# DrorT/demucs

Hardware: AMD Instinct MI355X
Metric: real-time factor (audio-sec/wall-sec) htdemucs 4-stem 44.1kHz stereo, 1/8 GPU (higher is better)
Workload: dtype f32

## Files before the change

demucs_amd/_lib.py:

```python
from __future__ import annotations

import ctypes as C
import os
import threading

_HERE = os.path.dirname(os.path.abspath(__file__))
LIB_PATH = os.environ.get("DEMUCS_AMD_LIB") or os.path.join(_HERE, "libdemucs_amd.so")

MI_OK = 0


class MiTensorDesc(C.Structure):
    _fields_ = [("name", C.c_char_p), ("data", C.c_void_p), ("numel", C.c_int64)]


class MiConfig(C.Structure):
    _fields_ = [("n_sources", C.c_int32), ("segment_length", C.c_int32), ("max_batch", C.c_int32),
                ("dtype", C.c_int32)]


class MiProfileRow(C.Structure):
    _fields_ = [("name", C.c_char * 48), ("launches", C.c_int64), ("ms", C.c_double), ("flops", C.c_double),
                ("bytes", C.c_double)]


class MiConvDesc(C.Structure):
    _fields_ = [
        ("wt", C.c_void_p), ("M", C.c_int32), ("Mpad", C.c_int32), ("K", C.c_int32), ("Kpad", C.c_int32),
        ("ktab", C.c_void_p),
        ("x", C.c_void_p), ("x_bstride", C.c_int64),
        ("B", C.c_int32), ("D1", C.c_int32), ("D2", C.c_int32), ("O1", C.c_int32), ("O2", C.c_int32),
        ("S1", C.c_int32), ("S2", C.c_int32),
        ("pro", C.c_int32), ("pro_stats", C.c_void_p), ("pro_w", C.c_void_p), ("pro_b", C.c_void_p),
        ("row_mode", C.c_int32),
        ("epi", C.c_int32), ("flags", C.c_int32),
        ("bias", C.c_void_p), ("scale", C.c_void_p), ("res", C.c_void_p), ("emb", C.c_void_p),
        ("y", C.c_void_p), ("y_bstride", C.c_int64), ("y_cstride", C.c_int64),
        ("stats", C.c_void_p), ("gn_stats", C.c_void_p), ("gn_w", C.c_void_p), ("gn_b", C.c_void_p),
        ("out_len", C.c_int32), ("tile_m", C.c_int32), ("plain", C.c_int32), ("half", C.c_int32),
        ("o2_valid", C.c_int32), ("ktab_len", C.c_int32), ("sink", C.c_void_p), ("wx", C.c_void_p), ("tr_stride", C.c_int32), ("tr_pad", C.c_int32), ("x_ld", C.c_int32), ("x_ld_pad", C.c_int32), ("wh", C.c_void_p),
        ("xh", C.c_void_p), ("xh_n", C.c_int64), ("yh", C.c_void_p), ("yh_n", C.c_int64),
        ("wtap", C.c_void_p), ("ntaps", C.c_int32), ("tap_k2", C.c_int32), ("tap_pad1", C.c_int32), ("tap_pad2", C.c_int32),
        ("tap_dil1", C.c_int32), ("tap_dil2", C.c_int32), ("yh_pq", C.c_int64),
        ("dma_rows", C.c_int32), ("dma_rows_pad", C.c_int32),
    ]


SIGNATURES = {
    "mi_model_create": (C.c_int, [C.POINTER(MiConfig), C.POINTER(MiTensorDesc), C.c_size_t, C.POINTER(C.c_void_p)]),
    "mi_model_destroy": (None, [C.c_void_p]),
    "mi_model_forward": (C.c_int, [C.c_void_p, C.c_void_p, C.c_void_p, C.c_int32, C.c_void_p]),
    "mi_model_forward_core": (C.c_int, [C.c_void_p, C.c_void_p, C.c_void_p, C.c_void_p, C.c_void_p, C.c_int32, C.c_void_p]),
    "mi_model_tap": (C.c_int, [C.c_void_p, C.c_char_p, C.c_void_p, C.c_int32, C.POINTER(C.c_int64), C.c_void_p]),
    "mi_hmodel_create": (C.c_int, [C.POINTER(MiConfig), C.POINTER(MiTensorDesc), C.c_size_t, C.POINTER(C.c_void_p)]),
    "mi_hmodel_destroy": (None, [C.c_void_p]),
    "mi_hmodel_forward": (C.c_int, [C.c_void_p, C.c_void_p, C.c_void_p, C.c_int32, C.c_int32, C.c_void_p]),
    "mi_hmodel_tap": (C.c_int, [C.c_void_p, C.c_char_p, C.c_void_p, C.c_int32, C.POINTER(C.c_int64), C.c_void_p]),
    "mi_hmodel_device_bytes": (C.c_int64, [C.c_void_p]),
    "mi_hmodel_status": (C.c_int, [C.c_void_p, C.c_void_p]),
    "mi_set_two_streams": (C.c_int, [C.c_int32]),
    "mi_set_split_bf16": (C.c_int, [C.c_int32]),
    "mi_set_istft_fused": (C.c_int, [C.c_int32]),
    "mi_set_transpose_tiles": (C.c_int, [C.c_int32]),
    "mi_profile_begin": (C.c_int, [C.c_void_p]),
    "mi_profile_end": (C.c_int, [C.c_void_p, C.POINTER(MiProfileRow), C.c_int32, C.POINTER(C.c_int32), C.c_void_p]),
    "mi_model_device_bytes": (C.c_int64, [C.c_void_p]),
    "mi_segments_gather": (C.c_int, [C.c_void_p, C.c_int64, C.c_int32, C.c_void_p, C.c_int32, C.c_int32, C.c_void_p,
                                     C.c_int64, C.c_void_p]),
    "mi_ola_accumulate": (C.c_int, [C.c_void_p, C.c_int64, C.c_int32, C.c_void_p, C.c_int32, C.c_int64, C.c_void_p, C.c_void_p,
                                    C.c_void_p, C.c_int32, C.c_int64, C.c_int64, C.c_void_p, C.c_int32, C.c_void_p]),
    "mi_ola_finish": (C.c_int, [C.c_void_p, C.c_int64, C.c_int32, C.c_int64, C.c_void_p, C.c_void_p, C.c_int32,
                                C.c_int32, C.c_void_p, C.c_void_p]),
    "mi_segments_gather_packed": (C.c_int, [C.c_void_p, C.c_int64, C.c_int32, C.c_void_p, C.c_int32, C.c_int32, C.c_void_p,
                                            C.c_int64, C.c_void_p]),
    "mi_ola_accumulate_packed": (C.c_int, [C.c_void_p, C.c_int64, C.c_int32, C.c_void_p, C.c_int32, C.c_int64, C.c_void_p, C.c_int32,
                                           C.c_void_p, C.c_int32, C.c_void_p, C.c_int64, C.c_void_p]),
    "mi_ola_finish_packed": (C.c_int, [C.c_void_p, C.c_int64, C.c_int32, C.c_void_p, C.c_int32, C.c_void_p, C.c_int32, C.c_void_p,
                                       C.c_int64, C.c_void_p]),
    "mi_stream_emit": (C.c_int, [C.c_void_p, C.c_int64, C.c_int32, C.c_int32, C.c_void_p, C.c_int32, C.c_void_p, C.c_int32,
                                 C.c_void_p, C.c_int64, C.c_void_p, C.c_int32, C.c_int32, C.c_int32, C.c_void_p, C.c_int64,
                                 C.c_void_p, C.c_int64, C.c_void_p]),
    "mi_streams_emit": (C.c_int, [C.c_void_p, C.c_int64, C.c_int32, C.c_int32, C.c_void_p, C.c_int32, C.c_int64, C.c_void_p,
                                  C.c_int32, C.c_void_p, C.c_int32, C.c_void_p, C.c_int64, C.c_void_p, C.c_int32, C.c_int32,
                                  C.c_int32, C.c_void_p, C.c_int32, C.c_void_p, C.c_int64, C.c_void_p]),
    "mi_streams_append": (C.c_int, [C.c_void_p, C.c_int64, C.c_int32, C.c_void_p, C.c_int32, C.c_int64, C.c_void_p, C.c_int32,
                                    C.c_void_p]),
    "mi_streams_convert_append": (C.c_int, [C.c_void_p, C.c_int64, C.c_int32, C.c_void_p, C.c_int32, C.c_int64, C.c_void_p, C.c_int64,
                                            C.c_void_p, C.c_int64, C.c_void_p, C.c_int32, C.c_int32, C.c_void_p]),
    "mi_streams_compact": (C.c_int, [C.c_void_p, C.c_int64, C.c_void_p, C.c_int64, C.c_void_p, C.c_int32, C.c_int64, C.c_void_p]),
    "mi_mono_stats_scratch_bytes": (C.c_int32, []),
    "mi_mono_stats": (C.c_int, [C.c_void_p, C.c_int32, C.c_int64, C.c_void_p, C.c_void_p, C.c_void_p]),
    "mi_track_affine": (C.c_int, [C.c_void_p, C.c_int64, C.c_void_p, C.c_int32, C.c_void_p]),
    "mi_prevent_clip": (C.c_int, [C.c_void_p, C.c_int64, C.c_int32, C.c_void_p, C.c_void_p, C.c_void_p]),
    "mi_two_stems": (C.c_int, [C.c_void_p, C.c_int32, C.c_int32, C.c_void_p, C.c_int32, C.c_int64, C.c_void_p, C.c_void_p]),
    "mi_deliver_peaks": (C.c_int, [C.c_void_p, C.c_int32, C.c_int64, C.c_int32, C.c_int32, C.c_void_p, C.c_int32, C.c_int64, C.c_void_p]),
    "mi_deliver_pcm": (C.c_int, [C.c_void_p, C.c_int32, C.c_int64, C.c_int32, C.c_int32, C.c_void_p, C.c_int32, C.c_void_p, C.c_int64,
                                 C.c_void_p]),
    "mi_deliver_resample_pcm": (C.c_int, [C.c_void_p, C.c_int32, C.c_int64, C.c_int32, C.c_int32, C.c_void_p, C.c_int64, C.c_void_p,
                                          C.c_int64, C.c_int32, C.c_void_p, C.c_int64, C.c_void_p]),
    "mi_stft_cac": (C.c_int, [C.c_void_p, C.c_int32, C.c_int32, C.c_void_p, C.c_void_p]),
    "mi_istft_cac": (C.c_int, [C.c_void_p, C.c_int32, C.c_int32, C.c_int32, C.c_void_p, C.c_void_p]),
    "mi_stft_norm": (C.c_int, [C.c_void_p, C.c_int32, C.c_int32, C.c_void_p, C.c_int32, C.c_void_p, C.c_void_p, C.c_void_p]),
    "mi_istft_full": (C.c_int, [C.c_void_p, C.c_int32, C.c_int32, C.c_int32, C.c_int32, C.c_void_p, C.c_void_p, C.c_int32, C.c_void_p,
                                C.c_void_p, C.c_void_p]),
    "mi_item_norm": (C.c_int, [C.c_void_p, C.c_int32, C.c_int64, C.c_void_p, C.c_void_p, C.c_void_p, C.c_void_p]),
    "mi_item_denorm": (C.c_int, [C.c_void_p, C.c_int32, C.c_int64, C.c_void_p, C.c_void_p, C.c_void_p]),
    "mi_conv_forward": (C.c_int, [C.POINTER(MiConvDesc), C.c_void_p]),
    "mi_resample_frac": (C.c_int, [C.c_void_p, C.c_int32, C.c_int64, C.c_void_p, C.c_int32, C.c_int32, C.c_int32, C.c_void_p, C.c_int64,
                                   C.c_void_p]),
    "mi_conv_pack_split": (C.c_int, [C.c_void_p, C.c_int32, C.c_int32, C.c_int32, C.c_void_p, C.c_void_p]),
    "mi_conv_pack_half": (C.c_int, [C.c_void_p, C.c_int32, C.c_int32, C.c_int32, C.c_void_p, C.c_void_p]),
    "mi_f32_to_image": (C.c_int, [C.c_void_p, C.c_int32, C.c_int32, C.c_int64, C.c_int32, C.c_void_p, C.c_void_p]),
    "mi_conv_pack_tap": (C.c_int, [C.c_void_p, C.c_int32, C.c_int32, C.c_int32, C.c_int32, C.c_void_p, C.c_void_p]),
    "mi_attention": (C.c_int, [C.c_void_p, C.c_void_p, C.c_void_p, C.c_void_p, C.c_int32, C.c_int32, C.c_int32,
                               C.c_int32, C.c_int64, C.c_int64, C.c_int64, C.c_int32, C.c_void_p]),
    "mi_attention_split": (C.c_int, [C.c_void_p, C.c_void_p, C.c_void_p, C.c_void_p, C.c_int32, C.c_int32, C.c_int32,
                                     C.c_int32, C.c_int64, C.c_int64, C.c_int64, C.c_void_p]),
    "mi_attention_heads": (C.c_int, [C.c_void_p, C.c_void_p, C.c_void_p, C.c_void_p, C.c_int32, C.c_int32, C.c_int32, C.c_int32,
                                     C.c_int32, C.c_int32, C.c_int32, C.c_void_p]),
    "mi_attention_heads_image": (C.c_int, [C.c_void_p, C.c_void_p, C.c_void_p, C.c_void_p, C.c_int64, C.c_int32, C.c_int32, C.c_int32,
                                           C.c_int32, C.c_int32, C.c_int32, C.c_int32, C.c_void_p]),
    "mi_attention_image": (C.c_int, [C.c_void_p, C.c_void_p, C.c_void_p, C.c_void_p, C.c_int64, C.c_int32, C.c_int32, C.c_int32,
                                     C.c_int32, C.c_int64, C.c_int64, C.c_int32, C.c_void_p]),
    "mi_lstm_seq": (C.c_int, [C.c_void_p, C.c_void_p, C.c_int32, C.c_int32, C.c_int32, C.c_void_p, C.c_int32, C.c_void_p]),
    "mi_gn_gelu": (C.c_int, [C.c_void_p, C.c_int32, C.c_int32, C.c_int32, C.c_int32, C.c_int32, C.c_int32, C.c_void_p, C.c_void_p,
                             C.c_void_p, C.c_void_p]),
    "mi_gram_order": (C.c_int32, [C.c_int32]),
    "mi_gn_gelu_gram": (C.c_int, [C.c_void_p, C.c_int32, C.c_int32, C.c_int32, C.c_int32, C.c_int32, C.c_int32, C.c_int32, C.c_void_p,
                                  C.c_void_p, C.c_void_p, C.c_void_p, C.c_int32, C.c_void_p]),
    "mi_dconv_gn_gelu_gram": (C.c_int, [C.c_void_p, C.c_int32, C.c_int32, C.c_int32, C.c_int32, C.c_int32, C.c_int32, C.c_int32,
                                        C.c_void_p, C.c_void_p, C.c_void_p, C.c_void_p, C.c_int32, C.c_void_p]),
    "mi_gram_finalize": (C.c_int, [C.c_void_p, C.c_int32, C.c_int32, C.c_int32, C.c_void_p, C.c_void_p, C.c_double, C.c_double,
                                   C.c_double, C.c_double, C.c_float, C.c_void_p, C.c_void_p]),
    "mi_layernorm_cf": (C.c_int, [C.c_void_p, C.c_int32, C.c_int32, C.c_int32, C.c_void_p, C.c_void_p, C.c_void_p,
                                  C.c_void_p, C.c_void_p]),
    "mi_token_norm": (C.c_int, [C.c_int32, C.c_void_p, C.c_int32, C.c_int32, C.c_int32, C.c_void_p, C.c_void_p, C.c_void_p, C.c_void_p,
                                C.c_void_p, C.c_void_p, C.c_void_p, C.c_int64, C.c_int32, C.c_void_p]),
    "mi_local_attn": (C.c_int, [C.c_void_p, C.c_int32, C.c_int32, C.c_int32, C.c_int32, C.c_void_p, C.c_int32, C.c_void_p]),
    "mi_group_norm_apply": (C.c_int, [C.c_void_p, C.c_int32, C.c_int32, C.c_int32, C.c_int32, C.c_int32, C.c_int32, C.c_void_p,
                                      C.c_void_p, C.c_int32, C.c_int32, C.c_void_p, C.c_void_p, C.c_int32, C.c_void_p, C.c_int32,
                                      C.c_int32, C.c_int32, C.c_int32, C.c_void_p, C.c_void_p, C.c_void_p]),
    "mi_blstm_unfold": (C.c_int, [C.c_void_p, C.c_int32, C.c_int32, C.c_int32, C.c_int32, C.c_int32, C.c_int32, C.c_void_p, C.c_void_p]),
    "mi_blstm_restitch": (C.c_int, [C.c_void_p, C.c_int32, C.c_int32, C.c_int32, C.c_int32, C.c_int32, C.c_int32, C.c_void_p,
                                    C.c_void_p, C.c_void_p]),
    "mi_row_affine_pitch": (C.c_int, [C.c_void_p, C.c_int32, C.c_int32, C.c_int32, C.c_int32, C.c_void_p, C.c_void_p, C.c_void_p]),
    "mi_dconv_row": (C.c_int, [C.c_void_p, C.c_void_p, C.c_int32, C.c_int32, C.c_int32, C.c_int32, C.c_void_p, C.c_int32, C.c_void_p]),
    "mi_dconv_time_layer": (C.c_int, [C.c_void_p, C.c_void_p, C.c_int32, C.c_int32, C.c_int32, C.c_int32, C.c_int32, C.c_void_p,
                                      C.c_void_p, C.c_void_p, C.c_void_p, C.c_void_p, C.c_void_p]),
    "mi_debug_set_post_launch_hook": (None, [C.c_void_p]),
    "mi_debug_last_conv_route": (C.c_int, []),
    "mi_debug_last_conv_tile": (C.c_int, []),
    "mi_debug_conv_route": (C.c_int, [C.POINTER(MiConvDesc), C.POINTER(C.c_int)]),
    "mi_debug_switches": (C.c_int, [C.c_char_p, C.c_int32]),
    "mi_last_error": (C.c_char_p, []),
    "mi_version": (C.c_char_p, []),
}

_lib = None
_lock = threading.Lock()


class EngineError(RuntimeError):
    """A libdemucs_amd call returned a non-zero status (the reference convention for this path
    is "exceptions propagate", demucs/apply.py:289-293)."""


def load() -> C.CDLL:
    global _lib
    with _lock:
        if _lib is None:
            if not os.path.exists(LIB_PATH):
                raise EngineError(
                    f"{LIB_PATH} not found: build it with `python -c 'import __graft_entry__ as g; g.build()'` "
                    "(hipcc --offload-arch=gfx950).  demucs_amd has no CPU / eager fallback.")
            lib = C.CDLL(LIB_PATH)
            for name, (res, args) in SIGNATURES.items():
                fn = getattr(lib, name)
                fn.restype = res
                fn.argtypes = args
            _lib = lib
    return _lib


def check(status: int, what: str) -> None:
    if status != MI_OK:
        msg = load().mi_last_error().decode(errors="replace")
        raise EngineError(f"{what} failed ({status}): {msg}")


def current_stream_ptr() -> int:
    import torch
    return torch.cuda.current_stream().cuda_stream
```

demucs_amd/csrc/api.hip:

```cpp
#include <new>

#include "hmodel.h"
#include "model.h"

namespace mi {

post_launch_hook_t g_post_launch_hook = nullptr;
int g_last_conv_route = -1;
int g_last_conv_tile = -1;

char *last_error_buf() {
    static thread_local char buf[1024] = "";
    return buf;
}

int set_error(int code, const char *fmt, ...) {
    va_list ap;
    va_start(ap, fmt);
    vsnprintf(last_error_buf(), 1024, fmt, ap);
    va_end(ap);
    return code;
}

struct Tables {
// ... 476 lines not shown
    float *yt = nullptr, *fr = nullptr;
    MI_TRY(ws.get((size_t)B * S * T * 4 * 2048, &yt));
    MI_TRY(ws.get((size_t)B * S * T * 2 * 4096, &fr));
    hipStream_t st = (hipStream_t)stream;
    const int r = launch_istft(y_dev, B, S, L, (const float2 *)denorm_f_dev, xt_dev, (const float2 *)denorm_t_dev, tb, yt, fr, wav_dev, st,
                               xt_pitch, y_pitch);
    return finish_entry(r, st, "mi_istft_full");
}

int mi_istft_cac(const float *x_dev, int32_t B, int32_t S, int32_t L, float *wav_dev, void *stream) {
    MI_REQUIRE(x_dev && wav_dev && B > 0 && S > 0 && (int64_t)B * S <= 16383 && L >= 1, "mi_istft_cac: bad argument");
    return mi_istft_full(x_dev, B, S, L, 0, nullptr, nullptr, 0, nullptr, wav_dev, stream);
}

int mi_item_norm(const float *x_dev, int32_t rows, int64_t count, float *y_dev, float *norm_dev, float *denorm_dev, void *stream) {
    MI_REQUIRE(x_dev && y_dev && norm_dev && denorm_dev, "mi_item_norm: null argument");
    MI_REQUIRE(rows >= 1 && rows <= 65535, "mi_item_norm: rows = %d outside [1, 65535] (the grid's y range)", rows);
    MI_REQUIRE(count >= 2, "mi_item_norm: count = %lld: the unbiased std divides by count - 1", (long long)count);
    TestScratch ws;
    double *stats = nullptr;
    MI_TRY(ws.get((size_t)2 * kStatSlots * rows, &stats));
    hipStream_t st = (hipStream_t)stream;
    MI_HIP(hipMemsetAsync(stats, 0, sizeof(double) * 2 * kStatSlots * rows, st));
    int r = launch_row_stats(x_dev, rows, count, count, stats, st);
    if (r == MI_OK) r = launch_finalize_stats(stats, rows, (double)count, 1e-5f, 1, (float2 *)norm_dev, (float2 *)denorm_dev, st);
    if (r == MI_OK) r = launch_row_affine(x_dev, rows, count, (const float2 *)norm_dev, y_dev, st);
    return finish_entry(r, st, "mi_item_norm");
}

int mi_item_denorm(const float *x_dev, int32_t rows, int64_t count, const float *denorm_dev, float *y_dev, void *stream) {
    MI_REQUIRE(x_dev && denorm_dev && y_dev, "mi_item_denorm: null argument");
    MI_REQUIRE(rows >= 1 && rows <= 65535 && count >= 1, "mi_item_denorm: rows = %d outside [1, 65535] or count = %lld < 1", rows, (long long)count);
    return launch_row_denorm(x_dev, rows, count, (const float2 *)denorm_dev, y_dev, (hipStream_t)stream);
}

int mi_conv_forward(const struct mi_conv_desc *desc, void *stream) {
    MI_REQUIRE(desc, "mi_conv_forward: null descriptor");
    return launch_conv(*desc, (hipStream_t)stream);
}

int mi_resample_frac(const float *x_dev, int32_t rows, int64_t length, const float *table_dev, int32_t old_sr, int32_t new_sr,
                     int32_t width, float *y_dev, int64_t out_length, void *stream) {
    MI_REQUIRE(x_dev && table_dev && y_dev && old_sr > 0 && new_sr > 0 && width > 0, "mi_resample_frac: bad argument");
    return launch_resample_frac(x_dev, rows, length, table_dev, old_sr, new_sr, width, y_dev, out_length, (hipStream_t)stream);
}

int mi_conv_pack_split(const float *wt_dev, int32_t Kpad, int32_t Mpad, int32_t tile_m, void *wx_dev, void *stream) {
    MI_REQUIRE(wt_dev && wx_dev && Kpad > 0 && Mpad > 0 && (conv_x6_supported(tile_m) || tile_m == 192), "mi_conv_pack_split: bad argument");
    MI_REQUIRE(tile_m != 192 || Mpad % 192 == 0, "mi_conv_pack_split: tile_m 192 needs Mpad %% 192 == 0 (Mpad %d)", Mpad);
    return launch_pack_split(wt_dev, Kpad, Mpad, tile_m == 192 ? 96 : tile_m, wx_dev, (hipStream_t)stream);
}

int mi_conv_pack_tap(const float *wt_dev, int32_t Mpad, int32_t Cin, int32_t ntaps, int32_t dtype, void *wtap_dev, void *stream) {
    MI_REQUIRE(wt_dev && wtap_dev && Mpad > 0 && Cin > 0 && ntaps > 0, "mi_conv_pack_tap: bad argument");
    return launch_pack_tap(wt_dev, Mpad, Cin, ntaps, dtype, wtap_dev, (hipStream_t)stream);
}

int mi_f32_to_image(const float *x_dev, int32_t B, int32_t C, int64_t P, int32_t dtype, void *img_dev, void *stream) {
    MI_REQUIRE(x_dev && img_dev && B > 0 && C > 0 && P > 0, "mi_f32_to_image: bad argument");
    return launch_f32_to_image(x_dev, B, C, P, dtype, img_dev, (hipStream_t)stream);
}

int mi_conv_pack_half(const float *wt_dev, int32_t Kpad, int32_t Mpad, int32_t dtype, void *wh_dev, void *stream) {
    MI_REQUIRE(wt_dev && wh_dev && Kpad > 0 && Mpad > 0, "mi_conv_pack_half: bad argument");
    return launch_pack_half(wt_dev, Kpad, Mpad, dtype, wh_dev, (hipStream_t)stream);
}

int mi_attention(const float *q_dev, const float *k_dev, const float *v_dev, float *o_dev, int32_t B, int32_t heads, int32_t Tq,
                 int32_t Tk, int64_t q_batch_stride, int64_t kv_batch_stride, int64_t o_batch_stride, int32_t dtype, void *stream) {
    MI_REQUIRE(q_dev && k_dev && v_dev && o_dev && B > 0 && heads > 0 && Tq > 0 && Tk > 0, "mi_attention: bad argument");
    return launch_attention(q_dev, k_dev, v_dev, o_dev, B, heads, Tq, Tk, q_batch_stride, kv_batch_stride, o_batch_stride, dtype,
                            (hipStream_t)stream);
}

int mi_attention_split(const float *q_dev, const float *k_dev, const float *v_dev, float *o_dev, int32_t B, int32_t heads, int32_t Tq,
                       int32_t Tk, int64_t q_batch_stride, int64_t kv_batch_stride, int64_t o_batch_stride, void *stream) {
    MI_REQUIRE(q_dev && k_dev && v_dev && o_dev && B > 0 && heads > 0 && Tq > 0 && Tk > 0, "mi_attention_split: bad argument");
    return launch_attention_x6(q_dev, k_dev, v_dev, o_dev, B, heads, Tq, Tk, q_batch_stride, kv_batch_stride, o_batch_stride,
                               (hipStream_t)stream);
}

int mi_attention_heads(const void *q_dev, const void *k_dev, const void *v_dev, float *o_dev, int32_t B, int32_t heads, int32_t Tq, int32_t Tk,
                       int32_t Tq_pitch, int32_t Tk_pitch, int32_t dtype, void *stream) {
    MI_REQUIRE(q_dev && k_dev && v_dev && o_dev && B > 0 && heads > 0 && Tq > 0 && Tk > 0, "mi_attention_heads: bad argument");
    const void *zero = conv_zero_page();
    MI_REQUIRE(zero, "mi_attention_heads: could not allocate the zero page");
    return launch_attention_heads(q_dev, k_dev, v_dev, zero, B, heads, Tq, Tk, Tq_pitch, Tk_pitch, dtype, nullptr, 0, o_dev,
                                  (int64_t)heads * 64 * Tq, (hipStream_t)stream);
}

int mi_attention_heads_image(const void *q_dev, const void *k_dev, const void *v_dev, void *img_dev, int64_t n_img, int32_t B, int32_t heads,
                             int32_t Tq, int32_t Tk, int32_t Tq_pitch, int32_t Tk_pitch, int32_t dtype, void *stream) {
    MI_REQUIRE(q_dev && k_dev && v_dev && img_dev && B > 0 && heads > 0 && Tq > 0 && Tk > 0, "mi_attention_heads_image: bad argument");
    const void *zero = conv_zero_page();
    MI_REQUIRE(zero, "mi_attention_heads_image: could not allocate the zero page");
    return launch_attention_heads(q_dev, k_dev, v_dev, zero, B, heads, Tq, Tk, Tq_pitch, Tk_pitch, dtype, img_dev, n_img, nullptr, 0,
                                  (hipStream_t)stream);
}

int mi_attention_image(const float *q_dev, const float *k_dev, const float *v_dev, void *img_dev, int64_t n_img, int32_t B,
                       int32_t heads, int32_t Tq, int32_t Tk, int64_t q_batch_stride, int64_t kv_batch_stride, int32_t dtype,
                       void *stream) {
    MI_REQUIRE(q_dev && k_dev && v_dev && img_dev && B > 0 && heads > 0 && Tq > 0 && Tk > 0, "mi_attention_image: bad argument");
    MI_REQUIRE(dtype == MI_DTYPE_BF16 || dtype == MI_DTYPE_F16, "mi_attention_image: dtype %d is not a half mode", dtype);
    return launch_attention(q_dev, k_dev, v_dev, nullptr, B, heads, Tq, Tk, q_batch_stride, kv_batch_stride, 0, dtype,
                            (hipStream_t)stream, img_dev, n_img);
}

int mi_gn_gelu(float *x_dev, int32_t B, int32_t C, int32_t C_alloc, int32_t D1, int32_t D2, int32_t row_mode, const float *stats_dev,
               const float *w_dev, const float *b_dev, void *stream) {
    MI_REQUIRE(x_dev && stats_dev && w_dev && b_dev && B > 0 && C > 0 && D1 > 0 && D2 > 0, "mi_gn_gelu: bad argument");
    MI_REQUIRE(C_alloc >= C, "mi_gn_gelu: C_alloc < C");
    return launch_gn_gelu(x_dev, B, C, C_alloc, D1, D2, row_mode, (const float2 *)stats_dev, w_dev, b_dev, (hipStream_t)stream);
}

int32_t mi_gram_order(int32_t h) { return gram_hp(h); }

int mi_lstm_seq(const float *gx_dev, const float *whh_host, int32_t N, int32_t H, int32_t W, float *out_dev, int32_t mode, void *stream) {
    MI_REQUIRE(mode == 0 || mode == 1 || mode == 2, "mi_lstm_seq: mode 0 (one launch per step), 1 (persistent kernel) or 2 (generic small kernel)");
    hipStream_t st = (hipStream_t)stream;
    if (mode == 2) {
        MI_REQUIRE(gx_dev && whh_host && out_dev && N > 0 && N <= 65535 && W > 0 && H >= 1 && H <= 64,
                   "mi_lstm_seq: bad argument (mode 2 needs 1 <= H <= 64)");
        const size_t bytes = (size_t)2 * 4 * H * H * sizeof(float);
        float *wn = nullptr;
        MI_HIP(hipMalloc((void **)&wn, bytes));
        int rs = MI_OK;
        if (hipMemcpyAsync(wn, whh_host, bytes, hipMemcpyHostToDevice, st) != hipSuccess) rs = set_error(MI_EHIP, "mi_lstm_seq: hipMemcpyAsync failed");
        if (rs == MI_OK) rs = launch_lstm_small(gx_dev, wn, N, H, W, out_dev, st);
        const hipError_t es = hipStreamSynchronize(st);
        if (es != hipSuccess && rs == MI_OK) rs = set_error(MI_EHIP, "mi_lstm_seq: hipStreamSynchronize: %s", hipGetErrorString(es));
        (void)hipFree(wn);
        return rs;
    }
    MI_REQUIRE(gx_dev && whh_host && out_dev && N > 0 && W > 0 && (H == 192 || H == 384), "mi_lstm_seq: bad argument (H must be 192 or 384)");
    std::vector<float> packed((size_t)2 * 4 * H * H);
    pack_lstm_whh(whh_host, H, packed.data());
    float *wd = nullptr, *state = nullptr;
    void *scratch = nullptr;
    unsigned *flag = nullptr;
    int r = MI_OK;
    auto fail = [&](hipError_t e, const char *what) { if (e != hipSuccess && r == MI_OK) r = set_error(MI_EHIP, "mi_lstm_seq: %s: %s", what, hipGetErrorString(e)); };
    fail(hipMalloc((void **)&wd, packed.size() * sizeof(float)), "hipMalloc");
    fail(hipMalloc((void **)&state, (size_t)6 * N * H * sizeof(float)), "hipMalloc");
    fail(hipMalloc(&scratch, lstm_persist_scratch_bytes()), "hipMalloc");
    fail(hipHostMalloc((void **)&flag, 64, hipHostMallocMapped), "hipHostMalloc");
    if (r == MI_OK) {
        *flag = 0;
        fail(hipMemcpyAsync(wd, packed.data(), packed.size() * sizeof(float), hipMemcpyHostToDevice, st), "hipMemcpyAsync");
        if (r == MI_OK) r = mode ? launch_lstm_persist(gx_dev, wd, N, H, W, out_dev, scratch, flag, st) : launch_lstm_seq(gx_dev, wd, N, H, W, out_dev, state, st);
        fail(hipStreamSynchronize(st), "hipStreamSynchronize");
        if (r == MI_OK && *(volatile unsigned *)flag) r = set_error(MI_EHIP, "mi_lstm_seq: the persistent kernel timed out waiting for its hidden-state exchange");
        if (r == MI_OK && mode && switches().lstm_debug) {
                        unsigned dbg[16] = {};
            (void)hipMemcpy(dbg, (char *)scratch + lstm_persist_ctl_offset(), sizeof(dbg), hipMemcpyDeviceToHost);
            fprintf(stderr, "[lstm] H %d N %d W %d: block 0 / wave 1 spent %.1f us gathering h in %u poll passes (%.2f us, %.2f passes per step); "
                    "%s stores\n", H, N, W, dbg[2] * 0.01, dbg[3], dbg[2] * 0.01 / std::max(1, W - 1), (double)dbg[3] / std::max(1, W - 1),
                    dbg[4] ? "same-XCD plain" : "write-through");
            fprintf(stderr, "[lstm]   shader cycles per step: gather %.0f, issue + products %.0f, LDS write + barrier %.0f, gate stage %.0f; whole step %.0f\n",
                    (double)dbg[8] / W, (double)dbg[9] / W, (double)dbg[10] / W, (double)dbg[11] / W, (double)dbg[12] / W);
        }
    }
    if (wd) (void)hipFree(wd);
    if (state) (void)hipFree(state);
    if (scratch) (void)hipFree(scratch);
    if (flag) (void)hipHostFree(flag);
    return r;
}

int mi_gn_gelu_gram(float *x_dev, int32_t B, int32_t h, int32_t C_alloc, int32_t D1, int32_t D2, int32_t pitch, int32_t row_mode,
                    const float *stats_dev, const float *w_dev, const float *b_dev, double *gram_dev, int32_t slots, void *stream) {
    MI_REQUIRE(x_dev && stats_dev && w_dev && b_dev && gram_dev && B > 0 && h > 0 && D1 > 0 && D2 > 0 && slots > 0, "mi_gn_gelu_gram: bad argument");
    MI_REQUIRE(C_alloc >= h && pitch >= D2, "mi_gn_gelu_gram: C_alloc < h or pitch < D2");
    return launch_gn_gelu_gram(x_dev, B, h, C_alloc, D1, D2, pitch, row_mode, (const float2 *)stats_dev, w_dev, b_dev, gram_dev, slots,
                               false, (hipStream_t)stream);
}

int mi_dconv_gn_gelu_gram(float *x_dev, int32_t B, int32_t h, int32_t C_alloc, int32_t D1, int32_t D2, int32_t pitch, int32_t row_mode,
                          const float *stats_dev, const float *w_dev, const float *b_dev, double *gram_dev, int32_t slots, void *stream) {
    MI_REQUIRE(x_dev && stats_dev && w_dev && b_dev && gram_dev && B > 0 && h > 0 && D1 > 0 && D2 > 0 && slots > 0, "mi_dconv_gn_gelu_gram: bad argument");
    MI_REQUIRE(C_alloc >= h && C_alloc <= gram_hp(h) && pitch >= D2, "mi_dconv_gn_gelu_gram: C_alloc outside [h, mi_gram_order(h)] or pitch < D2");
    return launch_gn_gelu_gram(x_dev, B, h, C_alloc, D1, D2, pitch, row_mode, (const float2 *)stats_dev, w_dev, b_dev, gram_dev, slots,
                               true, (hipStream_t)stream);
}

int mi_gram_finalize(double *gram_dev, int32_t rows, int32_t h, int32_t slots, const double *wt_dev, const double *ct_dev, double sum_b,
                     double sum_bsq, double cols, double count, float eps, float *stats_out_dev, void *stream) {
    MI_REQUIRE(gram_dev && wt_dev && ct_dev && stats_out_dev && rows > 0 && h > 0 && slots > 0 && count > 0.0, "mi_gram_finalize: bad argument");
    return launch_gram_finalize(gram_dev, rows, h, slots, wt_dev, ct_dev, sum_b, sum_bsq, cols, count, eps, (float2 *)stats_out_dev,
                                (hipStream_t)stream);
}

int mi_layernorm_cf(const float *x_dev, int32_t B, int32_t C, int32_t T, const float *w_dev, const float *b_dev,
                    const float *add_dev, float *y_dev, void *stream) {
    MI_REQUIRE(x_dev && w_dev && b_dev && y_dev, "mi_layernorm_cf: null argument");
    return launch_layernorm_cf(x_dev, B, C, T, w_dev, b_dev, add_dev, y_dev, nullptr, (hipStream_t)stream);
}

int mi_token_norm(int32_t mode, const float *x_dev, int32_t B, int32_t C, int32_t T, const float *w_dev, const float *b_dev,
                  const float *pe_dev, const float *gstat_dev, float *y_dev, float *ostat_dev, void *img_dev, int64_t img_n,
                  int32_t img_dtype, void *stream) {
    MI_REQUIRE(mode >= 0 && mode <= 2, "mi_token_norm: mode %d (0 LayerNorm, 1 statistics, 2 GroupNorm(1) apply)", mode);
    MI_REQUIRE(x_dev && B > 0 && B <= 65535 && C > 0 && T > 0, "mi_token_norm: bad argument");
    hipStream_t st = (hipStream_t)stream;
    if (mode == 1) {
        MI_REQUIRE(ostat_dev, "mi_token_norm: mode 1 writes only the statistics, ostat_dev is NULL");
        return launch_token_stats(x_dev, B, C, T, (float2 *)ostat_dev, st, img_dev, img_n, img_dtype);
    }
    MI_REQUIRE(w_dev && b_dev && y_dev, "mi_token_norm: mode %d needs w_dev, b_dev and y_dev", mode);
    if (mode == 0) return launch_layernorm_cf(x_dev, B, C, T, w_dev, b_dev, pe_dev, y_dev, (float2 *)ostat_dev, st, img_dev, img_n, img_dtype);
    MI_REQUIRE(gstat_dev, "mi_token_norm: mode 2 needs gstat_dev");
    return launch_gn_apply_tokstats(x_dev, B, C, T, (const float2 *)gstat_dev, w_dev, b_dev, y_dev, (float2 *)ostat_dev, st, img_dev, img_n,
                                    img_dtype);
}

int mi_local_attn(const float *qkc_dev, int32_t B, int32_t C, int32_t T, int32_t ld, float *out_dev, int32_t ld_o, void *stream) {
    MI_REQUIRE(qkc_dev && out_dev && B > 0 && B <= 65535 && C > 0 && T > 0, "mi_local_attn: bad argument");
    MI_REQUIRE(ld_o >= T, "mi_local_attn: output pitch %d < T = %d", ld_o, T);
    return launch_local_attn(qkc_dev, B, C, T, ld, out_dev, ld_o, (hipStream_t)stream);
}

int mi_group_norm_apply(const float *x_dev, int32_t B, int32_t Cin, int32_t G, int32_t in_pitch, int32_t in_len, int32_t off,
                        const float *w_dev, const float *b_dev, int32_t glu, int32_t gelu, const float *scale_dev, const float *res_dev,
                        int32_t res_pitch, float *y_dev, int32_t Cout, int32_t out_len, int32_t out_pitch, int32_t chan_div,
                        double *stats_ws_dev, float *stats_out_dev, void *stream) {
    MI_REQUIRE(x_dev && w_dev && b_dev && y_dev && stats_ws_dev && stats_out_dev, "mi_group_norm_apply: null argument");
    MI_REQUIRE(B > 0 && B <= 65535 && Cin > 0 && G > 0 && (int64_t)B * G <= 65535 && Cin % G == 0 && Cout > 0 && Cout <= 65535 && in_len > 0 && out_len > 0 &&
               chan_div >= 1 && Cin % chan_div == 0, "mi_group_norm_apply: bad sizes");
    MI_REQUIRE(in_pitch == in_len, "mi_group_norm_apply: statistics need contiguous channel rows (in_pitch %d != in_len %d)", in_pitch, in_len);
    MI_REQUIRE(off >= 0 && (int64_t)off + out_len <= in_len, "mi_group_norm_apply: window [%d, %d + %d) outside the %d input columns", off, off,
               out_len, in_len);
    MI_REQUIRE(out_pitch >= out_len && (!res_dev || res_pitch >= out_len), "mi_group_norm_apply: a row pitch below out_len = %d", out_len);
    hipStream_t st = (hipStream_t)stream;
    const int64_t cnt = (int64_t)(Cin / G) * in_len;
    MI_TRY(launch_row_stats(x_dev, B * G, cnt, cnt, stats_ws_dev, st));
    MI_TRY(launch_finalize_stats(stats_ws_dev, B * G, (double)cnt, 1e-5f, 0, (float2 *)stats_out_dev, nullptr, st));
    return launch_gn_apply(x_dev, B, Cin, G, in_pitch, off, (const float2 *)stats_out_dev, w_dev, b_dev, glu ? 1 : 0, gelu ? 1 : 0, scale_dev,
                           res_dev, res_pitch, y_dev, Cout, out_len, out_pitch, st, chan_div);
}

int mi_blstm_unfold(const float *x_dev, int32_t B, int32_t C, int32_t T, int32_t F, int32_t W, int32_t S, float *frames_dev, void *stream) {
    MI_REQUIRE(x_dev && frames_dev && B > 0 && C > 0 && C <= 65535 && T > 0 && F > 0 && (int64_t)B * F <= 65535 && W > 0 && S > 0,
               "mi_blstm_unfold: bad argument");
    return launch_unfold_frames(x_dev, B, C, T, F, W, S, frames_dev, (hipStream_t)stream);
}

int mi_blstm_restitch(const float *frames_dev, int32_t B, int32_t C, int32_t T, int32_t F, int32_t W, int32_t S, const float *skip_dev,
                      float *y_dev, void *stream) {
    MI_REQUIRE(frames_dev && y_dev && B > 0 && B <= 65535 && C > 0 && C <= 65535 && T > 0 && F > 0 && W > 0 && S > 0,
               "mi_blstm_restitch: bad argument");
    const int64_t per = (int64_t)W - 2 * (S / 2);
    MI_REQUIRE(per > 0 && T <= W + (F - 1) * per, "mi_blstm_restitch: %d frames of %d columns every %d do not cover T = %d", F, W, S, T);
    return launch_restitch_frames(frames_dev, B, C, T, F, W, S, skip_dev, y_dev, (hipStream_t)stream);
}

int mi_row_affine_pitch(const float *x_dev, int32_t B, int32_t C, int32_t L, int32_t out_pitch, const float *norm_dev, float *y_dev,
                        void *stream) {
    MI_REQUIRE(x_dev && norm_dev && y_dev && B > 0 && C > 0 && (int64_t)B * C <= 65535 && L > 0 && out_pitch >= L,
               "mi_row_affine_pitch: bad argument");
    return launch_row_affine_pitch(x_dev, B, C, L, out_pitch, (const float2 *)norm_dev, y_dev, (hipStream_t)stream);
}

int mi_dconv_row(const float *x_dev, float *y_dev, int32_t B, int32_t C, int32_t Fr, int32_t T, const float *weights_host, int32_t variant,
                 void *stream) {
    MI_REQUIRE(x_dev && y_dev && weights_host && B > 0 && Fr > 0 && (int64_t)B * Fr <= (1 << 24), "mi_dconv_row: bad argument");
    MI_REQUIRE(((uintptr_t)x_dev & 7) == 0 && ((uintptr_t)y_dev & 7) == 0, "mi_dconv_row: tensors must be 8-byte aligned");
    MI_REQUIRE(dconv_row_supported(C, T), "mi_dconv_row: C = %d must be 48 or 96, T = %d a multiple of 6 up to 384", C, T);
    MI_REQUIRE(variant == 0 || variant == 1, "mi_dconv_row: variant 0 (one wave per row) or 1 (LDS-resident row)");
    MI_REQUIRE(variant == 0 || dconv_row_lds_supported(C, T), "mi_dconv_row: the LDS-resident kernel does not take C = %d, T = %d", C, T);
    const int64_t n = (int64_t)B * C * Fr * T;
    MI_REQUIRE(x_dev == y_dev || x_dev + n <= y_dev || y_dev + n <= x_dev, "mi_dconv_row: y must be x itself or not overlap it");
    DConvTestLayer l0, l1;
    MI_TRY(l0.init(C, weights_host));
    MI_TRY(l1.init(C, weights_host + dconv_layer_floats(C)));
    hipStream_t st = (hipStream_t)stream;
    const DConvRowArgs a{{l0.l, l1.l}, x_dev, y_dev, Fr, T};
    int r = launch_dconv_row(a, C, B * Fr, variant == 1, st);
    const hipError_t e = hipStreamSynchronize(st);
    if (e != hipSuccess && r == MI_OK) r = set_error(MI_EHIP, "mi_dconv_row: hipStreamSynchronize: %s", hipGetErrorString(e));
    return r;
}

int mi_dconv_time_layer(const float *x_dev, float *y_dev, int32_t B, int32_t C, int32_t Lv, int32_t Lp, int32_t dil,
                        const float *weights_host, float *hbuf_dev, double *stats_dev, double *gram_dev, float *st_dev, void *stream) {
    MI_REQUIRE(x_dev && y_dev && weights_host && hbuf_dev && stats_dev && gram_dev && st_dev, "mi_dconv_time_layer: null argument");
    MI_REQUIRE(B >= 1 && B <= 65535, "mi_dconv_time_layer: B = %d outside [1, 65535] (the grid's y range)", B);
    MI_REQUIRE(dconv_time_supported(C, Lp) && Lv >= 1 && Lp >= Lv, "mi_dconv_time_layer: C = %d must be 48 or 96, Lp = %d even and >= Lv = %d >= 1",
               C, Lp, Lv);
    MI_REQUIRE(dil == 1 || dil == 2, "mi_dconv_time_layer: dilation %d (1 or 2)", dil);
    MI_REQUIRE((((uintptr_t)x_dev | (uintptr_t)y_dev | (uintptr_t)hbuf_dev | (uintptr_t)stats_dev | (uintptr_t)gram_dev | (uintptr_t)st_dev) & 7) == 0,
               "mi_dconv_time_layer: buffers must be 8-byte aligned");
    const int64_t n = (int64_t)B * C * Lp;
    MI_REQUIRE(x_dev + n <= y_dev || y_dev + n <= x_dev, "mi_dconv_time_layer: y must not overlap x");
    DConvTestLayer l;
    MI_TRY(l.init(C, weights_host));
    hipStream_t st = (hipStream_t)stream;
    float2 *st1 = (float2 *)st_dev;
    int r = launch_dconv_time_layer(l.l, C, dil, B, Lv, Lp, x_dev, y_dev, hbuf_dev, stats_dev, gram_dev, st1, st1 + B, st);
    const hipError_t e = hipStreamSynchronize(st);
    if (e != hipSuccess && r == MI_OK) r = set_error(MI_EHIP, "mi_dconv_time_layer: hipStreamSynchronize: %s", hipGetErrorString(e));
    return r;
}

}
```

demucs_amd/csrc/dconv_time.hip:

```cpp
#include "common.h"
#include "kernels.h"

namespace mi {

constexpr int kTC = 6;
constexpr int kGramMax = 96;

__device__ __forceinline__ double wsum(double v) {
#pragma unroll
    for (int off = 32; off > 0; off >>= 1) v += __shfl_xor(v, off);
    return v;
}

struct Taps { float v[10]; };
__device__ __forceinline__ Taps load_taps(const float *row, int t0, int Lv, int Lp) {
    Taps r;
#pragma unroll
    for (int q = 0; q < 5; ++q) {
        const int p = t0 - 2 + 2 * q;
        float2 f = make_float2(0.f, 0.f);
        if (p >= 0 && p < Lp) f = *reinterpret_cast<const float2 *>(row + p);
        r.v[2 * q] = (p >= 0 && p < Lv) ? f.x : 0.f;
        r.v[2 * q + 1] = (p + 1 >= 0 && p + 1 < Lv) ? f.y : 0.f;
    }
    return r;
}

template <int C, int H, int DIL>
__global__ __launch_bounds__(256) void dconv_t_conv3_kernel(const DConvRowLayer L, const float *__restrict__ x, float *__restrict__ hbuf,
                                                            int Lv, int Lp, double *__restrict__ stats) {
    constexpr int HA = (H + 3) / 4 * 4;
    __shared__ __attribute__((aligned(16))) float w0s[C * 3 * HA];
    __shared__ float b0s[HA];
    const int tid = threadIdx.x, b = blockIdx.y;
    for (int i = tid; i < C * 3 * HA; i += 256) w0s[i] = L.w0[i];
    if (tid < HA) b0s[tid] = L.b0[tid];
    __syncthreads();
    const int t0 = (blockIdx.x * 256 + tid) * kTC;
    const bool on = t0 < Lv;
    const float *xb = x + (size_t)b * C * Lp;
    v2f hid[kTC][HA / 2];
#pragma unroll
    for (int j = 0; j < kTC; ++j)
#pragma unroll
        for (int m = 0; m < HA / 2; ++m) hid[j][m] = (v2f){b0s[2 * m], b0s[2 * m + 1]};
    if (on) {
        Taps nx = load_taps(xb, t0, Lv, Lp);
#pragma unroll 2
        for (int c = 0; c < C; ++c) {
            v2f xs[10];
#pragma unroll
            for (int i = 0; i < 10; ++i) xs[i] = splat2(nx.v[i]);
            if (c + 1 < C) nx = load_taps(xb + (size_t)(c + 1) * Lp, t0, Lv, Lp);
            const float4 *wv = reinterpret_cast<const float4 *>(w0s + c * 3 * HA);
#pragma unroll
            for (int q = 0; q < HA / 4; ++q) {
                const float4 wa = wv[q], wb = wv[HA / 4 + q], wc = wv[2 * (HA / 4) + q];
#pragma unroll
                for (int j = 0; j < kTC; ++j) {
                    const v2f x0 = xs[2 + j - DIL], x1 = xs[2 + j], x2 = xs[2 + j + DIL];
                    hid[j][2 * q] = fma2((v2f){wc.x, wc.y}, x2, fma2((v2f){wb.x, wb.y}, x1, fma2((v2f){wa.x, wa.y}, x0, hid[j][2 * q])));
                    hid[j][2 * q + 1] = fma2((v2f){wc.z, wc.w}, x2, fma2((v2f){wb.z, wb.w}, x1, fma2((v2f){wa.z, wa.w}, x0, hid[j][2 * q + 1])));
                }
            }
        }
    }
    double p1 = 0.0, p2 = 0.0;
    if (on) {
        float *hb = hbuf + (size_t)b * HA * Lp + t0;
#pragma unroll
        for (int m = 0; m < H; ++m) {
#pragma unroll
            for (int j = 0; j < kTC; ++j)
                if (t0 + j < Lv) { const double v = (double)hid[j][m >> 1][m & 1]; p1 += v; p2 += v * v; }
#pragma unroll
            for (int j = 0; j < kTC; j += 2)
                if (t0 + j < Lp) *reinterpret_cast<float2 *>(hb + (size_t)m * Lp + j) = make_float2(hid[j][m >> 1][m & 1], hid[j + 1][m >> 1][m & 1]);
        }
    }
    double s1 = wsum(p1), s2 = wsum(p2);
    __shared__ double red[8];
    if ((tid & 63) == 0) { red[(tid >> 6) * 2] = s1; red[(tid >> 6) * 2 + 1] = s2; }
    __syncthreads();
    if (tid == 0) {
        double *dst = stats + ((size_t)b * kStatSlots + (blockIdx.x % kStatSlots)) * 2;
        atomicAdd(dst, red[0] + red[2] + red[4] + red[6]);
        atomicAdd(dst + 1, red[1] + red[3] + red[5] + red[7]);
    }
}

template <int H, int HA>
__device__ __forceinline__ void load_g(const float *hb, int Lp, int t0, int Lv, float mu, float rs, const float *gw, const float *gb,
                                       float (&g)[kTC][HA]) {
#pragma unroll
    for (int m = 0; m < HA; ++m) {
        if (m < H) {
            const float a = rs * gw[m], c = gb[m] - mu * a;
#pragma unroll
            for (int j = 0; j < kTC; j += 2) {
                float2 f = make_float2(0.f, 0.f);
                if (t0 + j < Lp) f = *reinterpret_cast<const float2 *>(hb + (size_t)m * Lp + j);
                g[j][m] = t0 + j < Lv ? gelu_exact(fmaf(f.x, a, c)) : 0.f;
                g[j + 1][m] = t0 + j + 1 < Lv ? gelu_exact(fmaf(f.y, a, c)) : 0.f;
            }
        } else {
#pragma unroll
            for (int j = 0; j < kTC; ++j) g[j][m] = 0.f;
        }
    }
}

template <int H>
__global__ __launch_bounds__(256) void dconv_t_gram_kernel(const DConvRowLayer L, const float *__restrict__ hbuf, int Lv, int Lp,
                                                           const float2 *__restrict__ st1, double *__restrict__ gram) {
    constexpr int HA = (H + 3) / 4 * 4, NG = H * (H + 1) / 2 + H;
    __shared__ double red[4][NG];
    __shared__ float gws[HA], gbs[HA];
    const int tid = threadIdx.x, b = blockIdx.y, lane = tid & 63, wv = tid >> 6;
    if (tid < HA) { gws[tid] = L.g1w[tid]; gbs[tid] = L.g1b[tid]; }
    __syncthreads();
    const int t0 = (blockIdx.x * 256 + tid) * kTC;
    const float2 st = st1[b];
    float g[kTC][HA];
    if (t0 < Lv) load_g<H, HA>(hbuf + (size_t)b * HA * Lp + t0, Lp, t0, Lv, st.x, st.y, gws, gbs, g);
    else {
#pragma unroll
        for (int j = 0; j < kTC; ++j)
#pragma unroll
            for (int m = 0; m < HA; ++m) g[j][m] = 0.f;
    }
    int idx = 0;
#pragma unroll
    for (int i = 0; i < H; ++i) {
#pragma unroll
        for (int k = i; k < H; ++k) {
            float p = 0.f;
#pragma unroll
            for (int j = 0; j < kTC; ++j) p = fmaf(g[j][i], g[j][k], p);
            const double r = wsum((double)p);
            if (lane == 0) red[wv][idx] = r;
            ++idx;
        }
    }
#pragma unroll
    for (int i = 0; i < H; ++i) {
        float p = 0.f;
#pragma unroll
        for (int j = 0; j < kTC; ++j) p += g[j][i];
        const double r = wsum((double)p);
        if (lane == 0) red[wv][idx] = r;
        ++idx;
    }
    __syncthreads();
    if (tid < NG)
        atomicAdd(gram + ((size_t)b * kStatSlots + (blockIdx.x % kStatSlots)) * kGramMax + tid,
                  red[0][tid] + red[1][tid] + red[2][tid] + red[3][tid]);
}

__global__ __launch_bounds__(64) void dconv_t_gram_finalize_kernel(double *__restrict__ gram, int H, const double *__restrict__ ga ,
                                                                   const double *__restrict__ gv ,
                                                                   const double *__restrict__ gc , double sum_b3,
                                                                   double sum_b3sq, double cols, double count, float eps,
                                                                   float2 *__restrict__ out) {
    const int b = blockIdx.x, lane = threadIdx.x;
    const int nq = H * (H + 1) / 2;
    double s1 = 0.0, s2 = 0.0;
    for (int i = lane; i < nq + H; i += 64) {
        double acc = 0.0;
        for (int s = 0; s < kStatSlots; ++s) {
            double *p = gram + ((size_t)b * kStatSlots + s) * kGramMax + i;
            acc += *p;
            *p = 0.0;
        }
        if (i < nq) s2 += ga[i] * acc;
        else { s2 += gv[i - nq] * acc; s1 += gc[i - nq] * acc; }
    }
    s1 = wsum(s1) + cols * sum_b3;
    s2 = wsum(s2) + cols * sum_b3sq;
    if (lane == 0) {
        const double mean = s1 / count;
        double m2 = s2 - s1 * mean;
        if (m2 < 0.0) m2 = 0.0;
        out[b] = make_float2((float)mean, 1.0f / sqrtf((float)(m2 / count) + eps));
    }
}

template <int C, int H>
__global__ __launch_bounds__(256) void dconv_t_out_kernel(const DConvRowLayer L, const float *__restrict__ x, const float *__restrict__ hbuf,
                                                          float *__restrict__ y, int Lv, int Lp, const float2 *__restrict__ st1,
                                                          const float2 *__restrict__ st2) {
    constexpr int HA = (H + 3) / 4 * 4;
    __shared__ __attribute__((aligned(16))) float w3s[4 * C * HA];
    __shared__ float b3s[2 * C], g2ws[2 * C], g2bs[2 * C], lss[C], gws[HA], gbs[HA];
    const int tid = threadIdx.x, b = blockIdx.y;
    for (int i = tid; i < 4 * C * HA; i += 256) {
        const int half = (i >> 1) & 1, k = (i >> 2) % HA, c = (i >> 2) / HA;
        w3s[i] = L.w3[(size_t)(c + half * C) * HA + k];
    }
    for (int i = tid; i < 2 * C; i += 256) { b3s[i] = L.b3[i]; g2ws[i] = L.g2w[i]; g2bs[i] = L.g2b[i]; }
    for (int i = tid; i < C; i += 256) lss[i] = L.ls[i];
    if (tid < HA) { gws[tid] = L.g1w[tid]; gbs[tid] = L.g1b[tid]; }
    __syncthreads();
    const int t0 = (blockIdx.x * 256 + tid) * kTC;
    if (t0 >= Lv) return;
    const float2 s1 = st1[b], s2 = st2[b];
    float g[kTC][HA];
    load_g<H, HA>(hbuf + (size_t)b * HA * Lp + t0, Lp, t0, Lv, s1.x, s1.y, gws, gbs, g);
    const float *xb = x + (size_t)b * C * Lp + t0;
    float *yb = y + (size_t)b * C * Lp + t0;
    const float mu2 = s2.x, rs2 = s2.y;
    auto ld3 = [&](const float *p, float (&r)[kTC]) {
#pragma unroll
        for (int j = 0; j < kTC; j += 2) {
            float2 f = make_float2(0.f, 0.f);
            if (t0 + j < Lp) f = *reinterpret_cast<const float2 *>(p + j);
            r[j] = f.x; r[j + 1] = f.y;
        }
    };
    v2f gp[kTC / 2][HA];
#pragma unroll
    for (int jp = 0; jp < kTC / 2; ++jp)
#pragma unroll
        for (int m = 0; m < HA; ++m) gp[jp][m] = (v2f){g[2 * jp][m], g[2 * jp + 1][m]};
    float rn[kTC];
    ld3(xb, rn);
#pragma unroll 2
    for (int c = 0; c < C; ++c) {
        float r[kTC];
#pragma unroll
        for (int j = 0; j < kTC; ++j) r[j] = rn[j];
        if (c + 1 < C) ld3(xb + (size_t)(c + 1) * Lp, rn);
        const float4 *wp = reinterpret_cast<const float4 *>(w3s + (size_t)c * HA * 4);
        v2f zv[kTC / 2], zg[kTC / 2];
#pragma unroll
        for (int jp = 0; jp < kTC / 2; ++jp) { zv[jp] = splat2(b3s[c]); zg[jp] = splat2(b3s[c + C]); }
#pragma unroll
        for (int k = 0; k < HA; ++k) {
            const float4 w = wp[k];
#pragma unroll
            for (int jp = 0; jp < kTC / 2; ++jp) {
                zv[jp] = fma2((v2f){w.x, w.y}, gp[jp][k], zv[jp]);
                zg[jp] = fma2((v2f){w.z, w.w}, gp[jp][k], zg[jp]);
            }
        }
        const float aA = rs2 * g2ws[c], aB = g2bs[c] - mu2 * aA, gA = rs2 * g2ws[c + C], gB = g2bs[c + C] - mu2 * gA, sc = lss[c];
        float o[kTC];
#pragma unroll
        for (int j = 0; j < kTC; ++j) o[j] = r[j] + sc * (fmaf(zv[j >> 1][j & 1], aA, aB) * sigmoid_f(fmaf(zg[j >> 1][j & 1], gA, gB)));
#pragma unroll
        for (int j = 0; j < kTC; j += 2)
            if (t0 + j < Lp) *reinterpret_cast<float2 *>(yb + (size_t)c * Lp + j) = make_float2(o[j], o[j + 1]);
    }
}

bool dconv_time_supported(int C, int Lp) { return (C == 48 || C == 96) && Lp % 2 == 0; }

int launch_dconv_time_layer(const DConvTimeLayer &l, int C, int dil, int B, int Lv, int Lp, const float *x, float *y, float *hbuf,
                            double *stats, double *gram, float2 *st1, float2 *st2, hipStream_t st) {
    MI_REQUIRE(dconv_time_supported(C, Lp) && (dil == 1 || dil == 2), "dconv_time: unsupported C=%d Lp=%d dil=%d", C, Lp, dil);
    MI_REQUIRE(x != y && ((uintptr_t)x & 7) == 0 && ((uintptr_t)y & 7) == 0 && ((uintptr_t)hbuf & 7) == 0, "dconv_time: bad buffers");
    const int H = C / 8;
    const dim3 grid(ceil_div(Lv, 256 * kTC), B), blk(256);
#define MI_DT(CC, HH)                                                                                                         \
    do {                                                                                                                      \
        if (dil == 1) hipLaunchKernelGGL((dconv_t_conv3_kernel<CC, HH, 1>), grid, blk, 0, st, l.w, x, hbuf, Lv, Lp, stats);      \
        else hipLaunchKernelGGL((dconv_t_conv3_kernel<CC, HH, 2>), grid, blk, 0, st, l.w, x, hbuf, Lv, Lp, stats);               \
        MI_CHECK_LAUNCH();                                                                                                    \
        MI_TRY(launch_finalize_stats(stats, B, (double)HH * Lv, 1e-5f, 0, st1, nullptr, st));                                  \
        hipLaunchKernelGGL((dconv_t_gram_kernel<HH>), grid, blk, 0, st, l.w, hbuf, Lv, Lp, st1, gram);                           \
        MI_CHECK_LAUNCH();                                                                                                    \
        hipLaunchKernelGGL(dconv_t_gram_finalize_kernel, dim3(B), dim3(64), 0, st, gram, HH, l.gram_a, l.gram_v,               \
                           l.gram_c, l.sum_b3, l.sum_b3sq, (double)Lv, 2.0 * CC * Lv, 1e-5f, st2);                             \
        MI_CHECK_LAUNCH();                                                                                                    \
        hipLaunchKernelGGL((dconv_t_out_kernel<CC, HH>), grid, blk, 0, st, l.w, x, hbuf, y, Lv, Lp, st1, st2);                   \
        MI_CHECK_LAUNCH();                                                                                                    \
    } while (0)
    if (C == 48) MI_DT(48, 6);
    else MI_DT(96, 12);
#undef MI_DT
    (void)H;
    return MI_OK;
}

}
```

demucs_amd/csrc/engine_core.h:

```cpp
#pragma once
#include <algorithm>
#include <cstring>
#include <map>
#include <string>
#include <vector>

#include "common.h"
#include "gemm_conv.h"
#include "kernels.h"

namespace mi {

extern int g_two_streams;

struct DeviceArena {
    int64_t bytes = 0;
    DeviceArena() = default;
    DeviceArena(const DeviceArena &) = delete;
    DeviceArena &operator=(const DeviceArena &) = delete;
    int alloc(void **p, size_t n);
    void release(void *p);
    ~DeviceArena();

   private:
    std::map<void *, size_t> sizes;
};

struct PackedConv {
    float *wt = nullptr, *bias = nullptr;
    void *wx = nullptr;
    void *wh = nullptr;
    void *wtap = nullptr;
    int ntaps = 0;
    int M = 0, Mpad = 0, K = 0, Kpad = 0, tile = 0, half = 0;
};

struct DConvLayerW {
    PackedConv conv3, conv1;
    mi_ktab_entry *ktab3 = nullptr, *ktab1 = nullptr;
    float *gn1_w = nullptr, *gn1_b = nullptr, *gn2_w = nullptr, *gn2_b = nullptr, *ls = nullptr;
    double *gram_wt = nullptr, *gram_ct = nullptr, sum_b = 0.0, sum_bsq = 0.0;
};
struct DConvW {
    DConvLayerW l[2];
    int h = 0;
    bool has_row = false;
    DConvRowLayer row[2];
    bool has_time = false;
    DConvTimeLayer tl[2];
};

struct ProfRow {
    int cls = 0;
    char name[48] = "";
    long long launches = 0;
    double ms = 0.0, flops = 0.0, bytes = 0.0;
};
struct Profiler {
    bool on = false;
    struct Pending { int cls; hipEvent_t a, b; double flops, bytes; long long launches = 1; };
    std::vector<Pending> pending;
    std::vector<hipEvent_t> pool;
    ProfRow rows[128];
    hipEvent_t get();
    template <typename Fn>
    int timed(int cls, const char *name, double flops, double bytes, hipStream_t st, Fn &&fn, long long launches = 1) {
        if (!on) return fn();
        Pending p{cls, get(), get(), flops, bytes, launches};
        MI_HIP(hipEventRecord(p.a, st));
        const int r = fn();
        MI_HIP(hipEventRecord(p.b, st));
        pending.push_back(p);
        if (name) snprintf(rows[cls].name, sizeof(rows[cls].name), "%s", name);
        return r;
    }
    void begin();
    int end(hipStream_t st);
    ~Profiler();
};

enum SplitScope {
    SPLIT_OPT_IN,
    SPLIT_DEFAULT,
    SPLIT_ROWS,
};

struct WeightTable {
    std::map<std::string, std::pair<const float *, int64_t>> t;
    int get(const std::string &name, int64_t numel, const float **out) const {
        auto it = t.find(name);
        if (it == t.end()) return set_error(MI_EWEIGHT, "missing tensor '%s'", name.c_str());
        if (it->second.second != numel)
            return set_error(MI_EWEIGHT, "tensor '%s' has %lld elements, expected %lld", name.c_str(),
                             (long long)it->second.second, (long long)numel);
        *out = it->second.first;
        return MI_OK;
    }
};

static inline int round_up(int v, int m) { return (v + m - 1) / m * m; }

struct Gather {
    int Cin, K1, K2, dil1, dil2, pad1, pad2;
    int64_t chan_stride;
    int D2;
};

static inline std::vector<mi_ktab_entry> build_ktab(const Gather &g, int Kpad) {
    std::vector<mi_ktab_entry> tab(Kpad);
    const int K = g.Cin * g.K1 * g.K2;
    for (int k = 0; k < Kpad; ++k) {
        mi_ktab_entry e;
        if (k < K) {
            const int ci = k / (g.K1 * g.K2), r = k % (g.K1 * g.K2), k1 = r / g.K2, k2 = r % g.K2;
            e.d1 = k1 * g.dil1 - g.pad1;
            e.d2 = k2 * g.dil2 - g.pad2;
            e.off = (int32_t)(ci * g.chan_stride + (int64_t)e.d1 * g.D2 + e.d2);
            e.ci = ci;
        } else {
            e.d1 = -(1 << 29); e.d2 = -(1 << 29); e.off = 0; e.ci = 0;
        }
        tab[k] = e;
    }
    return tab;
}

struct Geo {
    int B, D1, D2;
    int row_mode;
    int ld;
    int pitch() const { return ld ? ld : D2; }
};

static inline mi_conv_desc base_desc(const PackedConv &pc, const mi_ktab_entry *ktab, const float *x, int64_t x_bs, const Geo &g) {
    mi_conv_desc d;
    memset(&d, 0, sizeof(d));
    d.wt = pc.wt; d.M = pc.M; d.Mpad = pc.Mpad; d.K = pc.K; d.Kpad = pc.Kpad; d.ktab = ktab; d.bias = pc.bias; d.tile_m = pc.tile; d.wx = pc.wx;
    d.wh = pc.wh; d.half = pc.wh ? pc.half : 0; d.ktab_len = round_up(pc.Kpad, 32);
    d.x = x; d.x_bstride = x_bs; d.B = g.B; d.D1 = g.D1; d.D2 = g.D2; d.O1 = g.D1; d.O2 = g.pitch(); d.S1 = 1; d.S2 = 1;
    d.o2_valid = g.pitch() != g.D2 ? g.D2 : 0;
    d.x_ld = g.pitch() != g.D2 ? g.pitch() : 0;
    d.row_mode = g.row_mode;
    return d;
}

enum EngineKind { ENGINE_HTDEMUCS, ENGINE_HDEMUCS };

struct EngineCore {
    const EngineKind kind;
    mi_config cfg{};
    Profiler prof;
    int conv(const mi_conv_desc &d, hipStream_t st);
    DeviceArena weights;
    FftTables fft{};

    hipStream_t side_st = nullptr;
    hipEvent_t ev_main = nullptr, ev_side = nullptr;
    int side_streams();

   protected:
    explicit EngineCore(EngineKind k) : kind(k) {}
    ~EngineCore();
    template <typename T> int upload(const std::vector<T> &h, T **dptr) {
        void *p = nullptr;
        MI_TRY(weights.alloc(&p, std::max<size_t>(h.size(), 1) * sizeof(T)));
        MI_HIP(hipMemcpy(p, h.data(), h.size() * sizeof(T), hipMemcpyHostToDevice));
        *dptr = (T *)p;
        return MI_OK;
    }
    int upload_fft_tables();
    int pack_split(PackedConv *pc, SplitScope scope);
    int pack_half(PackedConv *pc);
    int pack_conv(const float *W, const float *bias, int M, int K, bool glu, PackedConv *pc, int ntaps = 0, SplitScope scope = SPLIT_OPT_IN);
    int pack_tap(PackedConv *pc, int ntaps);
    int pack_enc_tap(const float *W, int Cin, PackedConv *pc);
    int pack_convtr(const float *W, const float *bias, int Cin, int Cout, PackedConv *pc, int stride = 4, SplitScope scope = SPLIT_OPT_IN);
    int pack_vec(const float *v, int n, int npad, bool glu, float **out);
    int pack_linear_ln(const float *W, const float *bias, const float *ln_w, const float *ln_b, int M, int K, PackedConv *pc,
                       float **c1, SplitScope scope);
    int make_ktab(const Gather &g, int Kpad, mi_ktab_entry **out);
    int load_dconv(const WeightTable &wt, const std::string &prefix, int C, int64_t chan_stride, int D2, bool freq, DConvW *dw, int comp = 8);
    double *dconv_gram = nullptr;
    double *dconv_gram2 = nullptr;
    size_t dconv_gram2_bytes = 0;
    bool dconv_tap_dma = false;
    int run_dconv(const DConvW &w, int C, const Geo &g, float *x, float *tmp, float *hidden, double *stats, float2 *st1, float2 *st2,
                  hipStream_t st, double *gram2 = nullptr, size_t gram2_cap = 0);
};

}
```

demucs_amd/csrc/engine_core.hip:

```cpp
#include <cmath>
#include <string>
#include <vector>

#include "engine_core.h"

namespace mi {

int DeviceArena::alloc(void **p, size_t n) {
    n = (n + 255) & ~(size_t)255;
    hipError_t e = hipMalloc(p, n);
    if (e != hipSuccess) return set_error(MI_ENOMEM, "hipMalloc(%zu) failed: %s", n, hipGetErrorString(e));
    sizes[*p] = n;
    bytes += (int64_t)n;
    return MI_OK;
}
void DeviceArena::release(void *p) {
    auto it = sizes.find(p);
    if (it == sizes.end()) return;
    (void)hipFree(p);
    bytes -= (int64_t)it->second;
    sizes.erase(it);
}
DeviceArena::~DeviceArena() {
    for (auto &a : sizes) (void)hipFree(a.first);
}

int EngineCore::upload_fft_tables() {
    const FftHostTables h = fft_host_tables();
    float *dw, *de; float2 *dt;
    MI_TRY(upload(h.window, &dw)); MI_TRY(upload(h.twiddle, &dt)); MI_TRY(upload(h.envelope, &de));
    fft = FftTables{dw, dt, de};
    return MI_OK;
}

EngineCore::~EngineCore() {
    if (side_st) (void)hipStreamDestroy(side_st);
    if (ev_main) (void)hipEventDestroy(ev_main);
    if (ev_side) (void)hipEventDestroy(ev_side);
}

int g_two_streams = 1;

int EngineCore::side_streams() {
    if (side_st) return MI_OK;
    const int prio = switches().side_prio;
    if (prio) {
        int least = 0, greatest = 0;
        MI_HIP(hipDeviceGetStreamPriorityRange(&least, &greatest));
        MI_HIP(hipStreamCreateWithPriority(&side_st, hipStreamNonBlocking, prio < 0 ? least : greatest));
    } else
        MI_HIP(hipStreamCreateWithFlags(&side_st, hipStreamNonBlocking));
    MI_HIP(hipEventCreateWithFlags(&ev_main, hipEventDisableTiming));
    MI_HIP(hipEventCreateWithFlags(&ev_side, hipEventDisableTiming));
    return MI_OK;
}

hipEvent_t Profiler::get() {
    if (!pool.empty()) { hipEvent_t e = pool.back(); pool.pop_back(); return e; }
    hipEvent_t e;
    (void)hipEventCreate(&e);
    return e;
}
void Profiler::begin() {
    for (auto &r : rows) r = ProfRow();
    on = true;
}
int Profiler::end(hipStream_t st) {
    on = false;
    MI_HIP(hipStreamSynchronize(st));
    for (auto &p : pending) {
        float ms = 0.f;
        MI_HIP(hipEventElapsedTime(&ms, p.a, p.b));
        ProfRow &r = rows[p.cls];
        r.cls = p.cls; r.launches += p.launches; r.ms += ms; r.flops += p.flops; r.bytes += p.bytes;
        pool.push_back(p.a); pool.push_back(p.b);
    }
    pending.clear();
    return MI_OK;
}
Profiler::~Profiler() {
    for (auto &p : pending) { (void)hipEventDestroy(p.a); (void)hipEventDestroy(p.b); }
    for (auto e : pool) (void)hipEventDestroy(e);
}

static const char *kEpiNames[6] = {"linear", "glu", "bias_stats", "stats_only", "gn_glu", "convtr"};

int EngineCore::conv(const mi_conv_desc &d, hipStream_t st) {
    if (!prof.on) return launch_conv(d, st);
    const int route = conv_route(d).route;
    const int tile = d.tile_m && d.tile_m != 192 ? d.tile_m : conv_pick_tile(d.M), ti = tile == 32 ? 0 : tile == 64 ? 1 : tile == 96 ? 2 : 3;
    const bool tap_x6 = route == MI_ROUTE_TAP_X6, rows_x6 = route == MI_ROUTE_ROWS_X6;
    const int cls = tap_x6    ? 105 + (d.ntaps == 9 ? 2 : 0) + (tile == 128 ? 1 : 0)
                    : rows_x6 ? 109 + (d.epi == MI_EPI_CONVTR ? 4 : d.epi == MI_EPI_GLU ? 2 : 0) + (tile == 128 ? 1 : 0)
                              : (route >= MI_ROUTE_X6 ? 48 : 0) + d.epi * 8 + ti * 2 + (d.plain ? 1 : 0);
    const double N = (double)d.B * d.O1 * d.O2;
    const double in_bytes = 4.0 * (double)d.B * (double)d.x_bstride;
    double out_rows = d.M;
    if (d.epi == MI_EPI_GLU || d.epi == MI_EPI_GN_GLU) out_rows = d.M / 2;
    if (d.epi == MI_EPI_CONVTR) out_rows = d.M;
    if (d.epi == MI_EPI_STATS_ONLY) out_rows = 0;
    double bytes = in_bytes + 4.0 * out_rows * N + 4.0 * (double)d.M * d.K;
    if (d.flags & MI_FLAG_RES || d.epi == MI_EPI_GN_GLU) bytes += 4.0 * out_rows * N;
    char name[sizeof(ProfRow::name)];
    const bool unnamed = !prof.rows[cls].name[0];
    if (unnamed && tap_x6)
        snprintf(name, sizeof(name), "conv_tap_x6<%s,tile%d,taps%d>", kEpiNames[d.epi], tile, d.ntaps);
    else if (unnamed && rows_x6)
        snprintf(name, sizeof(name), "conv_rows_x6<%s,tile%d>", kEpiNames[d.epi], tile);
    else if (unnamed)
        snprintf(name, sizeof(name), "conv_gemm%s<%s,tile%d%s>", d.half == MI_DTYPE_BF16 ? "_bf16" : d.half == MI_DTYPE_F16 ? "_f16" : cls >= 48 ? "_x6" : "",
                 kEpiNames[d.epi], tile, d.plain ? ",1x1" : "");
    return prof.timed(cls, unnamed ? name : nullptr, 2.0 * d.M * (double)d.K * N, bytes, st, [&] { return launch_conv(d, st); });
}

int EngineCore::pack_split(PackedConv *pc, SplitScope scope) {
    const Switches &sw = switches();
    const bool in_default = scope == SPLIT_DEFAULT || (scope == SPLIT_ROWS && !sw.no_dma_rows);
    const bool want = sw.x6_scope == 2 || (sw.x6_scope == 1 && in_default && cfg.dtype == MI_DTYPE_F32);
    if (!want || !conv_x6_supported(pc->tile)) return MI_OK;
    const bool t192 = pc->M % 192 == 0 && pc->Mpad == pc->M;
    MI_TRY(weights.alloc(&pc->wx, (size_t)6 * pc->Kpad * pc->Mpad));
    MI_TRY(launch_pack_split(pc->wt, pc->Kpad, pc->Mpad, t192 ? 96 : pc->tile, pc->wx, nullptr));
    MI_HIP(hipStreamSynchronize(nullptr));
    if (t192) pc->tile = 192;
    return MI_OK;
}

int EngineCore::pack_half(PackedConv *pc) {
    if (cfg.dtype == MI_DTYPE_F32) return MI_OK;
    const int Kh = round_up(pc->Kpad, 32);
    MI_TRY(weights.alloc(&pc->wh, (size_t)2 * Kh * pc->Mpad));
    pc->half = cfg.dtype;
    MI_TRY(launch_pack_half(pc->wt, pc->Kpad, pc->Mpad, cfg.dtype, pc->wh, nullptr));
    MI_HIP(hipStreamSynchronize(nullptr));
    return MI_OK;
}

int EngineCore::pack_tap(PackedConv *pc, int ntaps) {
    if (cfg.dtype == MI_DTYPE_F32 || switches().no_tap_image || ntaps < 2 || pc->K % ntaps || (pc->K / ntaps) % 8) return MI_OK;
    const int Cin = pc->K / ntaps;
    MI_TRY(weights.alloc(&pc->wtap, (size_t)16 * conv_tap_pairs_pad(Cin, ntaps) * pc->Mpad));
    pc->ntaps = ntaps;
    MI_TRY(launch_pack_tap(pc->wt, pc->Mpad, Cin, ntaps, cfg.dtype, pc->wtap, nullptr));
    MI_HIP(hipStreamSynchronize(nullptr));
    return MI_OK;
}

int EngineCore::pack_enc_tap(const float *W , int Cin, PackedConv *pc) {
    if (cfg.dtype == MI_DTYPE_F32 || switches().no_enc_image || switches().no_tap_image || Cin % 8) return MI_OK;
    const int M = pc->M, K = 8 * Cin;
    std::vector<float> wt((size_t)K * pc->Mpad, 0.f);
    for (int m = 0; m < M; ++m)
        for (int ci = 0; ci < Cin; ++ci)
            for (int rho = 0; rho < 4; ++rho)
                for (int j = 0; j < 2; ++j) {
                    const int tau = 4 * (j - (rho >= 2)) + rho + 2, ce = ((ci >> 3) * 4 + rho) * 8 + (ci & 7);
                    wt[(size_t)(ce * 2 + j) * pc->Mpad + m] = W[((size_t)m * Cin + ci) * 8 + tau];
                }
    float *tmp = nullptr;
    MI_HIP(hipMalloc((void **)&tmp, wt.size() * sizeof(float)));
    MI_HIP(hipMemcpy(tmp, wt.data(), wt.size() * sizeof(float), hipMemcpyHostToDevice));
    int r = weights.alloc(&pc->wtap, (size_t)16 * conv_tap_pairs_pad(4 * Cin, 2) * pc->Mpad);
    if (r == MI_OK) r = launch_pack_tap(tmp, pc->Mpad, 4 * Cin, 2, cfg.dtype, pc->wtap, nullptr);
    (void)hipStreamSynchronize(nullptr);
    (void)hipFree(tmp);
    if (r == MI_OK) pc->ntaps = 2;
    return r;
}

int EngineCore::pack_conv(const float *W, const float *bias, int M, int K, bool glu, PackedConv *pc, int ntaps, SplitScope scope) {
    const int tile = conv_pick_tile(M);
    pc->M = M; pc->K = K; pc->Mpad = round_up(M, tile); pc->Kpad = round_up(K, 16); pc->tile = tile;
    std::vector<float> wt((size_t)pc->Kpad * pc->Mpad, 0.f), b(pc->Mpad, 0.f);
    for (int m = 0; m < M; ++m) {
        const int src = glu ? ((m & 1) ? (m >> 1) + M / 2 : (m >> 1)) : m;
        for (int k = 0; k < K; ++k) wt[(size_t)k * pc->Mpad + m] = W[(size_t)src * K + k];
        b[m] = bias ? bias[src] : 0.f;
    }
    MI_TRY(upload(wt, &pc->wt));
    MI_TRY(upload(b, &pc->bias));
    MI_TRY(pack_half(pc));
    MI_TRY(pack_tap(pc, ntaps));
    return pack_split(pc, scope);
}

int EngineCore::pack_convtr(const float *W, const float *bias, int Cin, int Cout, PackedConv *pc, int stride, SplitScope scope) {
    const int M = stride * Cout, K = 2 * Cin, ks = 2 * stride;
    const int tile = conv_pick_tile(M);
    pc->M = M; pc->K = K; pc->Mpad = round_up(M, tile); pc->Kpad = round_up(K, 16); pc->tile = tile;
    std::vector<float> wt((size_t)pc->Kpad * pc->Mpad, 0.f), b(pc->Mpad, 0.f);
    for (int ci = 0; ci < Cin; ++ci)
        for (int co = 0; co < Cout; ++co)
            for (int r = 0; r < stride; ++r)
                for (int j = 0; j < 2; ++j)
                    wt[(size_t)(2 * ci + j) * pc->Mpad + stride * co + r] = W[((size_t)ci * Cout + co) * ks + r + stride * j];
    for (int co = 0; co < Cout; ++co)
        for (int r = 0; r < stride; ++r) b[stride * co + r] = bias[co];
    MI_TRY(upload(wt, &pc->wt));
    MI_TRY(upload(b, &pc->bias));
    MI_TRY(pack_half(pc));
    MI_TRY(pack_tap(pc, 2));
    return pack_split(pc, scope);
}

int EngineCore::pack_linear_ln(const float *W, const float *bias, const float *ln_w, const float *ln_b, int M, int K, PackedConv *pc,
                               float **c1, SplitScope scope) {
    std::vector<float> wf((size_t)M * K), c2(M), c1h(M);
    for (int m = 0; m < M; ++m) {
        double s1 = 0.0, s2 = bias ? (double)bias[m] : 0.0;
        for (int k = 0; k < K; ++k) {
            const float wp = W[(size_t)m * K + k] * ln_w[k];
            wf[(size_t)m * K + k] = wp;
            s1 += (double)wp;
            s2 += (double)W[(size_t)m * K + k] * (double)ln_b[k];
        }
        c1h[m] = (float)s1; c2[m] = (float)s2;
    }
    MI_TRY(pack_conv(wf.data(), c2.data(), M, K, false, pc, 0, scope));
    return pack_vec(c1h.data(), M, pc->Mpad, false, c1);
}

int EngineCore::pack_vec(const float *v, int n, int npad, bool glu, float **out) {
    std::vector<float> h(npad, 0.f);
    for (int m = 0; m < n; ++m) h[m] = v[glu ? ((m & 1) ? (m >> 1) + n / 2 : (m >> 1)) : m];
    return upload(h, out);
}

int EngineCore::make_ktab(const Gather &g, int Kpad, mi_ktab_entry **out) {
    return upload(build_ktab(g, round_up(Kpad, 32)), out);
}

int EngineCore::load_dconv(const WeightTable &wt, const std::string &prefix, int C, int64_t chan_stride, int D2, bool freq, DConvW *dw, int comp) {
    const int h = C / comp;
    dw->h = h;
    dw->has_row = comp == 8 && freq && dconv_row_supported(C, D2);
    dw->has_time = comp == 8 && !freq && !switches().no_dconv_time && dconv_time_supported(C, D2);
    for (int d = 0; d < 2; ++d) {
        DConvLayerW &l = dw->l[d];
        const std::string p = prefix + ".dconv.layers." + std::to_string(d);
        const float *w0, *b0, *g1w, *g1b, *w3, *b3, *g2w, *g2b, *ls;
        MI_TRY(wt.get(p + ".0.weight", (int64_t)h * C * 3, &w0));
        MI_TRY(wt.get(p + ".0.bias", h, &b0));
        MI_TRY(wt.get(p + ".1.weight", h, &g1w));
        MI_TRY(wt.get(p + ".1.bias", h, &g1b));
        MI_TRY(wt.get(p + ".3.weight", (int64_t)2 * C * h, &w3));
        MI_TRY(wt.get(p + ".3.bias", 2 * C, &b3));
        MI_TRY(wt.get(p + ".4.weight", 2 * C, &g2w));
        MI_TRY(wt.get(p + ".4.bias", 2 * C, &g2b));
        MI_TRY(wt.get(p + ".6.scale", C, &ls));
        MI_TRY(pack_conv(w0, b0, h, 3 * C, false, &l.conv3));
        const int dil = 1 << d;
        MI_TRY(make_ktab(Gather{C, 1, 3, 1, dil, 0, dil, chan_stride, D2}, l.conv3.Kpad, &l.ktab3));
        const int hp = round_up(h, 16);
        std::vector<float> w3p((size_t)2 * C * hp, 0.f);
        for (int m = 0; m < 2 * C; ++m)
            for (int k = 0; k < h; ++k) w3p[(size_t)m * hp + k] = w3[(size_t)m * h + k];
        MI_TRY(pack_conv(w3p.data(), b3, 2 * C, hp, true, &l.conv1));
        MI_TRY(make_ktab(Gather{hp, 1, 1, 1, 1, 0, 0, chan_stride, D2}, l.conv1.Kpad, &l.ktab1));
        MI_TRY(pack_vec(g1w, h, h, false, &l.gn1_w));
        MI_TRY(pack_vec(g1b, h, h, false, &l.gn1_b));
        MI_TRY(pack_vec(g2w, 2 * C, l.conv1.Mpad, true, &l.gn2_w));
        MI_TRY(pack_vec(g2b, 2 * C, l.conv1.Mpad, true, &l.gn2_b));
        MI_TRY(pack_vec(ls, C, C, false, &l.ls));
        {
            const int HP = gram_hp(h);
            std::vector<double> gw((size_t)HP * HP, 0.0), gc(HP, 0.0);
            double sb = 0.0, sbq = 0.0;
            for (int m = 0; m < 2 * C; ++m) { sb += (double)b3[m]; sbq += (double)b3[m] * (double)b3[m]; }
            for (int i = 0; i < h; ++i) {
                for (int k = 0; k < h; ++k) {
                    if ((k >> 5) < (i >> 5)) continue;
                    double a = 0.0;
                    for (int m = 0; m < 2 * C; ++m) a += (double)w3[(size_t)m * h + i] * (double)w3[(size_t)m * h + k];
                    gw[(size_t)i * HP + k] = (k >> 5) > (i >> 5) ? 2.0 * a : a;
                }
                double v = 0.0, c1 = 0.0;
                for (int m = 0; m < 2 * C; ++m) { v += 2.0 * (double)w3[(size_t)m * h + i] * (double)b3[m]; c1 += (double)w3[(size_t)m * h + i]; }
                gw[(size_t)i * HP + h] = v;
                gc[i] = c1;
            }
            MI_TRY(upload(gw, &l.gram_wt)); MI_TRY(upload(gc, &l.gram_ct));
            l.sum_b = sb; l.sum_bsq = sbq;
        }
        if (dw->has_row || dw->has_time) {
            const DConvHostPack pk = dconv_pack_host(C, h, w0, b0, g1w, g1b, w3, b3);
            float *p0, *p1, *p2, *p3, *p4, *p5, *p6, *p7;
            MI_TRY(upload(pk.w0, &p0)); MI_TRY(upload(pk.b0, &p1)); MI_TRY(upload(pk.g1w, &p2)); MI_TRY(upload(pk.g1b, &p3));
            MI_TRY(upload(pk.w3, &p4));
            MI_TRY(pack_vec(b3, 2 * C, 2 * C, false, &p5)); MI_TRY(pack_vec(g2w, 2 * C, 2 * C, false, &p6));
            MI_TRY(pack_vec(g2b, 2 * C, 2 * C, false, &p7));
            dw->row[d] = DConvRowLayer{p0, p1, p2, p3, p4, p5, p6, p7, l.ls};
            double *da, *dv, *dc, *de1, *de2;
            MI_TRY(upload(pk.gram_a, &da)); MI_TRY(upload(pk.gram_v, &dv)); MI_TRY(upload(pk.gram_c, &dc));
            MI_TRY(upload(pk.gram_e1, &de1)); MI_TRY(upload(pk.gram_e2, &de2));
            dw->tl[d] = DConvTimeLayer{dw->row[d], da, dv, dc, de1, de2, pk.sum_b3, pk.sum_b3sq};
        }
    }
    return MI_OK;
}

int EngineCore::run_dconv(const DConvW &w, int C, const Geo &g, float *x, float *tmp, float *hidden, double *stats, float2 *st1,
                          float2 *st2, hipStream_t st, double *gram2, size_t gram2_cap) {
    if (!gram2) { gram2 = dconv_gram2; gram2_cap = dconv_gram2_bytes; }
    const int h = w.h, hp = round_up(h, 16);
    const int64_t P = (int64_t)g.D1 * g.pitch();
    const int rows = g.row_mode ? g.B * g.D1 : g.B;
    if (w.has_row && g.row_mode == 1) {
        DConvRowArgs a{{w.tl[0], w.tl[1]}, x, x, g.D1, g.D2};
        return prof.timed(101, "dconv_row_kernel", 2.0 * 2.0 * (3.0 * C * h + 2.0 * 2 * C * h) * (double)rows * g.D2,
                          2.0 * 4.0 * C * (double)rows * g.D2, st, [&] { return launch_dconv_row(a, C, rows, switches().dconv_row_lds, st); });
    }
    if (w.has_time && g.row_mode == 0 && g.D1 == 1) {
        MI_REQUIRE(dconv_gram, "dconv: the engine set no Gram buffer for the time kernels");
        return prof.timed(102, "dconv_time_kernels", 2.0 * 2.0 * (3.0 * C * h + 2.0 * C * h) * (double)g.B * g.D2, 2.0 * 4.0 * C * (double)g.B * g.D2, st, [&] {
            float *s = x, *dd = tmp;
            for (int dlayer = 0; dlayer < 2; ++dlayer) {
                MI_TRY(launch_dconv_time_layer(w.tl[dlayer], C, 1 << dlayer, g.B, g.D2, g.pitch(), s, dd, hidden, stats, dconv_gram, st1, st2, st));
                std::swap(s, dd);
            }
            return (int)MI_OK;
        });
    }
    const double cnt_row = g.row_mode ? (double)g.D2 : (double)g.D1 * g.D2;
    float *src = x, *dst = tmp;
    for (int dlayer = 0; dlayer < 2; ++dlayer) {
        const DConvLayerW &l = w.l[dlayer];
        mi_conv_desc d = base_desc(l.conv3, l.ktab3, src, (int64_t)C * P, g);
        d.epi = MI_EPI_BIAS_STATS; d.y = hidden; d.y_bstride = (int64_t)hp * P; d.y_cstride = P; d.stats = stats;
        if (dconv_tap_dma) {
            d.ntaps = 3; d.tap_k2 = 3; d.tap_pad1 = 0; d.tap_pad2 = 1 << dlayer; d.tap_dil2 = 1 << dlayer;
        }
        MI_TRY(conv(d, st));
        MI_TRY(launch_finalize_stats(stats, rows, cnt_row * h, 1e-5f, 0, st1, nullptr, st));
        const int gslots = g.row_mode ? 1 : 8, HP = gram_hp(h);
        MI_REQUIRE((size_t)rows * gslots * HP * HP * sizeof(double) <= gram2_cap, "dconv: Gram accumulators need %zu bytes, workspace has %zu",
                   (size_t)rows * gslots * HP * HP * sizeof(double), gram2_cap);
        MI_TRY(launch_gn_gelu_gram(hidden, g.B, h, hp, g.D1, g.D2, g.pitch(), g.row_mode, st1, l.gn1_w, l.gn1_b, gram2, gslots, true, st));
        MI_TRY(launch_gram_finalize(gram2, rows, h, gslots, l.gram_wt, l.gram_ct, l.sum_b, l.sum_bsq, cnt_row, cnt_row * 2 * C, 1e-5f, st2, st));
        mi_conv_desc e = base_desc(l.conv1, l.ktab1, hidden, (int64_t)hp * P, g);
        e.plain = 1;
        e.epi = MI_EPI_GN_GLU; e.stats = nullptr; e.gn_stats = (const float *)st2; e.gn_w = l.gn2_w; e.gn_b = l.gn2_b;
        e.scale = l.ls; e.res = src; e.y = dst; e.y_bstride = (int64_t)C * P; e.y_cstride = P;
        MI_TRY(conv(e, st));
        std::swap(src, dst);
    }
    return MI_OK;
}

}
```

demucs_amd/csrc/kernels.h:

```cpp
#pragma once
#include <cmath>
#include <vector>
#include <hip/hip_runtime.h>
#include <stdint.h>

#include "gemm_conv.h"

namespace mi {

struct FftTables {
    const float *window;
    const float2 *twiddle;
    const float *envelope;
};
struct FftHostTables {
    std::vector<float> window, envelope;
    std::vector<float2> twiddle;
};
static inline FftHostTables fft_host_tables() {
    FftHostTables t{std::vector<float>(4096), std::vector<float>(1024), std::vector<float2>(2048)};
    for (int i = 0; i < 4096; ++i) t.window[i] = 0.5f - 0.5f * cosf((float)i * (float)(2.0 * M_PI / 4096.0));
    for (int r = 0; r < 1024; ++r) {
        float e = 0.f;
        for (int j = 3; j >= 0; --j) e += t.window[r + 1024 * j] * t.window[r + 1024 * j];
        t.envelope[r] = e;
    }
    for (int i = 0; i < 2048; ++i) { const double a = -2.0 * M_PI * i / 4096.0; t.twiddle[i] = make_float2((float)cos(a), (float)sin(a)); }
    return t;
}

int launch_stft_frames(const float *mix, int B, int L, const FftTables &tb, float *zt, double *stats, hipStream_t st);
int launch_cac_transpose(const float *zt, int B, int T, const float2 *norm, float *x, hipStream_t st, int x_pitch = 0 );
int launch_istft(const float *y, int B, int S, int L, const float2 *denorm, const float *xt, const float2 *denorm_t,
                 const FftTables &tb, float *yt, float *fr, float *out, hipStream_t st, int xt_pitch = 0 ,
                 int y_pitch = 0 );

extern int g_transpose_tiles;
extern int g_istft_fused;

int launch_row_stats(const float *x, int rows, int64_t count, int64_t row_stride, double *stats, hipStream_t st);
int launch_finalize_stats(double *stats, int rows, double count, float eps, int mode, float2 *out_a, float2 *out_b,
                          hipStream_t st);
int launch_row_affine(const float *x, int rows, int64_t count, const float2 *norm, float *y, hipStream_t st);
int launch_row_denorm(const float *x, int rows, int64_t count, const float2 *denorm, float *y, hipStream_t st);
int launch_layernorm_cf(const float *x, int B, int C, int T, const float *w, const float *b, const float *pe, float *y,
                        float2 *ostat, hipStream_t st, void *img = nullptr, int64_t img_n = 0, int img_dtype = 0);
int launch_token_stats(const float *x, int B, int C, int T, float2 *ostat, hipStream_t st, void *img = nullptr, int64_t img_n = 0,
                       int img_dtype = 0);
int launch_gn_apply_tokstats(const float *x, int B, int C, int T, const float2 *gstat, const float *w, const float *b, float *y,
                             float2 *ostat, hipStream_t st, void *img = nullptr, int64_t img_n = 0, int img_dtype = 0);

int gram_hp(int h);
int launch_gn_gelu_gram(float *x, int B, int h, int Cs, int D1, int D2 , int pitch, int row_mode, const float2 *stats, const float *w,
                        const float *b, double *gram , int slots, bool zero_pad, hipStream_t st);
int launch_gram_finalize(double *gram, int rows, int h, int slots, const double *wt , const double *ct , double sum_b,
                         double sum_bsq, double cols, double count, float eps, float2 *out, hipStream_t st);
int launch_gn_gelu(float *x, int B, int C, int Cs, int D1, int D2, int row_mode, const float2 *stats, const float *w, const float *b,
                   hipStream_t st);

struct DConvRowLayer {
    const float *w0;
    const float *b0;
    const float *g1w, *g1b;
    const float *w3;
    const float *b3, *g2w, *g2b;
    const float *ls;
};
struct DConvTimeLayer {
    DConvRowLayer w;
    const double *gram_a;
    const double *gram_v;
    const double *gram_c;
    const double *gram_e1, *gram_e2;
    double sum_b3, sum_b3sq;
};
struct DConvRowArgs {
    DConvTimeLayer l[2];
    const float *x;
    float *y;
    int Fr, T;
};
struct DConvHostPack {
    std::vector<float> w0, b0, g1w, g1b, w3;
    std::vector<double> gram_a, gram_v, gram_c, gram_e1, gram_e2;
    double sum_b3, sum_b3sq;
};
DConvHostPack dconv_pack_host(int C, int h, const float *w0, const float *b0, const float *g1w, const float *g1b, const float *w3,
                              const float *b3);
bool dconv_row_supported(int C, int T);
bool dconv_row_lds_supported(int C, int T);
int launch_dconv_row(const DConvRowArgs &a, int C, int rows, bool lds_row, hipStream_t st);

bool dconv_time_supported(int C, int Lp);
int launch_dconv_time_layer(const DConvTimeLayer &l, int C, int dil, int B, int Lv, int Lp, const float *x, float *y, float *hbuf,
                            double *stats, double *gram, float2 *st1, float2 *st2, hipStream_t st);

int launch_conv(const mi_conv_desc &d, hipStream_t st);

constexpr int BK = 16;
constexpr int BN = 128;
int conv_pick_tile(int M);
int conv_check_tile_m(const mi_conv_desc &d);
int conv_validate(const mi_conv_desc &d);
extern int g_split_bf16;
struct ConvRoute { int route; int tile; bool plain; bool mgroups; };
ConvRoute conv_route(const mi_conv_desc &d);
struct Switches {
    bool no_dma;
    bool no_dma_tap;
    bool no_dma_rows;
    bool no_dma_dconv;
    bool small_tile;
    bool mgroups;
    bool x6_plain_only;
    bool img256;
    bool half_tile256;
    int x6_scope;
    bool no_tap_image;
    bool no_enc_image;
    bool no_dconv_time;
    bool no_lin2_stats;
    bool no_ffn_image;
    bool no_qkv_heads;
    bool no_input_image;
    bool one_stream;
    bool debug_sync;
    int side_prio;
    bool h_no_deep_tap;
    bool h_no_last_tap;
    bool h_one_stream;
    bool lstm_steps;
    bool lstm_write_through;
    bool lstm_debug;
    int transpose_tiles;
    bool istft_split;
    bool dconv_row_lds;
};
const Switches &switches();
constexpr bool conv_x6_supported(int tile) { return tile == 128 || tile == 96 || tile == 64; }
constexpr int kRowTaps = -1;
constexpr bool conv_x6_tile192(int epi, int lflags, bool plain, int ntaps) {
    if (ntaps > 0) return epi == MI_EPI_GLU;
    if (ntaps == kRowTaps) return (epi == MI_EPI_LINEAR && lflags == MI_FLAG_GELU) || epi == MI_EPI_CONVTR || epi == MI_EPI_GLU;
    return plain && epi == MI_EPI_LINEAR && lflags == MI_FLAG_LN;
}
int launch_conv_x6(const mi_conv_desc &d, int tile, int image_tile, bool plain, hipStream_t st);
int launch_conv_tap_x6(const mi_conv_desc &d, int tile, int image_tile, hipStream_t st);
int launch_conv_rows_x6(const mi_conv_desc &d, int tile, int image_tile, hipStream_t st);
int launch_pack_split(const float *wt, int Kpad, int Mpad, int tile_m, void *wx, hipStream_t st);

int launch_conv_half(const mi_conv_desc &d, const ConvRoute &r, hipStream_t st);
int launch_pack_half(const float *wt, int Kpad, int Mpad, int dtype, void *wh, hipStream_t st);
int conv_tap_pairs_pad(int Cin, int ntaps);
int launch_pack_tap(const float *wt, int Mpad, int Cin, int ntaps, int dtype, void *out, hipStream_t st);
int launch_conv_tap(const mi_conv_desc &d, int tile, hipStream_t st);
int launch_f32_to_image(const float *x, int B, int C, int64_t P, int dtype, void *img, hipStream_t st);

int launch_row_affine_pitch(const float *x, int B, int C, int L, int out_pitch, const float2 *norm, float *y, hipStream_t st);
int launch_gn_apply(const float *x, int B, int Cin, int G, int in_pitch, int off, const float2 *stats, const float *w, const float *bias,
                    int glu, int gelu, const float *scale, const float *res, int res_pitch, float *y, int Cout, int out_len,
                    int out_pitch, hipStream_t st, int chan_div = 1);
int launch_unfold_frames(const float *x, int B, int C, int T, int F, int W, int S, float *fr, hipStream_t st);
int launch_restitch_frames(const float *fr, int B, int C, int T, int F, int W, int S, const float *skip, float *y, hipStream_t st);
void pack_lstm_whh(const float *whh , int H, float *packed);
int launch_lstm_seq(const float *gx, const float *whh , int N, int H, int W, float *out, float *state , hipStream_t st);
size_t lstm_persist_scratch_bytes();
size_t lstm_persist_ctl_offset();
int launch_lstm_persist(const float *gx, const float *whh , int N, int H, int W, float *out, void *scratch, unsigned *ctl_host,
                        hipStream_t st);
int launch_lstm_small(const float *gx, const float *whh_natural , int N, int H, int W, float *out, hipStream_t st);
int launch_local_attn(const float *qkc, int B, int C, int T, int ld , float *out, int ld_o, hipStream_t st);

int launch_attention(const float *q, const float *k, const float *v, float *o, int B, int heads, int Tq, int Tk, int64_t q_bs,
                     int64_t kv_bs, int64_t o_bs, int dtype, hipStream_t st, void *oh = nullptr, int64_t oh_n = 0);
int launch_attention_x6(const float *q, const float *k, const float *v, float *o, int B, int heads, int Tq, int Tk, int64_t q_bs,
                        int64_t kv_bs, int64_t o_bs, hipStream_t st);

int launch_segments_gather(const float *track, int64_t track_len, int channels, const int64_t *starts_dev, int B, int valid,
                           float *seg, hipStream_t st);
int launch_ola_accumulate(float *acc, int64_t acc_len, int rows, const float *model_out, int valid, const int64_t *offs_dev,
                          const int32_t *lens_dev, const int32_t *trim_dev, int B, int64_t span_lo, int64_t span_hi,
                          const float *weight, int weight_len, hipStream_t st);
int launch_ola_finish(float *acc, int64_t acc_len, int rows, int64_t acc_off0, const int64_t *offs_dev, const int32_t *lens_dev,
                      int n_segments, int max_len, const float *weight, hipStream_t st);

int launch_segments_gather_packed(const float *tracks, int64_t tracks_cap, int channels, const int64_t *items_dev, int B, int valid,
                                  float *seg, hipStream_t st);
int launch_ola_accumulate_packed(float *acc, int64_t acc_cap, int rows, const float *model_out, int valid, const int64_t *items_dev,
                                 int B, const int64_t *tiles_dev, int n_tiles, const float *weights, int64_t weights_cap,
                                 hipStream_t st);
int launch_ola_finish_packed(float *acc, int64_t acc_cap, int rows, const int64_t *tiles_dev, int n_tiles, const int64_t *segs_dev,
                             int n_segs, const float *weights, int64_t weights_cap, hipStream_t st);

int launch_resample_frac(const float *x, int rows, int64_t L, const float *table, int old_sr, int new_sr, int width, float *y,
                         int64_t Lout, hipStream_t st);

int launch_streams_convert_append(float *win, int64_t win_cap, int channels, const int64_t *table, int n_streams, int64_t max_groups,
                                  const float *bank, int64_t bank_cap, float *hist, int64_t hist_cap, const float *stats, int n_stats,
                                  int lds_floats, hipStream_t st);

const void *conv_zero_page();
int launch_attention_heads(const void *q, const void *k, const void *v, const void *zero_page, int B, int heads, int Tq, int Tk, int Tq_pitch,
                           int Tk_pitch, int dtype, void *oh, int64_t oh_n, float *o, int64_t o_bs, hipStream_t st);

int post_stats_scratch_bytes();
int launch_mono_stats(const float *wav, int channels, int64_t length, double *scratch, float *stats, hipStream_t st);
int launch_stream_emit(const float *acc, int64_t acc_cap, int n_sources, int channels, const int64_t *passes, int n_passes,
                       const int64_t *segs, int n_segs, const float *weights, int64_t weights_cap, const float *scales, int n_members,
                       int shifts, int bag, const float *stats, int64_t n, float *out, hipStream_t st);
int launch_streams_emit(const float *acc, int64_t acc_cap, int n_sources, int channels, const int64_t *streams, int n_streams, int64_t max_n,
                        const int64_t *passes, int n_passes, const int64_t *segs, int n_segs, const float *weights, int64_t weights_cap,
                        const float *scales, int n_members, int shifts, int bag, const float *stats, int n_stats, float *out,
                        int64_t out_cap, hipStream_t st);
int launch_streams_append(float *win, int64_t win_cap, int channels, const int64_t *table, int n_streams, int64_t max_n,
                          const float *stats, int n_stats, hipStream_t st);
int launch_streams_compact(float *dst, int64_t dst_cap, const float *src, int64_t src_cap, const int64_t *table, int n_rows, int64_t max_len,
                           hipStream_t st);
int launch_track_affine(float *x, int64_t n, const float *stats, int mode, hipStream_t st);
int launch_prevent_clip(const float *x, int64_t n, int mode, unsigned *peak, float *y, hipStream_t st);
int launch_two_stems(const float *const *stems, int S, int sel, const float *origin, int mode, int64_t n, float *y, hipStream_t st);

int launch_deliver_peaks(const int64_t *table, int n_rows, int64_t max_n, int n_sources, int channels, unsigned *peaks, int n_peaks,
                         int64_t dst_cap, hipStream_t st);
int launch_deliver_pcm(const int64_t *table, int n_rows, int64_t max_n, int n_sources, int channels, const unsigned *peaks, int n_peaks,
                       unsigned char *dst, int64_t dst_cap, hipStream_t st);

int launch_deliver_resample_pcm(const int64_t *table, int n_rows, int64_t max_groups, int n_sources, int channels, const float *bank,
                                int64_t bank_cap, float *hist, int64_t hist_cap, int lds_floats, unsigned char *dst, int64_t dst_cap,
                                hipStream_t st);

}
```

demucs_amd/csrc/model.h:

```cpp
#pragma once
#include <memory>
#include <string>

#include "engine_core.h"

namespace mi {

struct EncW {
    PackedConv conv, rewrite;
    mi_ktab_entry *ktab_conv = nullptr, *ktab_rw = nullptr;
    DConvW dconv;
};
struct DecW {
    PackedConv rewrite, convtr;
    mi_ktab_entry *ktab_rw = nullptr, *ktab_tr = nullptr;
    DConvW dconv;
};
struct TrLayerW {
    PackedConv qkv_proj, q_proj, kv_proj, out_proj, lin1, lin2;
    float *qkv_c1 = nullptr, *q_c1 = nullptr, *kv_c1 = nullptr, *lin1_c1 = nullptr;
    float *norm_w[4] = {}, *norm_b[4] = {};
    float *gamma1 = nullptr, *gamma2 = nullptr;
};

struct WorkspacePtrs {
    float *w_xt0 = nullptr, *w_zt = nullptr, *w_x0 = nullptr;
    float *w_skip[4] = {}, *w_skip_t[4] = {};
    void *w_eimg[2][3] = {};
    float *w_a = nullptr, *w_b = nullptr, *w_c = nullptr, *w_h = nullptr;
    float *w_ta = nullptr, *w_tb = nullptr, *w_tc = nullptr, *w_th = nullptr;
    float2 *w_tr_stat[2][2] = {}, *w_tr_stat1[2] = {};
    float *w_tr_x[2][2] = {}, *w_tr_qkv[2] = {}, *w_tr_att[2] = {}, *w_tr_x1[2] = {},
          *w_tr_x2[2] = {}, *w_tr_ffh[2] = {};
    float *w_tr_ximg[2][2] = {}, *w_tr_x1img[2] = {};
    float *w_yspec = nullptr, *w_ytime = nullptr, *w_yt = nullptr, *w_fr = nullptr;
    double *w_stats = nullptr, *w_stats_t = nullptr, *w_gram = nullptr, *w_gram2 = nullptr, *w_gram2_t = nullptr;
    size_t gram2t_bytes = 0;
    size_t gram2_bytes = 0;
    float2 *w_st1 = nullptr, *w_st2 = nullptr, *w_st1_t = nullptr, *w_st2_t = nullptr;
    float2 *w_norm_f = nullptr, *w_denorm_f = nullptr, *w_norm_t = nullptr, *w_denorm_t = nullptr;
};
struct Workspace : WorkspacePtrs {
    std::string key;
    DeviceArena mem;
    size_t stats_bytes = 0, gram_bytes = 0;
    bool dirty = false;
};

struct Model : EngineCore, WorkspacePtrs {
    Model() : EngineCore(ENGINE_HTDEMUCS) {}
    struct Plan {
        bool ffn_img = false;
        bool qkv_heads = false;
        bool in_img = false;
        bool lin2_stats = false;
        bool tap_img = false;
        bool enc_img[2][4] = {};
    } plan;
    int attn(const float *q, const float *k, const float *v, float *o, int B, int Tq, int Tk, int64_t q_bs, int64_t kv_bs,
             int64_t o_bs, hipStream_t st, bool image = false);
    int attn_heads(const void *q, const void *k, const void *v, float *o, int B, int Tq, int Tk, hipStream_t st);
    int S = 0, SL = 0, T = 0, Lt[5] = {};
    int Lp[5] = {};

    EncW enc[4], tenc[4];
    DecW dec[4], tdec[4];
    float *freq_emb = nullptr;
    PackedConv chan[4];
    mi_ktab_entry *chan_ktab[4] = {};
    mi_ktab_entry *tr_ktab512[2] = {}, *tr_ktab2048[2] = {};
    float *norm_in_w[2] = {}, *norm_in_b[2] = {}, *pos_emb[2] = {};
    TrLayerW tr[2][5];

    std::shared_ptr<Workspace> ws;

    int init(const mi_config &c, const mi_tensor_desc *weights, size_t n);
    int forward(const float *mix, float *out, int B, hipStream_t st);
    int forward_core(const float *mix, const float *mag, float *spec_out, float *time_out, int B, hipStream_t st);
    int run_core(const float *mix, const float *mag, int B, hipStream_t st);
    int run_core_impl(const float *mix, const float *mag, int B, hipStream_t st);

   protected:
    int alloc_workspace();
    int fill_workspace(Workspace &w);
    int run_tr_layer(int br, int k, int B, const float *x, const float2 *xstat, const float *other, const float2 *ostat, float *out,
                     float2 *outstat, hipStream_t st, const void *ximg, const void *oimg, void *outimg);
};

}
```

demucs_amd/csrc/model.hip:

```cpp
#include <cmath>
#include <map>
#include <memory>
#include <mutex>
#include <string>
#include <vector>

#include "model.h"

namespace mi {

int Model::attn(const float *q, const float *k, const float *v, float *o, int B, int Tq, int Tk, int64_t q_bs, int64_t kv_bs,
                int64_t o_bs, hipStream_t st, bool image) {
    void *oh = image ? (void *)o : nullptr;
    const int64_t oh_n = (int64_t)B * Tq;
    const bool x6 = cfg.dtype == MI_DTYPE_F32 && !image && g_split_bf16 && switches().x6_scope != 0;
    auto launch = [&]() {
        return x6 ? launch_attention_x6(q, k, v, o, B, 8, Tq, Tk, q_bs, kv_bs, o_bs, st)
                  : launch_attention(q, k, v, o, B, 8, Tq, Tk, q_bs, kv_bs, o_bs, cfg.dtype, st, oh, oh_n);
    };
    const int cls = x6 ? 104 : 100;
    const char *name = x6 ? "attention_x6_kernel" : cfg.dtype == MI_DTYPE_BF16 ? "attention_bf16_kernel" : cfg.dtype == MI_DTYPE_F16 ? "attention_f16_kernel" : "attention_kernel";
    return prof.timed(cls, name, 4.0 * B * 8 * (double)Tq * Tk * 64.0, 4.0 * B * 512.0 * (2.0 * Tq + 2.0 * Tk), st, launch);
}

int Model::attn_heads(const void *q, const void *k, const void *v, float *o, int B, int Tq, int Tk, hipStream_t st) {
    const int64_t oh_n = (int64_t)B * Tq;
    const void *zero = conv_zero_page();
    MI_REQUIRE(zero, "attention: could not allocate the zero page");
    return prof.timed(100, cfg.dtype == MI_DTYPE_BF16 ? "attention_heads_bf16_kernel" : "attention_heads_f16_kernel",
                      4.0 * B * 8 * (double)Tq * Tk * 64.0, 2.0 * B * 512.0 * (2.0 * Tq + 2.0 * Tk), st,
                      [&] { return launch_attention_heads(q, k, v, zero, B, 8, Tq, Tk, Tq, Tk, cfg.dtype, o, oh_n, nullptr, 0, st); });
}

static const int kFr[5] = {2048, 512, 128, 32, 8};
static const int kCh[4] = {48, 96, 192, 384};

int Model::init(const mi_config &c, const mi_tensor_desc *weights, size_t n) {
    cfg = c;
    MI_REQUIRE(c.n_sources >= 1 && c.n_sources <= 8, "n_sources %d unsupported", c.n_sources);
    MI_REQUIRE(c.max_batch >= 1 && c.max_batch <= 64, "max_batch %d out of range [1, 64]", c.max_batch);
    MI_REQUIRE(c.dtype == MI_DTYPE_F32 || c.dtype == MI_DTYPE_BF16 || c.dtype == MI_DTYPE_F16, "unknown compute dtype %d", c.dtype);
    MI_REQUIRE(c.segment_length > 4096 && c.segment_length % 4 == 0, "segment_length %d unsupported", c.segment_length);
    S = c.n_sources; SL = c.segment_length; T = (SL + 1023) / 1024;
    MI_REQUIRE(T % 4 == 0, "segment_length %d gives %d STFT frames; the engine needs a multiple of 4", SL, T);
    Lt[0] = SL;
    for (int i = 0; i < 4; ++i) Lt[i + 1] = (Lt[i] + 3) / 4;
    for (int i = 0; i < 5; ++i) Lp[i] = round_up(Lt[i], 4);
    MI_REQUIRE(Lt[4] % 4 == 0, "time branch bottleneck length %d must be a multiple of 4", Lt[4]);
    WeightTable wt;
    for (size_t i = 0; i < n; ++i) wt.t[weights[i].name] = {weights[i].data, weights[i].numel};

    MI_TRY(upload_fft_tables());

    for (int i = 0; i < 4; ++i) {
        const int Cin = i ? kCh[i - 1] : 4, C = kCh[i];
        const std::string p = "encoder." + std::to_string(i);
        const float *w, *b, *rw, *rb;
        MI_TRY(wt.get(p + ".conv.weight", (int64_t)C * Cin * 8, &w));
        MI_TRY(wt.get(p + ".conv.bias", C, &b));
        MI_TRY(wt.get(p + ".rewrite.weight", (int64_t)2 * C * C, &rw));
        MI_TRY(wt.get(p + ".rewrite.bias", 2 * C, &rb));
        EncW &e = enc[i];
        MI_TRY(pack_conv(w, b, C, Cin * 8, false, &e.conv, 0, i > 0 ? SPLIT_ROWS : SPLIT_OPT_IN));
        if (i) MI_TRY(pack_enc_tap(w, Cin, &e.conv));
        MI_TRY(make_ktab(Gather{Cin, 8, 1, 1, 1, 2, 0, (int64_t)kFr[i] * T, T}, e.conv.Kpad, &e.ktab_conv));
        MI_TRY(pack_conv(rw, rb, 2 * C, C, true, &e.rewrite, 0, i >= 2 ? SPLIT_ROWS : SPLIT_OPT_IN));
        MI_TRY(make_ktab(Gather{C, 1, 1, 1, 1, 0, 0, (int64_t)kFr[i + 1] * T, T}, e.rewrite.Kpad, &e.ktab_rw));
        MI_TRY(load_dconv(wt, p, C, (int64_t)kFr[i + 1] * T, T, true, &e.dconv));

        const int Cint = i ? kCh[i - 1] : 2;
        const std::string pt = "tencoder." + std::to_string(i);
        MI_TRY(wt.get(pt + ".conv.weight", (int64_t)C * Cint * 8, &w));
        MI_TRY(wt.get(pt + ".conv.bias", C, &b));
        MI_TRY(wt.get(pt + ".rewrite.weight", (int64_t)2 * C * C, &rw));
        MI_TRY(wt.get(pt + ".rewrite.bias", 2 * C, &rb));
        EncW &te = tenc[i];
        MI_TRY(pack_conv(w, b, C, Cint * 8, false, &te.conv));
        if (i) MI_TRY(pack_enc_tap(w, Cint, &te.conv));
        MI_TRY(make_ktab(Gather{Cint, 1, 8, 1, 1, 0, 2, (int64_t)Lp[i], Lp[i]}, te.conv.Kpad, &te.ktab_conv));
        MI_TRY(pack_conv(rw, rb, 2 * C, C, true, &te.rewrite, 0, i >= 2 ? SPLIT_ROWS : SPLIT_OPT_IN));
        MI_TRY(make_ktab(Gather{C, 1, 1, 1, 1, 0, 0, (int64_t)Lp[i + 1], Lp[i + 1]}, te.rewrite.Kpad, &te.ktab_rw));
        MI_TRY(load_dconv(wt, pt, C, (int64_t)Lp[i + 1], Lp[i + 1], false, &te.dconv));
    }
    {
        const float *ew;
        MI_TRY(wt.get("freq_emb.embedding.weight", 512 * 48, &ew));
        std::vector<float> emb(48 * 512);
        for (int f = 0; f < 512; ++f)
            for (int ch = 0; ch < 48; ++ch) emb[ch * 512 + f] = 0.2f * (ew[f * 48 + ch] * 10.0f);
        MI_TRY(upload(emb, &freq_emb));
    }
    for (int j = 0; j < 4; ++j) {
        const int C = kCh[3 - j], Fr = kFr[4 - j];
        const int Cout = j < 3 ? kCh[2 - j] : 4 * S, Coutt = j < 3 ? kCh[2 - j] : 2 * S;
        const std::string p = "decoder." + std::to_string(j);
        const float *w, *b, *rw, *rb;
        MI_TRY(wt.get(p + ".conv_tr.weight", (int64_t)C * Cout * 8, &w));
        MI_TRY(wt.get(p + ".conv_tr.bias", Cout, &b));
        MI_TRY(wt.get(p + ".rewrite.weight", (int64_t)2 * C * C * 9, &rw));
        MI_TRY(wt.get(p + ".rewrite.bias", 2 * C, &rb));
        DecW &dd = dec[j];
        MI_TRY(pack_conv(rw, rb, 2 * C, C * 9, true, &dd.rewrite, 9, SPLIT_DEFAULT));
        MI_TRY(make_ktab(Gather{C, 3, 3, 1, 1, 1, 1, (int64_t)Fr * T, T}, dd.rewrite.Kpad, &dd.ktab_rw));
        MI_TRY(load_dconv(wt, p, C, (int64_t)Fr * T, T, true, &dd.dconv));
        MI_TRY(pack_convtr(w, b, C, Cout, &dd.convtr, 4, j < 3 ? SPLIT_ROWS : SPLIT_OPT_IN));
        MI_TRY(make_ktab(Gather{C, 2, 1, -1, 1, 0, 0, (int64_t)Fr * T, T}, dd.convtr.Kpad, &dd.ktab_tr));

        const int L = Lp[4 - j];
        const std::string pt = "tdecoder." + std::to_string(j);
        MI_TRY(wt.get(pt + ".conv_tr.weight", (int64_t)C * Coutt * 8, &w));
        MI_TRY(wt.get(pt + ".conv_tr.bias", Coutt, &b));
        MI_TRY(wt.get(pt + ".rewrite.weight", (int64_t)2 * C * C * 3, &rw));
        MI_TRY(wt.get(pt + ".rewrite.bias", 2 * C, &rb));
        DecW &td = tdec[j];
        MI_TRY(pack_conv(rw, rb, 2 * C, C * 3, true, &td.rewrite, 3, SPLIT_DEFAULT));
        MI_TRY(make_ktab(Gather{C, 1, 3, 1, 1, 0, 1, (int64_t)L, L}, td.rewrite.Kpad, &td.ktab_rw));
        MI_TRY(load_dconv(wt, pt, C, (int64_t)L, L, false, &td.dconv));
        MI_TRY(pack_convtr(w, b, C, Coutt, &td.convtr));
        MI_TRY(make_ktab(Gather{C, 1, 2, 1, -1, 0, 0, (int64_t)L, L}, td.convtr.Kpad, &td.ktab_tr));
    }
    const int Tf = 8 * T, Tt = Lt[4];
    {
        const char *names[4] = {"channel_upsampler", "channel_upsampler_t", "channel_downsampler", "channel_downsampler_t"};
        for (int i = 0; i < 4; ++i) {
            const int M = i < 2 ? 512 : 384, K = i < 2 ? 384 : 512, P = (i & 1) ? Tt : Tf;
            const float *w, *b;
            MI_TRY(wt.get(std::string(names[i]) + ".weight", (int64_t)M * K, &w));
            MI_TRY(wt.get(std::string(names[i]) + ".bias", M, &b));
            MI_TRY(pack_conv(w, b, M, K, false, &chan[i]));
            MI_TRY(make_ktab(Gather{K, 1, 1, 1, 1, 0, 0, (int64_t)P, P}, chan[i].Kpad, &chan_ktab[i]));
        }
        for (int br = 0; br < 2; ++br) {
            const int P = br ? Tt : Tf;
            MI_TRY(make_ktab(Gather{512, 1, 1, 1, 1, 0, 0, (int64_t)P, P}, 512, &tr_ktab512[br]));
            MI_TRY(make_ktab(Gather{2048, 1, 1, 1, 1, 0, 0, (int64_t)P, P}, 2048, &tr_ktab2048[br]));
        }
    }
    for (int br = 0; br < 2; ++br) {
        const std::string ni = br ? "crosstransformer.norm_in_t" : "crosstransformer.norm_in";
        const float *w, *b;
        MI_TRY(wt.get(ni + ".weight", 512, &w)); MI_TRY(wt.get(ni + ".bias", 512, &b));
        MI_TRY(pack_vec(w, 512, 512, false, &norm_in_w[br])); MI_TRY(pack_vec(b, 512, 512, false, &norm_in_b[br]));
        for (int k = 0; k < 5; ++k) {
            const std::string p = std::string("crosstransformer.") + (br ? "layers_t." : "layers.") + std::to_string(k);
            const bool cross = k & 1;
            const std::string at = p + (cross ? ".cross_attn" : ".self_attn");
            TrLayerW &l = tr[br][k];
            const float *ipw, *ipb, *ow, *ob, *w1, *b1, *w2, *b2;
            MI_TRY(wt.get(at + ".in_proj_weight", 1536 * 512, &ipw));
            MI_TRY(wt.get(at + ".in_proj_bias", 1536, &ipb));
            MI_TRY(wt.get(at + ".out_proj.weight", 512 * 512, &ow));
            MI_TRY(wt.get(at + ".out_proj.bias", 512, &ob));
            MI_TRY(wt.get(p + ".linear1.weight", 2048 * 512, &w1)); MI_TRY(wt.get(p + ".linear1.bias", 2048, &b1));
            MI_TRY(wt.get(p + ".linear2.weight", 512 * 2048, &w2)); MI_TRY(wt.get(p + ".linear2.bias", 512, &b2));
            const float *nw[4] = {}, *nb[4] = {};
            const char *nn[4] = {".norm1", ".norm2", ".norm3", ".norm_out"};
            for (int q = 0; q < 4; ++q) {
                if (q == 2 && !cross) continue;
                MI_TRY(wt.get(p + nn[q] + ".weight", 512, &nw[q])); MI_TRY(wt.get(p + nn[q] + ".bias", 512, &nb[q]));
            }
            MI_TRY(pack_vec(nw[3], 512, 512, false, &l.norm_w[3])); MI_TRY(pack_vec(nb[3], 512, 512, false, &l.norm_b[3]));
            if (cross) {
                MI_TRY(pack_linear_ln(ipw, ipb, nw[0], nb[0], 512, 512, &l.q_proj, &l.q_c1, SPLIT_DEFAULT));
                MI_TRY(pack_linear_ln(ipw + 512 * 512, ipb + 512, nw[1], nb[1], 1024, 512, &l.kv_proj, &l.kv_c1, SPLIT_DEFAULT));
                MI_TRY(pack_linear_ln(w1, b1, nw[2], nb[2], 2048, 512, &l.lin1, &l.lin1_c1, SPLIT_DEFAULT));
            } else {
                MI_TRY(pack_linear_ln(ipw, ipb, nw[0], nb[0], 1536, 512, &l.qkv_proj, &l.qkv_c1, SPLIT_DEFAULT));
                MI_TRY(pack_linear_ln(w1, b1, nw[1], nb[1], 2048, 512, &l.lin1, &l.lin1_c1, SPLIT_DEFAULT));
            }
            MI_TRY(pack_conv(ow, ob, 512, 512, false, &l.out_proj, 0, SPLIT_DEFAULT));
            MI_TRY(pack_conv(w2, b2, 512, 2048, false, &l.lin2, 0, SPLIT_DEFAULT));
            MI_TRY(wt.get(p + ".gamma_1.scale", 512, &w)); MI_TRY(pack_vec(w, 512, 512, false, &l.gamma1));
            MI_TRY(wt.get(p + ".gamma_2.scale", 512, &w)); MI_TRY(pack_vec(w, 512, 512, false, &l.gamma2));
        }
    }
    {
        std::vector<float> pe2((size_t)512 * Tf), pe1((size_t)512 * Tt);
        for (int i = 0; i < 128; ++i) {
            const float div = expf((float)(2 * i) * (float)(-(log(10000.0) / 256.0)));
            for (int fr = 0; fr < 8; ++fr)
                for (int t1 = 0; t1 < T; ++t1) {
                    const size_t tok = (size_t)fr * T + t1;
                    pe2[(size_t)(2 * i) * Tf + tok] = sinf((float)t1 * div);
                    pe2[(size_t)(2 * i + 1) * Tf + tok] = cosf((float)t1 * div);
                    pe2[(size_t)(256 + 2 * i) * Tf + tok] = sinf((float)fr * div);
                    pe2[(size_t)(256 + 2 * i + 1) * Tf + tok] = cosf((float)fr * div);
                }
        }
        for (int i = 0; i < 256; ++i) {
            const float den = powf(10000.0f, (float)i / 255.0f);
            for (int t2 = 0; t2 < Tt; ++t2) {
                const float ph = (float)t2 / den;
                pe1[(size_t)i * Tt + t2] = cosf(ph);
                pe1[(size_t)(256 + i) * Tt + t2] = sinf(ph);
            }
        }
        MI_TRY(upload(pe2, &pos_emb[0])); MI_TRY(upload(pe1, &pos_emb[1]));
    }
    MI_TRY(alloc_workspace());
    {
        const Switches &sw = switches();
        const bool half = cfg.dtype != MI_DTYPE_F32;
        plan.ffn_img = half && !sw.no_ffn_image;
        plan.qkv_heads = plan.ffn_img && !sw.no_qkv_heads;
        plan.in_img = plan.qkv_heads && !sw.no_input_image;
        plan.lin2_stats = !sw.no_lin2_stats;
        plan.tap_img = half && dec[0].rewrite.wtap && tdec[0].rewrite.wtap;
        for (int i = 1; i < 4; ++i) {
            plan.enc_img[0][i] = enc[i].conv.wtap && w_eimg[0][i - 1];
            plan.enc_img[1][i] = tenc[i].conv.wtap && w_eimg[1][i - 1];
        }
    }
    MI_HIP(hipDeviceSynchronize());
    return MI_OK;
}

static std::mutex g_ws_mutex;
static std::map<std::string, std::weak_ptr<Workspace>> g_ws;

int Model::alloc_workspace() {
    int dev = 0;
    MI_HIP(hipGetDevice(&dev));
    char key[128];
    snprintf(key, sizeof(key), "htdemucs dev%d S%d SL%d B%d %s", dev, S, SL, cfg.max_batch, cfg.dtype == MI_DTYPE_F32 ? "f32" : "half");
    std::lock_guard<std::mutex> lock(g_ws_mutex);
    auto it = g_ws.find(key);
    if (it != g_ws.end()) ws = it->second.lock();
    if (!ws) {
        auto w = std::make_shared<Workspace>();
        w->key = key;
        MI_TRY(fill_workspace(*w));
        g_ws[key] = w;
        ws = w;
    }
    static_cast<WorkspacePtrs &>(*this) = *ws;
    dconv_gram = w_gram; dconv_gram2 = w_gram2; dconv_gram2_bytes = gram2_bytes;
    dconv_tap_dma = true;
    return MI_OK;
}

int Model::fill_workspace(Workspace &w) {
    const size_t B = cfg.max_batch;
    auto A = [&](float **p, size_t per_item) { return w.mem.alloc((void **)p, per_item * B * sizeof(float)); };
    auto dev_alloc = [&](void **p, size_t n) { return w.mem.alloc(p, n); };
    MI_TRY(A(&w.w_xt0, (size_t)2 * SL));
    MI_TRY(A(&w.w_zt, (size_t)4 * 2048 * T));
    MI_TRY(A(&w.w_x0, (size_t)4 * 2048 * T));
    size_t big = 0;
    for (int i = 0; i < 4; ++i) {
        const size_t nf = (size_t)kCh[i] * kFr[i + 1] * T, nt = (size_t)kCh[i] * Lp[i + 1];
        MI_TRY(A(&w.w_skip[i], nf)); MI_TRY(A(&w.w_skip_t[i], nt));
        big = std::max(big, std::max(nf, nt));
    }
    if (cfg.dtype != MI_DTYPE_F32)
        for (int i = 0; i < 3; ++i) {
            const size_t pqf = (size_t)(kFr[i + 1] / 4 + 1) * T, pqt = round_up(ceil_div(Lt[i + 1], 4) + 1, 4);
            float *pf = nullptr, *pt = nullptr;
            MI_TRY(A(&pf, 2 * kCh[i] * pqf)); MI_TRY(A(&pt, 2 * kCh[i] * pqt));
            MI_HIP(hipMemset(pf, 0, 2 * kCh[i] * pqf * B * sizeof(float)));
            MI_HIP(hipMemset(pt, 0, 2 * kCh[i] * pqt * B * sizeof(float)));
            w.w_eimg[0][i] = pf; w.w_eimg[1][i] = pt;
        }
    MI_TRY(A(&w.w_h, big / 2)); MI_TRY(A(&w.w_th, big / 2));
    for (float **p : {&w.w_a, &w.w_b, &w.w_ta, &w.w_tb, &w.w_c, &w.w_tc}) {
        MI_TRY(w.mem.alloc((void **)p, (big * B + 64) * sizeof(float)));
        *p += 32;
    }
    MI_HIP(hipMemset(w.w_h, 0, (big / 2) * B * sizeof(float)));
    MI_HIP(hipMemset(w.w_th, 0, (big / 2) * B * sizeof(float)));
    const size_t Tf = 8 * (size_t)T, Tt = Lt[4];
    for (int br = 0; br < 2; ++br) {
        const size_t P = br ? Tt : Tf;
        MI_TRY(A(&w.w_tr_x[br][0], 512 * P)); MI_TRY(A(&w.w_tr_x[br][1], 512 * P));
        if (cfg.dtype != MI_DTYPE_F32) {
            MI_TRY(A(&w.w_tr_ximg[br][0], 256 * P)); MI_TRY(A(&w.w_tr_ximg[br][1], 256 * P)); MI_TRY(A(&w.w_tr_x1img[br], 256 * P));
        }
        for (int q = 0; q < 2; ++q) MI_TRY(dev_alloc((void **)&w.w_tr_stat[br][q], B * P * sizeof(float2)));
        MI_TRY(dev_alloc((void **)&w.w_tr_stat1[br], B * P * sizeof(float2)));
        MI_TRY(A(&w.w_tr_qkv[br], 1536 * Tf)) ; MI_TRY(A(&w.w_tr_att[br], 512 * P));
        MI_TRY(A(&w.w_tr_x1[br], 512 * P)); MI_TRY(A(&w.w_tr_x2[br], 512 * P)); MI_TRY(A(&w.w_tr_ffh[br], 2048 * P));
    }
    MI_TRY(A(&w.w_yspec, (size_t)4 * S * 2048 * T));
    MI_TRY(A(&w.w_ytime, (size_t)2 * S * SL));
    MI_TRY(A(&w.w_yt, (size_t)4 * S * 2048 * T));
    MI_TRY(A(&w.w_fr, (size_t)S * T * 2 * 4096));
    const size_t max_rows = B * 512;
    w.stats_bytes = max_rows * kStatSlots * 2 * sizeof(double);
    MI_TRY(dev_alloc((void **)&w.w_stats, w.stats_bytes));
    MI_TRY(dev_alloc((void **)&w.w_stats_t, w.stats_bytes));
    w.gram_bytes = B * kStatSlots * 96 * sizeof(double);
    MI_TRY(dev_alloc((void **)&w.w_gram, w.gram_bytes));
    MI_HIP(hipMemset(w.w_gram, 0, w.gram_bytes));
    w.gram2_bytes = B * ((size_t)4 << 20);
    MI_TRY(dev_alloc((void **)&w.w_gram2, w.gram2_bytes));
    MI_HIP(hipMemset(w.w_gram2, 0, w.gram2_bytes));
    w.gram2t_bytes = B * ((size_t)1 << 20);
    MI_TRY(dev_alloc((void **)&w.w_gram2_t, w.gram2t_bytes));
    MI_HIP(hipMemset(w.w_gram2_t, 0, w.gram2t_bytes));
    MI_HIP(hipMemset(w.w_stats, 0, w.stats_bytes));
    MI_HIP(hipMemset(w.w_stats_t, 0, w.stats_bytes));
    MI_TRY(dev_alloc((void **)&w.w_st1, max_rows * sizeof(float2)));
    MI_TRY(dev_alloc((void **)&w.w_st2, max_rows * sizeof(float2)));
    MI_TRY(dev_alloc((void **)&w.w_st1_t, max_rows * sizeof(float2)));
    MI_TRY(dev_alloc((void **)&w.w_st2_t, max_rows * sizeof(float2)));
    MI_TRY(dev_alloc((void **)&w.w_norm_f, B * sizeof(float2))); MI_TRY(dev_alloc((void **)&w.w_denorm_f, B * sizeof(float2)));
    MI_TRY(dev_alloc((void **)&w.w_norm_t, B * sizeof(float2))); MI_TRY(dev_alloc((void **)&w.w_denorm_t, B * sizeof(float2)));
    return MI_OK;
}

#define MI_STAGE(name)                                                                        \
    do {                                                                                      \
        if (switches().debug_sync) {                                                          \
            hipError_t _e = hipStreamSynchronize(st);                                         \
            fprintf(stderr, "[mi] reached %s (%s)\n", name, hipGetErrorString(_e));          \
            fflush(stderr);                                                                   \
            if (_e != hipSuccess) return set_error(MI_EHIP, "stage before %s failed: %s", name, hipGetErrorString(_e)); \
        }                                                                                     \
    } while (0)

int Model::run_tr_layer(int br, int k, int B, const float *x, const float2 *xstat, const float *other, const float2 *ostat,
                        float *out, float2 *outstat, hipStream_t st, const void *ximg, const void *oimg, void *outimg) {
    const TrLayerW &l = tr[br][k];
    const bool cross = k & 1;
    const int Tf = 8 * T, Tt = Lt[4];
    const int Tq = br ? Tt : Tf, Tk = cross ? (br ? Tf : Tt) : Tq;
    const Geo gq{B, 1, Tq, 0}, gk{B, 1, Tk, 0};
    float *qkv = w_tr_qkv[br], *att = w_tr_att[br], *x1 = w_tr_x1[br], *x2 = w_tr_x2[br], *ffh = w_tr_ffh[br];
    double *stats = br ? w_stats_t : w_stats;
    float2 *st1 = br ? w_st1_t : w_st1;
    const bool img = plan.ffn_img, heads = plan.qkv_heads, in_img = plan.in_img, lin2_stats = plan.lin2_stats;
    unsigned short *qh = reinterpret_cast<unsigned short *>(qkv);
    const size_t plane_q = (size_t)B * 512 * Tq, plane_k = (size_t)B * 512 * Tk;
    if (!cross) {
        mi_conv_desc d = base_desc(l.qkv_proj, tr_ktab512[br], x, (int64_t)512 * Tq, gq);
        d.plain = 1; d.epi = MI_EPI_LINEAR; d.flags = MI_FLAG_LN; d.scale = l.qkv_c1; d.pro_stats = (const float *)xstat;
        d.y = qkv; d.y_bstride = (int64_t)1536 * Tq; d.y_cstride = Tq;
        if (heads) { d.flags |= MI_FLAG_HEADS; d.yh = qh; d.yh_n = Tq; }
        if (in_img) { d.xh = ximg; d.xh_n = (int64_t)B * Tq; }
        MI_TRY(conv(d, st));
        if (heads) MI_TRY(attn_heads(qh, qh + plane_q, qh + 2 * plane_q, att, B, Tq, Tq, st));
        else MI_TRY(attn(qkv, qkv + (size_t)512 * Tq, qkv + (size_t)1024 * Tq, att, B, Tq, Tq, (int64_t)1536 * Tq, (int64_t)1536 * Tq,
                         (int64_t)512 * Tq, st, img));
    } else {
        mi_conv_desc d = base_desc(l.q_proj, tr_ktab512[br], x, (int64_t)512 * Tq, gq);
        d.plain = 1; d.epi = MI_EPI_LINEAR; d.flags = MI_FLAG_LN; d.scale = l.q_c1; d.pro_stats = (const float *)xstat;
        d.y = qkv; d.y_bstride = (int64_t)512 * Tq; d.y_cstride = Tq;
        if (heads) { d.flags |= MI_FLAG_HEADS; d.yh = qh; d.yh_n = Tq; }
        if (in_img) { d.xh = ximg; d.xh_n = (int64_t)B * Tq; }
        MI_TRY(conv(d, st));
        float *kv = qkv + (size_t)B * 512 * Tq;
        unsigned short *kvh = qh + plane_q;
        mi_conv_desc e = base_desc(l.kv_proj, tr_ktab512[1 - br], other, (int64_t)512 * Tk, gk);
        e.plain = 1; e.epi = MI_EPI_LINEAR; e.flags = MI_FLAG_LN; e.scale = l.kv_c1; e.pro_stats = (const float *)ostat;
        e.y = kv; e.y_bstride = (int64_t)1024 * Tk; e.y_cstride = Tk;
        if (heads) { e.flags |= MI_FLAG_HEADS; e.yh = kvh; e.yh_n = Tk; }
        if (in_img) { e.xh = oimg; e.xh_n = (int64_t)B * Tk; }
        MI_TRY(conv(e, st));
        if (heads) MI_TRY(attn_heads(qh, kvh, kvh + plane_k, att, B, Tq, Tk, st));
        else MI_TRY(attn(qkv, kv, kv + (size_t)512 * Tk, att, B, Tq, Tk, (int64_t)512 * Tq, (int64_t)1024 * Tk, (int64_t)512 * Tq, st, img));
    }
    {
        mi_conv_desc d = base_desc(l.out_proj, tr_ktab512[br], att, (int64_t)512 * Tq, gq);
        d.plain = 1; d.epi = MI_EPI_LINEAR; d.flags = MI_FLAG_SCALE | MI_FLAG_RES; d.scale = l.gamma1; d.res = x;
        d.y = x1; d.y_bstride = (int64_t)512 * Tq; d.y_cstride = Tq;
        if (img) { d.xh = att; d.xh_n = (int64_t)B * Tq; }
        MI_TRY(conv(d, st));
    }
    MI_TRY(launch_token_stats(x1, B, 512, Tq, w_tr_stat1[br], st, in_img ? w_tr_x1img[br] : nullptr, (int64_t)B * Tq, cfg.dtype));
    {
        mi_conv_desc d = base_desc(l.lin1, tr_ktab512[br], x1, (int64_t)512 * Tq, gq);
        d.plain = 1; d.epi = MI_EPI_LINEAR; d.flags = MI_FLAG_LN | MI_FLAG_GELU; d.scale = l.lin1_c1;
        d.pro_stats = (const float *)w_tr_stat1[br];
        d.y = ffh; d.y_bstride = (int64_t)2048 * Tq; d.y_cstride = Tq;
        if (img) { d.flags |= MI_FLAG_IMG; d.yh = ffh; d.yh_n = (int64_t)B * Tq; }
        if (in_img) { d.xh = w_tr_x1img[br]; d.xh_n = (int64_t)B * Tq; }
        MI_TRY(conv(d, st));
        mi_conv_desc e = base_desc(l.lin2, tr_ktab2048[br], ffh, (int64_t)2048 * Tq, gq);
        if (img) { e.xh = ffh; e.xh_n = (int64_t)B * Tq; }
        e.plain = 1; e.epi = MI_EPI_LINEAR; e.flags = MI_FLAG_SCALE | MI_FLAG_RES; e.scale = l.gamma2; e.res = x1;
        if (lin2_stats) { e.flags |= MI_FLAG_STATS; e.stats = stats; }
        e.y = x2; e.y_bstride = (int64_t)512 * Tq; e.y_cstride = Tq;
        MI_TRY(conv(e, st));
    }
    if (!lin2_stats) MI_TRY(launch_row_stats(x2, B, (int64_t)512 * Tq, (int64_t)512 * Tq, stats, st));
    MI_TRY(launch_finalize_stats(stats, B, (double)512 * Tq, 1e-5f, 0, st1, nullptr, st));
    MI_TRY(launch_gn_apply_tokstats(x2, B, 512, Tq, st1, l.norm_w[3], l.norm_b[3], out, outstat, st, in_img ? outimg : nullptr,
                                    (int64_t)B * Tq, cfg.dtype));
    return MI_OK;
}

int Model::run_core(const float *mix, const float *mag, int B, hipStream_t st) {
    if (ws->dirty) {
        MI_HIP(hipMemsetAsync(w_stats, 0, ws->stats_bytes, st));
        MI_HIP(hipMemsetAsync(w_stats_t, 0, ws->stats_bytes, st));
        MI_HIP(hipMemsetAsync(w_gram, 0, ws->gram_bytes, st));
        MI_HIP(hipMemsetAsync(w_gram2, 0, gram2_bytes, st));
        MI_HIP(hipMemsetAsync(w_gram2_t, 0, gram2t_bytes, st));
        ws->dirty = false;
    }
    const int r = run_core_impl(mix, mag, B, st);
    if (r != MI_OK) {
        ws->dirty = true;
        if (side_st) (void)hipStreamSynchronize(side_st);
    }
    return r;
}

int Model::forward(const float *mix, float *out, int B, hipStream_t st) {
    MI_REQUIRE(mix && out, "forward: null buffer");
    MI_TRY(run_core(mix, nullptr, B, st));
    MI_TRY(launch_istft(w_yspec, B, S, SL, w_denorm_f, w_ytime, w_denorm_t, fft, w_yt, w_fr, out, st));
    MI_STAGE("istft done");
    return MI_OK;
}

int Model::forward_core(const float *mix, const float *mag, float *spec_out, float *time_out, int B, hipStream_t st) {
    MI_REQUIRE(mix && spec_out && time_out, "forward_core: null buffer");
    MI_TRY(run_core(mix, mag, B, st));
    MI_TRY(launch_row_denorm(w_yspec, B, (int64_t)4 * S * 2048 * T, w_denorm_f, spec_out, st));
    MI_TRY(launch_row_denorm(w_ytime, B, (int64_t)2 * S * SL, w_denorm_t, time_out, st));
    return MI_OK;
}

int Model::run_core_impl(const float *mix, const float *mag, int B, hipStream_t st) {
    MI_REQUIRE(B >= 1 && B <= cfg.max_batch, "forward: batch %d outside [1, %d]", B, cfg.max_batch);
    const int Tf = 8 * T, Tt = Lt[4];
    const bool two = !switches().one_stream && g_two_streams && !switches().debug_sync && side_streams() == MI_OK;
    hipStream_t stt = two ? side_st : st;
    auto fork = [&]() -> int {
        if (!two) return MI_OK;
        MI_HIP(hipEventRecord(ev_main, st));
        MI_HIP(hipStreamWaitEvent(side_st, ev_main, 0));
        return MI_OK;
    };
    auto join = [&]() -> int {
        if (!two) return MI_OK;
        MI_HIP(hipEventRecord(ev_side, side_st));
        MI_HIP(hipStreamWaitEvent(st, ev_side, 0));
        return MI_OK;
    };
    MI_TRY(fork());
    MI_TRY(launch_row_stats(mix, B, (int64_t)2 * SL, (int64_t)2 * SL, w_stats_t, stt));
    MI_TRY(launch_finalize_stats(w_stats_t, B, 2.0 * SL, 1e-5f, 1, w_norm_t, w_denorm_t, stt));
    MI_TRY(launch_row_affine(mix, B, (int64_t)2 * SL, w_norm_t, w_xt0, stt));
    MI_STAGE("time normalisation done");
    if (mag) {
        const int64_t cnt = (int64_t)4 * 2048 * T;
        MI_TRY(launch_row_stats(mag, B, cnt, cnt, w_stats, st));
        MI_TRY(launch_finalize_stats(w_stats, B, (double)cnt, 1e-5f, 1, w_norm_f, w_denorm_f, st));
        MI_TRY(launch_row_affine(mag, B, cnt, w_norm_f, w_x0, st));
    } else {
        MI_TRY(launch_stft_frames(mix, B, SL, fft, w_zt, w_stats, st));
        MI_TRY(launch_finalize_stats(w_stats, B, 4.0 * 2048 * T, 1e-5f, 1, w_norm_f, w_denorm_f, st));
        MI_TRY(launch_cac_transpose(w_zt, B, T, w_norm_f, w_x0, st));
    }
    MI_STAGE("stft done");

    const float *xf = w_x0, *xt = w_xt0;
    for (int i = 0; i < 4; ++i) {
        const int Cin = i ? kCh[i - 1] : 4, Cint = i ? kCh[i - 1] : 2, C = kCh[i];
        {
            const Geo gin{B, kFr[i], T, 1}, go{B, kFr[i + 1], T, 1};
            const int64_t Pin = (int64_t)kFr[i] * T, P = (int64_t)kFr[i + 1] * T;
            mi_conv_desc d = base_desc(enc[i].conv, enc[i].ktab_conv, xf, Cin * Pin, gin);
            d.O1 = kFr[i + 1]; d.S1 = 4; d.epi = MI_EPI_LINEAR; d.flags = MI_FLAG_GELU;
            d.y = w_a; d.y_bstride = C * P; d.y_cstride = P;
            d.dma_rows = 1;
            if (plan.enc_img[0][i]) {
                const int Q = kFr[i] / 4 + 1;
                d.xh = w_eimg[0][i - 1]; d.xh_n = (int64_t)cfg.max_batch * Q * T; d.wtap = enc[i].conv.wtap; d.ntaps = 2; d.tap_k2 = 1;
                d.D1 = Q; d.S1 = 1;
            }
            MI_TRY(conv(d, st));
            MI_STAGE("enc conv done");
            MI_TRY(run_dconv(enc[i].dconv, C, go, w_a, w_b, w_h, w_stats, w_st1, w_st2, st));
            MI_STAGE("enc dconv done");
            mi_conv_desc r = base_desc(enc[i].rewrite, enc[i].ktab_rw, w_a, C * P, go);
            r.plain = 1; r.epi = MI_EPI_GLU; r.y = w_skip[i]; r.y_bstride = C * P; r.y_cstride = P;
            if (i == 0) { r.flags = MI_FLAG_EMB; r.emb = freq_emb; }
            if (i < 3 && plan.enc_img[0][i + 1]) {
                const int64_t pq = (int64_t)(kFr[i + 1] / 4 + 1) * T;
                r.flags |= MI_FLAG_IMG4 | MI_FLAG_TR_FREQ; r.yh = w_eimg[0][i]; r.yh_pq = pq; r.yh_n = (int64_t)cfg.max_batch * pq;
            }
            MI_TRY(conv(r, st));
            xf = w_skip[i];
            MI_STAGE("enc rewrite done");
        }
        {
            const Geo gin{B, 1, Lt[i], 0, Lp[i]}, go{B, 1, Lt[i + 1], 0, Lp[i + 1]};
            const int64_t P = Lp[i + 1];
            mi_conv_desc d = base_desc(tenc[i].conv, tenc[i].ktab_conv, xt, (int64_t)Cint * Lp[i], gin);
            d.O2 = Lp[i + 1]; d.o2_valid = Lt[i + 1]; d.S2 = 4; d.epi = MI_EPI_LINEAR; d.flags = MI_FLAG_GELU;
            d.y = w_ta; d.y_bstride = C * P; d.y_cstride = P;
            if (plan.enc_img[1][i]) {
                const int Qp = round_up(ceil_div(Lt[i], 4) + 1, 4);
                d.xh = w_eimg[1][i - 1]; d.xh_n = (int64_t)cfg.max_batch * Qp; d.wtap = tenc[i].conv.wtap; d.ntaps = 2; d.tap_k2 = 2;
                d.D2 = Qp; d.x_ld = Qp; d.S2 = 1;
            }
            MI_TRY(conv(d, stt));
            MI_TRY(run_dconv(tenc[i].dconv, C, go, w_ta, w_tb, w_th, w_stats_t, w_st1_t, w_st2_t, stt, w_gram2_t, gram2t_bytes));
            mi_conv_desc r = base_desc(tenc[i].rewrite, tenc[i].ktab_rw, w_ta, C * P, go);
            r.plain = 1; r.epi = MI_EPI_GLU; r.y = w_skip_t[i]; r.y_bstride = C * P; r.y_cstride = P;
            if (i < 3 && plan.enc_img[1][i + 1]) {
                const int64_t pq = round_up(ceil_div(Lt[i + 1], 4) + 1, 4);
                r.flags |= MI_FLAG_IMG4; r.yh = w_eimg[1][i]; r.yh_pq = pq; r.yh_n = (int64_t)cfg.max_batch * pq;
            }
            MI_TRY(conv(r, stt));
            xt = w_skip_t[i];
            MI_STAGE("tenc layer done");
        }
    }
    int cur[2] = {0, 0};
    const bool in_img = plan.in_img;
    for (int br = 0; br < 2; ++br) {
        const int P = br ? Tt : Tf;
        const Geo g{B, 1, P, 0};
        hipStream_t sb = br ? stt : st;
        mi_conv_desc d = base_desc(chan[br], chan_ktab[br], br ? xt : xf, (int64_t)384 * P, g);
        d.plain = 1; d.epi = MI_EPI_LINEAR; d.y = w_tr_x1[br]; d.y_bstride = (int64_t)512 * P; d.y_cstride = P;
        MI_TRY(conv(d, sb));
        MI_TRY(launch_layernorm_cf(w_tr_x1[br], B, 512, P, norm_in_w[br], norm_in_b[br], pos_emb[br], w_tr_x[br][0],
                                   w_tr_stat[br][0], sb, in_img ? w_tr_ximg[br][0] : nullptr, (int64_t)B * P, cfg.dtype));
    }
    MI_STAGE("upsample + norm_in done");
    for (int k = 0; k < 5; ++k) {
        const float *f_in = w_tr_x[0][cur[0]], *t_in = w_tr_x[1][cur[1]];
        const float2 *f_st = w_tr_stat[0][cur[0]], *t_st = w_tr_stat[1][cur[1]];
        const void *f_img = in_img ? w_tr_ximg[0][cur[0]] : nullptr, *t_img = in_img ? w_tr_ximg[1][cur[1]] : nullptr;
        MI_TRY(join());
        MI_TRY(fork());
        MI_TRY(run_tr_layer(0, k, B, f_in, f_st, t_in, t_st, w_tr_x[0][cur[0] ^ 1], w_tr_stat[0][cur[0] ^ 1], st, f_img, t_img,
                            w_tr_ximg[0][cur[0] ^ 1]));
        MI_TRY(run_tr_layer(1, k, B, t_in, t_st, f_in, f_st, w_tr_x[1][cur[1] ^ 1], w_tr_stat[1][cur[1] ^ 1], stt, t_img, f_img,
                            w_tr_ximg[1][cur[1] ^ 1]));
        cur[0] ^= 1; cur[1] ^= 1;
        MI_STAGE("transformer layer done");
    }
    float *din = w_c, *dtin = w_tc;
    const bool tapimg = plan.tap_img;
    for (int br = 0; br < 2; ++br) {
        const int P = br ? Tt : Tf;
        const Geo g{B, 1, P, 0};
        mi_conv_desc d = base_desc(chan[2 + br], chan_ktab[2 + br], w_tr_x[br][cur[br]], (int64_t)512 * P, g);
        d.plain = 1; d.epi = MI_EPI_LINEAR; d.flags = MI_FLAG_RES; d.res = br ? w_skip_t[3] : w_skip[3];
        d.y = br ? dtin : din; d.y_bstride = (int64_t)384 * P; d.y_cstride = P;
        if (tapimg) { d.flags |= MI_FLAG_IMG; d.yh = br ? dtin : din; d.yh_n = (int64_t)B * P; }
        MI_TRY(conv(d, br ? stt : st));
    }
    for (int j = 0; j < 4; ++j) {
        const int C = kCh[3 - j], Fr = kFr[4 - j];
        const bool last = j == 3;
        {
            const Geo g{B, Fr, T, 1};
            const int64_t P = (int64_t)Fr * T;
            mi_conv_desc r = base_desc(dec[j].rewrite, dec[j].ktab_rw, din, C * P, g);
            r.epi = MI_EPI_GLU; r.y = w_a; r.y_bstride = C * P; r.y_cstride = P;
            r.ntaps = 9; r.tap_k2 = 3; r.tap_pad1 = 1; r.tap_pad2 = 1;
            if (tapimg) { r.xh = din; r.xh_n = (int64_t)B * P; r.wtap = dec[j].rewrite.wtap; }
            MI_TRY(conv(r, st));
            MI_TRY(run_dconv(dec[j].dconv, C, g, w_a, w_b, w_h, w_stats, w_st1, w_st2, st));
            const int Cout = last ? 4 * S : kCh[2 - j];
            mi_conv_desc t = base_desc(dec[j].convtr, dec[j].ktab_tr, w_a, C * P, g);
            t.O1 = Fr + 1; t.epi = MI_EPI_CONVTR; t.flags = MI_FLAG_TR_FREQ; t.out_len = 4 * Fr;
            t.y_cstride = (int64_t)4 * Fr * T; t.y_bstride = Cout * t.y_cstride;
            t.dma_rows = 1;
            if (last) t.y = w_yspec;
// ... 39 lines not shown
```

include/demucs_amd.h:

```cpp
#ifndef DEMUCS_AMD_H
#define DEMUCS_AMD_H

#include <stddef.h>
#include <stdint.h>

#ifdef __cplusplus
extern "C" {
#endif

#define MI_OK 0
#define MI_EINVAL (-1)
#define MI_EHIP (-2)
#define MI_ENOMEM (-3)
#define MI_EWEIGHT (-4)

typedef struct mi_tensor_desc {
    const char *name;
    const float *data;
    int64_t numel;
} mi_tensor_desc;

typedef struct mi_config {
    int32_t n_sources;
    int32_t segment_length;
    int32_t max_batch;
    int32_t dtype;
} mi_config;

#define MI_DTYPE_F32 0
#define MI_DTYPE_BF16 1
#define MI_DTYPE_F16 2

int mi_model_create(const mi_config *cfg, const mi_tensor_desc *weights, size_t n_weights, void **handle);
void mi_model_destroy(void *handle);

int mi_model_forward(void *handle, const float *mix_dev, float *out_dev, int32_t B, void *stream);

int mi_model_forward_core(void *handle, const float *mix_dev, const float *mag_dev, float *spec_out_dev,
                          float *time_out_dev, int32_t B, void *stream);

int mi_hmodel_create(const mi_config *cfg, const mi_tensor_desc *weights, size_t n_weights, void **handle);
void mi_hmodel_destroy(void *handle);
int mi_hmodel_forward(void *handle, const float *mix_dev, float *out_dev, int32_t B, int32_t length, void *stream);
int mi_hmodel_tap(void *handle, const char *name, float *dst_dev, int32_t B, int64_t *numel_per_item, void *stream);
int64_t mi_hmodel_device_bytes(void *handle);
int mi_hmodel_status(void *handle, void *stream);

int mi_model_tap(void *handle, const char *name, float *dst_dev, int32_t B, int64_t *numel_per_item, void *stream);

typedef struct mi_profile_row {
    char name[48];
    int64_t launches;
    double ms, flops, bytes;
} mi_profile_row;
int mi_set_two_streams(int32_t enabled);
int mi_set_istft_fused(int32_t enabled);
int mi_set_split_bf16(int32_t enabled);
int mi_set_transpose_tiles(int32_t enabled);
int mi_profile_begin(void *handle);
int mi_profile_end(void *handle, mi_profile_row *rows, int32_t max_rows, int32_t *n_rows, void *stream);

int64_t mi_model_device_bytes(void *handle);

int mi_segments_gather(const float *track_dev, int64_t track_len, int32_t channels, const int64_t *starts_idx_dev,
                       int32_t B, int32_t valid, float *seg_dev, int64_t seg_capacity, void *stream);

int mi_ola_accumulate(float *acc_dev, int64_t acc_len, int32_t rows, const float *model_out_dev, int32_t valid,
                      int64_t out_capacity, const int64_t *offs_idx_dev, const int32_t *lens_idx_dev,
                      const int32_t *trim_idx_dev, int32_t B, int64_t span_lo, int64_t span_hi, const float *weight_dev,
                      int32_t weight_len, void *stream);

int mi_ola_finish(float *acc_dev, int64_t acc_len, int32_t rows, int64_t acc_off0, const int64_t *offs_idx_dev,
                  const int32_t *lens_idx_dev, int32_t n_segments, int32_t max_len, const float *weight_dev, void *stream);

#define MI_PACK_SRC_OFF 0
#define MI_PACK_SRC_LEN 1
#define MI_PACK_START 2
#define MI_PACK_ACC_BASE 3
#define MI_PACK_ACC_LEN 4
#define MI_PACK_OFF 5
#define MI_PACK_LEN 6
#define MI_PACK_TRIM 7
#define MI_PACK_ITEM_COLS 8
#define MI_PACK_T_ACC_BASE 0
#define MI_PACK_T_ACC_LEN 1
#define MI_PACK_T_POS 2
#define MI_PACK_T_LO 3
#define MI_PACK_T_HI 4
#define MI_PACK_T_W_OFF 5
#define MI_PACK_T_W_LEN 6
#define MI_PACK_TILE_COLS 7
#define MI_PACK_TILE_SPAN 1024

int mi_segments_gather_packed(const float *tracks_dev, int64_t tracks_capacity, int32_t channels, const int64_t *items_dev,
                              int32_t B, int32_t valid, float *seg_dev, int64_t seg_capacity, void *stream);

int mi_ola_accumulate_packed(float *acc_dev, int64_t acc_capacity, int32_t rows, const float *model_out_dev, int32_t valid,
                             int64_t out_capacity, const int64_t *items_dev, int32_t B, const int64_t *tiles_dev, int32_t n_tiles,
                             const float *weights_dev, int64_t weights_capacity, void *stream);

int mi_ola_finish_packed(float *acc_dev, int64_t acc_capacity, int32_t rows, const int64_t *tiles_dev, int32_t n_tiles,
                         const int64_t *segs_dev, int32_t n_segs, const float *weights_dev, int64_t weights_capacity, void *stream);

#define MI_EMIT_ACC_BASE 0
#define MI_EMIT_ACC_LEN 1
#define MI_EMIT_Q0 2
#define MI_EMIT_SEG_LO 3
#define MI_EMIT_SEG_HI 4
#define MI_EMIT_W_OFF 5
#define MI_EMIT_W_LEN 6
#define MI_EMIT_MEMBER 7
#define MI_EMIT_PASS_COLS 8
int mi_stream_emit(const float *acc_dev, int64_t acc_capacity, int32_t n_sources, int32_t channels, const int64_t *passes_dev,
                   int32_t n_passes, const int64_t *segs_dev, int32_t n_segs, const float *weights_dev, int64_t weights_capacity,
                   const float *scales_dev, int32_t n_members, int32_t shifts, int32_t bag, const float *stats_dev, int64_t n,
                   float *out_dev, int64_t out_capacity, void *stream);

#define MI_STREAMS_EMIT_PASS_LO 0
#define MI_STREAMS_EMIT_PASS_HI 1
#define MI_STREAMS_EMIT_SEG_LO 2
#define MI_STREAMS_EMIT_SEG_HI 3
#define MI_STREAMS_EMIT_STATS 4
#define MI_STREAMS_EMIT_OUT_OFF 5
#define MI_STREAMS_EMIT_N 6
#define MI_STREAMS_EMIT_COLS 7
#define MI_APPEND_SRC 0
#define MI_APPEND_N 1
#define MI_APPEND_DST_OFF 2
#define MI_APPEND_DST_LEN 3
#define MI_APPEND_COL 4
#define MI_APPEND_STATS 5
#define MI_APPEND_COLS 6
#define MI_COMPACT_SRC_OFF 0
#define MI_COMPACT_DST_OFF 1
#define MI_COMPACT_N 2
#define MI_COMPACT_LEN 3
#define MI_COMPACT_COLS 4
int mi_streams_emit(const float *acc_dev, int64_t acc_capacity, int32_t n_sources, int32_t channels, const int64_t *streams_dev,
                    int32_t n_streams, int64_t max_n, const int64_t *passes_dev, int32_t n_passes, const int64_t *segs_dev, int32_t n_segs,
                    const float *weights_dev, int64_t weights_capacity, const float *scales_dev, int32_t n_members, int32_t shifts,
                    int32_t bag, const float *stats_dev, int32_t n_stats, float *out_dev, int64_t out_capacity, void *stream);
int mi_streams_append(float *win_dev, int64_t win_capacity, int32_t channels, const int64_t *table_dev, int32_t n_streams, int64_t max_n,
                      const float *stats_dev, int32_t n_stats, void *stream);
int mi_streams_compact(float *dst_dev, int64_t dst_capacity, const float *src_dev, int64_t src_capacity, const int64_t *table_dev,
                       int32_t n_rows, int64_t max_len, void *stream);

#define MI_CVT_SRC 0
#define MI_CVT_SRC_CH 1
#define MI_CVT_N_IN 2
#define MI_CVT_BEFORE 3
#define MI_CVT_HIST_LEN 4
#define MI_CVT_HIST_RD 5
#define MI_CVT_HIST_WR 6
#define MI_CVT_HIST_START 7
#define MI_CVT_HIST_NEXT 8
#define MI_CVT_OUT0 9
#define MI_CVT_N_OUT 10
#define MI_CVT_TOTAL 11
#define MI_CVT_OLD 12
#define MI_CVT_NEW 13
#define MI_CVT_WIDTH 14
#define MI_CVT_BANK_OFF 15
#define MI_CVT_DST_OFF 16
#define MI_CVT_DST_LEN 17
#define MI_CVT_COL 18
#define MI_CVT_STATS 19
#define MI_CVT_COLS 20
#define MI_CVT_LDS_FLOATS 16384
int mi_streams_convert_append(float *win_dev, int64_t win_capacity, int32_t channels, const int64_t *table_dev, int32_t n_streams,
                              int64_t max_groups, const float *bank_dev, int64_t bank_capacity, float *hist_dev, int64_t hist_capacity,
                              const float *stats_dev, int32_t n_stats, int32_t lds_floats, void *stream);

int mi_resample_frac(const float *x_dev, int32_t rows, int64_t length, const float *table_dev, int32_t old_sr, int32_t new_sr,
                     int32_t width, float *y_dev, int64_t out_length, void *stream);

int32_t mi_mono_stats_scratch_bytes(void);
int mi_mono_stats(const float *wav_dev, int32_t channels, int64_t length, void *scratch_dev, float *stats_dev, void *stream);
int mi_track_affine(float *x_dev, int64_t numel, const float *stats_dev, int32_t inverse, void *stream);

#define MI_CLIP_RESCALE 1
#define MI_CLIP_CLAMP 2
#define MI_CLIP_TANH 3
int mi_prevent_clip(const float *x_dev, int64_t numel, int32_t mode, void *peak_dev, float *y_dev, void *stream);
int mi_two_stems(const float *const *stems_dev, int32_t n_stems, int32_t selected, const float *origin_dev, int32_t minus, int64_t numel,
                 float *y_dev, void *stream);

#define MI_DELIVER_SRC 0
#define MI_DELIVER_ORIGIN 1
#define MI_DELIVER_N 2
#define MI_DELIVER_KIND 3
#define MI_DELIVER_SEL 4
#define MI_DELIVER_CLIP 5
#define MI_DELIVER_PEAK 6
#define MI_DELIVER_FMT 7
#define MI_DELIVER_DST_OFF 8
#define MI_DELIVER_COLS 9
#define MI_DELIVER_STEM 0
#define MI_DELIVER_ADD 1
#define MI_DELIVER_MINUS 2
#define MI_DELIVER_I16 0
#define MI_DELIVER_F32 1
int mi_deliver_peaks(const int64_t *table_dev, int32_t n_rows, int64_t max_n, int32_t n_sources, int32_t channels, void *peaks_dev,
                     int32_t n_peaks, int64_t dst_capacity, void *stream);
int mi_deliver_pcm(const int64_t *table_dev, int32_t n_rows, int64_t max_n, int32_t n_sources, int32_t channels, const void *peaks_dev,
                   int32_t n_peaks, void *dst_dev, int64_t dst_capacity, void *stream);

#define MI_RATE_SRC 0
#define MI_RATE_N_IN 1
#define MI_RATE_BEFORE 2
#define MI_RATE_KIND 3
#define MI_RATE_SEL 4
#define MI_RATE_CLIP 5
#define MI_RATE_FMT 6
#define MI_RATE_OLD 7
#define MI_RATE_NEW 8
#define MI_RATE_WIDTH 9
#define MI_RATE_BANK_OFF 10
#define MI_RATE_OUT0 11
#define MI_RATE_N_OUT 12
#define MI_RATE_TOTAL 13
#define MI_RATE_HIST_LEN 14
#define MI_RATE_HIST_RD 15
#define MI_RATE_HIST_WR 16
#define MI_RATE_HIST_START 17
#define MI_RATE_HIST_NEXT 18
#define MI_RATE_DST_OFF 19
#define MI_RATE_COLS 20
#define MI_RATE_LDS_FLOATS 16384
int mi_deliver_resample_pcm(const int64_t *table_dev, int32_t n_rows, int64_t max_groups, int32_t n_sources, int32_t channels,
                            const float *bank_dev, int64_t bank_capacity, float *hist_dev, int64_t hist_capacity, int32_t lds_floats,
                            void *dst_dev, int64_t dst_capacity, void *stream);

int mi_stft_cac(const float *mix_dev, int32_t B, int32_t L, float *cac_dev, void *stream);
int mi_istft_cac(const float *x_dev, int32_t B, int32_t S, int32_t L, float *wav_dev, void *stream);

int mi_stft_norm(const float *mix_dev, int32_t B, int32_t L, float *x_dev, int32_t x_pitch, float *norm_dev, float *denorm_dev, void *stream);
int mi_istft_full(const float *y_dev, int32_t B, int32_t S, int32_t L, int32_t y_pitch, const float *denorm_f_dev, const float *xt_dev,
                  int32_t xt_pitch, const float *denorm_t_dev, float *wav_dev, void *stream);
int mi_item_norm(const float *x_dev, int32_t rows, int64_t count, float *y_dev, float *norm_dev, float *denorm_dev, void *stream);
int mi_item_denorm(const float *x_dev, int32_t rows, int64_t count, const float *denorm_dev, float *y_dev, void *stream);

struct mi_conv_desc;
int mi_conv_forward(const struct mi_conv_desc *desc, void *stream);

int mi_conv_pack_split(const float *wt_dev, int32_t Kpad, int32_t Mpad, int32_t tile_m, void *wx_dev, void *stream);

int mi_conv_pack_tap(const float *wt_dev, int32_t Mpad, int32_t Cin, int32_t ntaps, int32_t dtype, void *wtap_dev, void *stream);
int mi_f32_to_image(const float *x_dev, int32_t B, int32_t C, int64_t P, int32_t dtype, void *img_dev, void *stream);

int mi_conv_pack_half(const float *wt_dev, int32_t Kpad, int32_t Mpad, int32_t dtype, void *wh_dev, void *stream);

int mi_attention(const float *q_dev, const float *k_dev, const float *v_dev, float *o_dev, int32_t B, int32_t heads,
                 int32_t Tq, int32_t Tk, int64_t q_batch_stride, int64_t kv_batch_stride, int64_t o_batch_stride,
                 int32_t dtype, void *stream);

int mi_attention_split(const float *q_dev, const float *k_dev, const float *v_dev, float *o_dev, int32_t B, int32_t heads,
                       int32_t Tq, int32_t Tk, int64_t q_batch_stride, int64_t kv_batch_stride, int64_t o_batch_stride,
                       void *stream);

int mi_attention_heads(const void *q_dev, const void *k_dev, const void *v_dev, float *o_dev, int32_t B, int32_t heads, int32_t Tq, int32_t Tk,
                       int32_t Tq_pitch, int32_t Tk_pitch, int32_t dtype, void *stream);

int mi_attention_heads_image(const void *q_dev, const void *k_dev, const void *v_dev, void *img_dev, int64_t n_img, int32_t B, int32_t heads,
                             int32_t Tq, int32_t Tk, int32_t Tq_pitch, int32_t Tk_pitch, int32_t dtype, void *stream);

int mi_attention_image(const float *q_dev, const float *k_dev, const float *v_dev, void *img_dev, int64_t n_img, int32_t B,
                       int32_t heads, int32_t Tq, int32_t Tk, int64_t q_batch_stride, int64_t kv_batch_stride, int32_t dtype,
                       void *stream);

int mi_gn_gelu(float *x_dev, int32_t B, int32_t C, int32_t C_alloc, int32_t D1, int32_t D2, int32_t row_mode, const float *stats_dev,
               const float *w_dev, const float *b_dev, void *stream);

int32_t mi_gram_order(int32_t h);
int mi_gn_gelu_gram(float *x_dev, int32_t B, int32_t h, int32_t C_alloc, int32_t D1, int32_t D2, int32_t pitch, int32_t row_mode,
                    const float *stats_dev, const float *w_dev, const float *b_dev, double *gram_dev, int32_t slots, void *stream);
int mi_dconv_gn_gelu_gram(float *x_dev, int32_t B, int32_t h, int32_t C_alloc, int32_t D1, int32_t D2, int32_t pitch, int32_t row_mode,
                          const float *stats_dev, const float *w_dev, const float *b_dev, double *gram_dev, int32_t slots, void *stream);
int mi_gram_finalize(double *gram_dev, int32_t rows, int32_t h, int32_t slots, const double *wt_dev, const double *ct_dev, double sum_b,
                     double sum_bsq, double cols, double count, float eps, float *stats_out_dev, void *stream);

int mi_lstm_seq(const float *gx_dev, const float *whh_host, int32_t N, int32_t H, int32_t W, float *out_dev, int32_t mode, void *stream);

int mi_layernorm_cf(const float *x_dev, int32_t B, int32_t C, int32_t T, const float *w_dev, const float *b_dev,
                    const float *add_dev, float *y_dev, void *stream);


int mi_token_norm(int32_t mode, const float *x_dev, int32_t B, int32_t C, int32_t T, const float *w_dev, const float *b_dev,
                  const float *pe_dev, const float *gstat_dev, float *y_dev, float *ostat_dev, void *img_dev, int64_t img_n,
                  int32_t img_dtype, void *stream);

int mi_local_attn(const float *qkc_dev, int32_t B, int32_t C, int32_t T, int32_t ld, float *out_dev, int32_t ld_o, void *stream);

int mi_group_norm_apply(const float *x_dev, int32_t B, int32_t Cin, int32_t G, int32_t in_pitch, int32_t in_len, int32_t off,
                        const float *w_dev, const float *b_dev, int32_t glu, int32_t gelu, const float *scale_dev, const float *res_dev,
                        int32_t res_pitch, float *y_dev, int32_t Cout, int32_t out_len, int32_t out_pitch, int32_t chan_div,
                        double *stats_ws_dev, float *stats_out_dev, void *stream);

int mi_blstm_unfold(const float *x_dev, int32_t B, int32_t C, int32_t T, int32_t F, int32_t W, int32_t S, float *frames_dev, void *stream);
int mi_blstm_restitch(const float *frames_dev, int32_t B, int32_t C, int32_t T, int32_t F, int32_t W, int32_t S, const float *skip_dev,
                      float *y_dev, void *stream);

int mi_row_affine_pitch(const float *x_dev, int32_t B, int32_t C, int32_t L, int32_t out_pitch, const float *norm_dev, float *y_dev,
                        void *stream);


int mi_dconv_row(const float *x_dev, float *y_dev, int32_t B, int32_t C, int32_t Fr, int32_t T, const float *weights_host, int32_t variant,
                 void *stream);

int mi_dconv_time_layer(const float *x_dev, float *y_dev, int32_t B, int32_t C, int32_t Lv, int32_t Lp, int32_t dil,
                        const float *weights_host, float *hbuf_dev, double *stats_dev, double *gram_dev, float *st_dev, void *stream);

void mi_debug_set_post_launch_hook(void (*hook)(void *stream));

enum mi_conv_route {
    MI_ROUTE_TABLE = 0,
    MI_ROUTE_DMA = 1,
    MI_ROUTE_DMATAP = 2,
    MI_ROUTE_DMAROW = 3,
    MI_ROUTE_X6 = 4,
    MI_ROUTE_HALF = 5,
    MI_ROUTE_TAP_HALF = 6,
    MI_ROUTE_TAP_X6 = 7,
    MI_ROUTE_ROWS_X6 = 8,
    MI_ROUTE_HALF_IMG = 9,
    MI_ROUTE_HALF_IMG256 = 10
};

int mi_debug_last_conv_route(void);

int mi_debug_last_conv_tile(void);

int mi_debug_conv_route(const struct mi_conv_desc *desc, int *tile);

int mi_debug_switches(char *buf, int32_t n);

const char *mi_last_error(void);
const char *mi_version(void);

#ifdef __cplusplus
}
#endif
#endif
```

Measured before the change: 2357.

## Fuse both time-branch DConv layers into one block launch sequence with DPP halo sharing

```diff
diff --git a/demucs_amd/_lib.py b/demucs_amd/_lib.py
--- a/demucs_amd/_lib.py
+++ b/demucs_amd/_lib.py
@@ -147,6 +147,8 @@
     "mi_dconv_row": (C.c_int, [C.c_void_p, C.c_void_p, C.c_int32, C.c_int32, C.c_int32, C.c_int32, C.c_void_p, C.c_int32, C.c_void_p]),
     "mi_dconv_time_layer": (C.c_int, [C.c_void_p, C.c_void_p, C.c_int32, C.c_int32, C.c_int32, C.c_int32, C.c_int32, C.c_void_p,
                                       C.c_void_p, C.c_void_p, C.c_void_p, C.c_void_p, C.c_void_p]),
+    "mi_dconv_time_block": (C.c_int, [C.c_void_p, C.c_void_p, C.c_void_p, C.c_int32, C.c_int32, C.c_int32, C.c_int32, C.c_int32, C.c_int32,
+                                      C.c_void_p, C.c_void_p, C.c_int64, C.c_void_p, C.c_void_p, C.c_void_p, C.c_void_p]),
     "mi_debug_set_post_launch_hook": (None, [C.c_void_p]),
     "mi_debug_last_conv_route": (C.c_int, []),
     "mi_debug_last_conv_tile": (C.c_int, []),
diff --git a/demucs_amd/csrc/api.hip b/demucs_amd/csrc/api.hip
--- a/demucs_amd/csrc/api.hip
+++ b/demucs_amd/csrc/api.hip
@@ -802,4 +802,32 @@
     return r;
 }
 
-}
+int mi_dconv_time_block(const float *x_dev, float *y1_dev, float *y2_dev, int32_t B, int32_t C, int32_t Lv, int32_t Lp, int32_t dil0, int32_t dil1,
+                        const float *weights_host, float *hbuf_dev, int64_t hbuf_floats, double *stats_dev, double *gram_dev, float *st_dev,
+                        void *stream) {
+    MI_REQUIRE(x_dev && y1_dev && y2_dev && weights_host && hbuf_dev && stats_dev && gram_dev && st_dev, "mi_dconv_time_block: null argument");
+    MI_REQUIRE(B >= 1 && B <= 65535, "mi_dconv_time_block: B = %d outside [1, 65535] (the grid's y range)", B);
+    MI_REQUIRE(dconv_time_supported(C, Lp) && Lv >= 1 && Lp >= Lv, "mi_dconv_time_block: C = %d must be 48 or 96, Lp = %d even and >= Lv = %d >= 1",
+               C, Lp, Lv);
+    MI_REQUIRE(dil0 == 1 && dil1 == 2, "mi_dconv_time_block: dilations (%d, %d): a block is (1, 2)", dil0, dil1);
+    MI_REQUIRE((((uintptr_t)x_dev | (uintptr_t)y1_dev | (uintptr_t)y2_dev | (uintptr_t)hbuf_dev | (uintptr_t)stats_dev | (uintptr_t)gram_dev |
+                 (uintptr_t)st_dev) & 7) == 0, "mi_dconv_time_block: buffers must be 8-byte aligned");
+    const int64_t n = (int64_t)B * C * Lp;
+    MI_REQUIRE(x_dev + n <= y1_dev || y1_dev + n <= x_dev, "mi_dconv_time_block: y1 must not overlap x");
+    MI_REQUIRE(y1_dev + n <= y2_dev || y2_dev + n <= y1_dev, "mi_dconv_time_block: y2 must not overlap y1");
+    MI_REQUIRE(y2_dev == x_dev || x_dev + n <= y2_dev || y2_dev + n <= x_dev, "mi_dconv_time_block: y2 must be x itself or not overlap it");
+    const int64_t need = 2 * (int64_t)B * round_up(C / 8, 4) * Lp;
+    MI_REQUIRE(hbuf_floats >= need, "mi_dconv_time_block: two hidden tensors need %lld floats, hbuf holds %lld", (long long)need, (long long)hbuf_floats);
+    DConvTestLayer l0, l1;
+    MI_TRY(l0.init(C, weights_host));
+    MI_TRY(l1.init(C, weights_host + dconv_layer_floats(C)));
+    hipStream_t st = (hipStream_t)stream;
+    float2 *sp = (float2 *)st_dev;
+    int r = launch_dconv_time_block(l0.l, l1.l, C, B, Lv, Lp, x_dev, y1_dev, y2_dev, hbuf_dev, (size_t)hbuf_floats, stats_dev, gram_dev, sp, sp + B,
+                                    sp + 2 * B, sp + 3 * B, st);
+    const hipError_t e = hipStreamSynchronize(st);
+    if (e != hipSuccess && r == MI_OK) r = set_error(MI_EHIP, "mi_dconv_time_block: hipStreamSynchronize: %s", hipGetErrorString(e));
+    return r;
+}
+
+}
diff --git a/demucs_amd/csrc/dconv_time.hip b/demucs_amd/csrc/dconv_time.hip
--- a/demucs_amd/csrc/dconv_time.hip
+++ b/demucs_amd/csrc/dconv_time.hip
@@ -5,6 +5,8 @@
 
 constexpr int kTC = 6;
 constexpr int kGramMax = 96;
+constexpr int kGramGroup = 16;
+constexpr int kFL = 62;
 
 __device__ __forceinline__ double wsum(double v) {
 #pragma unroll
@@ -12,27 +14,70 @@
     return v;
 }
 
-struct Taps { float v[10]; };
-__device__ __forceinline__ Taps load_taps(const float *row, int t0, int Lv, int Lp) {
-    Taps r;
-#pragma unroll
-    for (int q = 0; q < 5; ++q) {
-        const int p = t0 - 2 + 2 * q;
-        float2 f = make_float2(0.f, 0.f);
-        if (p >= 0 && p < Lp) f = *reinterpret_cast<const float2 *>(row + p);
-        r.v[2 * q] = (p >= 0 && p < Lv) ? f.x : 0.f;
-        r.v[2 * q + 1] = (p + 1 >= 0 && p + 1 < Lv) ? f.y : 0.f;
-    }
-    return r;
+__device__ __forceinline__ float from_lower(float v) {
+    return __builtin_bit_cast(float, __builtin_amdgcn_update_dpp(0, __builtin_bit_cast(int, v), 0x138 , 0xf, 0xf, true));
+}
+__device__ __forceinline__ float from_upper(float v) {
+    return __builtin_bit_cast(float, __builtin_amdgcn_update_dpp(0, __builtin_bit_cast(int, v), 0x130 , 0xf, 0xf, true));
+}
+
+__device__ __forceinline__ unsigned clamp_col(int p, int Lp) { return 4u * (unsigned)min(max(p, 0), Lp - 2); }
+__device__ __forceinline__ float2 ld_at(const float *row, unsigned boff) {
+    return *reinterpret_cast<const float2 *>(reinterpret_cast<const char *>(row) + boff);
+}
+
+struct XChan { float2 a, b, c, e; };
+
+template <int HA, int DIL>
+__device__ __forceinline__ void conv3_taps(const float *w0c , const v2f (&v)[10], v2f (&hid)[kTC][HA / 2]) {
+    const float4 *wv = reinterpret_cast<const float4 *>(w0c);
+#pragma unroll
+    for (int q = 0; q < HA / 4; ++q) {
+        const float4 wa = wv[q], wb = wv[HA / 4 + q], wc = wv[2 * (HA / 4) + q];
+#pragma unroll
+        for (int j = 0; j < kTC; ++j) {
+            const v2f x0 = v[2 + j - DIL], x1 = v[2 + j], x2 = v[2 + j + DIL];
+            hid[j][2 * q] = fma2((v2f){wc.x, wc.y}, x2, fma2((v2f){wb.x, wb.y}, x1, fma2((v2f){wa.x, wa.y}, x0, hid[j][2 * q])));
+            hid[j][2 * q + 1] = fma2((v2f){wc.z, wc.w}, x2, fma2((v2f){wb.z, wb.w}, x1, fma2((v2f){wa.z, wa.w}, x0, hid[j][2 * q + 1])));
+        }
+    }
+}
+
+template <int H, int HA>
+__device__ __forceinline__ void hidden_out(const v2f (&hid)[kTC][HA / 2], float *hb , int t0, int Lv, int Lp, double &p1,
+                                           double &p2) {
+#pragma unroll
+    for (int m = 0; m < H; ++m) {
+#pragma unroll
+        for (int j = 0; j < kTC; ++j)
+            if (t0 + j < Lv) { const double v = (double)hid[j][m >> 1][m & 1]; p1 += v; p2 += v * v; }
+#pragma unroll
+        for (int j = 0; j < kTC; j += 2)
+            if (t0 + j < Lp) *reinterpret_cast<float2 *>(hb + (size_t)m * Lp + j) = make_float2(hid[j][m >> 1][m & 1], hid[j + 1][m >> 1][m & 1]);
+    }
+}
+
+__device__ __forceinline__ void block_stats(double p1, double p2, double *stats, int b) {
+    const int tid = threadIdx.x;
+    const double s1 = wsum(p1), s2 = wsum(p2);
+    __shared__ double red[8];
+    if ((tid & 63) == 0) { red[(tid >> 6) * 2] = s1; red[(tid >> 6) * 2 + 1] = s2; }
+    __syncthreads();
+    if (tid == 0) {
+        double *dst = stats + ((size_t)b * kStatSlots + (blockIdx.x % kStatSlots)) * 2;
+        atomicAdd(dst, red[0] + red[2] + red[4] + red[6]);
+        atomicAdd(dst + 1, red[1] + red[3] + red[5] + red[7]);
+    }
 }
 
 template <int C, int H, int DIL>
 __global__ __launch_bounds__(256) void dconv_t_conv3_kernel(const DConvRowLayer L, const float *__restrict__ x, float *__restrict__ hbuf,
                                                             int Lv, int Lp, double *__restrict__ stats) {
+    static_assert(C % 3 == 0, "the channel loop is unrolled by three");
     constexpr int HA = (H + 3) / 4 * 4;
     __shared__ __attribute__((aligned(16))) float w0s[C * 3 * HA];
     __shared__ float b0s[HA];
-    const int tid = threadIdx.x, b = blockIdx.y;
+    const int tid = threadIdx.x, b = blockIdx.y, lane = tid & 63;
     for (int i = tid; i < C * 3 * HA; i += 256) w0s[i] = L.w0[i];
     if (tid < HA) b0s[tid] = L.b0[tid];
     __syncthreads();
@@ -44,49 +89,37 @@
     for (int j = 0; j < kTC; ++j)
 #pragma unroll
         for (int m = 0; m < HA / 2; ++m) hid[j][m] = (v2f){b0s[2 * m], b0s[2 * m + 1]};
-    if (on) {
-        Taps nx = load_taps(xb, t0, Lv, Lp);
-#pragma unroll 2
-        for (int c = 0; c < C; ++c) {
-            v2f xs[10];
-#pragma unroll
-            for (int i = 0; i < 10; ++i) xs[i] = splat2(nx.v[i]);
-            if (c + 1 < C) nx = load_taps(xb + (size_t)(c + 1) * Lp, t0, Lv, Lp);
-            const float4 *wv = reinterpret_cast<const float4 *>(w0s + c * 3 * HA);
-#pragma unroll
-            for (int q = 0; q < HA / 4; ++q) {
-                const float4 wa = wv[q], wb = wv[HA / 4 + q], wc = wv[2 * (HA / 4) + q];
-#pragma unroll
-                for (int j = 0; j < kTC; ++j) {
-                    const v2f x0 = xs[2 + j - DIL], x1 = xs[2 + j], x2 = xs[2 + j + DIL];
-                    hid[j][2 * q] = fma2((v2f){wc.x, wc.y}, x2, fma2((v2f){wb.x, wb.y}, x1, fma2((v2f){wa.x, wa.y}, x0, hid[j][2 * q])));
-                    hid[j][2 * q + 1] = fma2((v2f){wc.z, wc.w}, x2, fma2((v2f){wb.z, wb.w}, x1, fma2((v2f){wa.z, wa.w}, x0, hid[j][2 * q + 1])));
-                }
-            }
-        }
+    if (t0 - lane * kTC < Lv) {
+        const bool first = lane == 0, last = lane == 63;
+        const int pe = first ? t0 - 2 : t0 + kTC;
+        const unsigned oa = clamp_col(t0, Lp), ob = clamp_col(t0 + 2, Lp), oc = clamp_col(t0 + 4, Lp), oe = clamp_col(pe, Lp);
+        const bool me0 = pe >= 0 && pe < Lv, me1 = pe >= 0 && pe + 1 < Lv;
+        auto fetch = [&](int c) {
+            const float *row = xb + (size_t)c * Lp;
+            XChan r;
+            r.a = ld_at(row, oa); r.b = ld_at(row, ob); r.c = ld_at(row, oc);
+            r.e = make_float2(0.f, 0.f);
+            if (first || last) r.e = ld_at(row, oe);
+            return r;
+        };
+        XChan c0 = fetch(0), c1 = fetch(1), c2 = fetch(2);
+        auto step = [&](int c, XChan &s, bool refill) {
+            __builtin_amdgcn_sched_barrier(0);
+            const float x0 = t0 < Lv ? s.a.x : 0.f, x1 = t0 + 1 < Lv ? s.a.y : 0.f, x2 = t0 + 2 < Lv ? s.b.x : 0.f, x3 = t0 + 3 < Lv ? s.b.y : 0.f,
+                        x4 = t0 + 4 < Lv ? s.c.x : 0.f, x5 = t0 + 5 < Lv ? s.c.y : 0.f, e0 = me0 ? s.e.x : 0.f, e1 = me1 ? s.e.y : 0.f;
+            const float dl0 = from_lower(x4), dl1 = from_lower(x5), dr0 = from_upper(x0), dr1 = from_upper(x1);
+            const v2f v[10] = {splat2(first ? e0 : dl0), splat2(first ? e1 : dl1), splat2(x0), splat2(x1), splat2(x2), splat2(x3), splat2(x4),
+                               splat2(x5), splat2(last ? e0 : dr0), splat2(last ? e1 : dr1)};
+            if (refill) s = fetch(c + 3);
+            conv3_taps<HA, DIL>(w0s + c * 3 * HA, v, hid);
+        };
+#pragma unroll 1
+        for (int c = 0; c < C - 3; c += 3) { step(c, c0, true); step(c + 1, c1, true); step(c + 2, c2, true); }
+        step(C - 3, c0, false); step(C - 2, c1, false); step(C - 1, c2, false);
     }
     double p1 = 0.0, p2 = 0.0;
-    if (on) {
-        float *hb = hbuf + (size_t)b * HA * Lp + t0;
-#pragma unroll
-        for (int m = 0; m < H; ++m) {
-#pragma unroll
-            for (int j = 0; j < kTC; ++j)
-                if (t0 + j < Lv) { const double v = (double)hid[j][m >> 1][m & 1]; p1 += v; p2 += v * v; }
-#pragma unroll
-            for (int j = 0; j < kTC; j += 2)
-                if (t0 + j < Lp) *reinterpret_cast<float2 *>(hb + (size_t)m * Lp + j) = make_float2(hid[j][m >> 1][m & 1], hid[j + 1][m >> 1][m & 1]);
-        }
-    }
-    double s1 = wsum(p1), s2 = wsum(p2);
-    __shared__ double red[8];
-    if ((tid & 63) == 0) { red[(tid >> 6) * 2] = s1; red[(tid >> 6) * 2 + 1] = s2; }
-    __syncthreads();
-    if (tid == 0) {
-        double *dst = stats + ((size_t)b * kStatSlots + (blockIdx.x % kStatSlots)) * 2;
-        atomicAdd(dst, red[0] + red[2] + red[4] + red[6]);
-        atomicAdd(dst + 1, red[1] + red[3] + red[5] + red[7]);
-    }
+    if (on) hidden_out<H, HA>(hid, hbuf + (size_t)b * HA * Lp + t0, t0, Lv, Lp, p1, p2);
+    block_stats(p1, p2, stats, b);
 }
 
 template <int H, int HA>
@@ -115,6 +148,7 @@
                                                            const float2 *__restrict__ st1, double *__restrict__ gram) {
     constexpr int HA = (H + 3) / 4 * 4, NG = H * (H + 1) / 2 + H;
     __shared__ double red[4][NG];
+    __shared__ __attribute__((aligned(16))) float slab[4][kGramGroup * 64];
     __shared__ float gws[HA], gbs[HA];
     const int tid = threadIdx.x, b = blockIdx.y, lane = tid & 63, wv = tid >> 6;
     if (tid < HA) { gws[tid] = L.g1w[tid]; gbs[tid] = L.g1b[tid]; }
@@ -129,7 +163,26 @@
 #pragma unroll
             for (int m = 0; m < HA; ++m) g[j][m] = 0.f;
     }
-    int idx = 0;
+    float *gp = slab[wv];
+    auto reduce_group = [&](int grp) {
+        const int e = lane >> 2, q = lane & 3, n = kGramGroup * grp + e;
+        const float4 *src4 = reinterpret_cast<const float4 *>(gp + e * 64 + 16 * q);
+        double sacc = 0.0;
+#pragma unroll
+        for (int v4 = 0; v4 < 4; ++v4) {
+            const float4 f = src4[v4];
+            sacc += (double)f.x; sacc += (double)f.y; sacc += (double)f.z; sacc += (double)f.w;
+        }
+        sacc += __shfl_xor(sacc, 1);
+        sacc += __shfl_xor(sacc, 2);
+        if (q == 0 && n < NG) red[wv][n] = sacc;
+    };
+    int n = 0;
+    auto entry = [&](float p) {
+        gp[(n & (kGramGroup - 1)) * 64 + lane] = p;
+        if ((n & (kGramGroup - 1)) == kGramGroup - 1 || n == NG - 1) reduce_group(n / kGramGroup);
+        ++n;
+    };
 #pragma unroll
     for (int i = 0; i < H; ++i) {
 #pragma unroll
@@ -137,9 +190,7 @@
             float p = 0.f;
 #pragma unroll
             for (int j = 0; j < kTC; ++j) p = fmaf(g[j][i], g[j][k], p);
-            const double r = wsum((double)p);
-            if (lane == 0) red[wv][idx] = r;
-            ++idx;
+            entry(p);
         }
     }
 #pragma unroll
@@ -147,9 +198,7 @@
         float p = 0.f;
 #pragma unroll
         for (int j = 0; j < kTC; ++j) p += g[j][i];
-        const double r = wsum((double)p);
-        if (lane == 0) red[wv][idx] = r;
-        ++idx;
+        entry(p);
     }
     __syncthreads();
     if (tid < NG)
@@ -185,101 +234,224 @@
     }
 }
 
+template <int C, int HA>
+struct OutLds {
+    __attribute__((aligned(16))) float w3s[4 * C * HA];
+    float b3s[2 * C], g2ws[2 * C], g2bs[2 * C], lss[C], gws[HA], gbs[HA];
+};
+template <int C, int HA>
+__device__ __forceinline__ void out_stage(const DConvRowLayer &L, OutLds<C, HA> &s) {
+    const int tid = threadIdx.x;
+    for (int i = tid; i < 4 * C * HA; i += 256) {
+        const int half = (i >> 1) & 1, k = (i >> 2) % HA, c = (i >> 2) / HA;
+        s.w3s[i] = L.w3[(size_t)(c + half * C) * HA + k];
+    }
+    for (int i = tid; i < 2 * C; i += 256) { s.b3s[i] = L.b3[i]; s.g2ws[i] = L.g2w[i]; s.g2bs[i] = L.g2b[i]; }
+    for (int i = tid; i < C; i += 256) s.lss[i] = L.ls[i];
+    if (tid < HA) { s.gws[tid] = L.g1w[tid]; s.gbs[tid] = L.g1b[tid]; }
+}
+template <int C, int HA>
+__device__ __forceinline__ void out_channel(const OutLds<C, HA> &s, int c, const v2f (&gp)[kTC / 2][HA], float mu2, float rs2, const float (&r)[kTC],
+                                            float (&o)[kTC]) {
+    const float4 *wp = reinterpret_cast<const float4 *>(s.w3s + (size_t)c * HA * 4);
+    v2f zv[kTC / 2], zg[kTC / 2];
+#pragma unroll
+    for (int jp = 0; jp < kTC / 2; ++jp) { zv[jp] = splat2(s.b3s[c]); zg[jp] = splat2(s.b3s[c + C]); }
+#pragma unroll
+    for (int k = 0; k < HA; ++k) {
+        const float4 w = wp[k];
+#pragma unroll
+        for (int jp = 0; jp < kTC / 2; ++jp) {
+            zv[jp] = fma2((v2f){w.x, w.y}, gp[jp][k], zv[jp]);
+            zg[jp] = fma2((v2f){w.z, w.w}, gp[jp][k], zg[jp]);
+        }
+    }
+    const float aA = rs2 * s.g2ws[c], aB = s.g2bs[c] - mu2 * aA, gA = rs2 * s.g2ws[c + C], gB = s.g2bs[c + C] - mu2 * gA, sc = s.lss[c];
+#pragma unroll
+    for (int j = 0; j < kTC; ++j) o[j] = r[j] + sc * (fmaf(zv[j >> 1][j & 1], aA, aB) * sigmoid_f(fmaf(zg[j >> 1][j & 1], gA, gB)));
+}
+struct Res { float2 a, b, c; };
+struct ResOff { unsigned a, b, c; };
+__device__ __forceinline__ Res ld_res(const float *row, const ResOff &o) { return Res{ld_at(row, o.a), ld_at(row, o.b), ld_at(row, o.c)}; }
+
 template <int C, int H>
 __global__ __launch_bounds__(256) void dconv_t_out_kernel(const DConvRowLayer L, const float *__restrict__ x, const float *__restrict__ hbuf,
                                                           float *__restrict__ y, int Lv, int Lp, const float2 *__restrict__ st1,
                                                           const float2 *__restrict__ st2) {
+    static_assert(C % 3 == 0, "the channel loop is unrolled by three");
     constexpr int HA = (H + 3) / 4 * 4;
-    __shared__ __attribute__((aligned(16))) float w3s[4 * C * HA];
-    __shared__ float b3s[2 * C], g2ws[2 * C], g2bs[2 * C], lss[C], gws[HA], gbs[HA];
+    __shared__ OutLds<C, HA> sm;
     const int tid = threadIdx.x, b = blockIdx.y;
-    for (int i = tid; i < 4 * C * HA; i += 256) {
-        const int half = (i >> 1) & 1, k = (i >> 2) % HA, c = (i >> 2) / HA;
-        w3s[i] = L.w3[(size_t)(c + half * C) * HA + k];
-    }
-    for (int i = tid; i < 2 * C; i += 256) { b3s[i] = L.b3[i]; g2ws[i] = L.g2w[i]; g2bs[i] = L.g2b[i]; }
-    for (int i = tid; i < C; i += 256) lss[i] = L.ls[i];
-    if (tid < HA) { gws[tid] = L.g1w[tid]; gbs[tid] = L.g1b[tid]; }
+    out_stage<C, HA>(L, sm);
     __syncthreads();
     const int t0 = (blockIdx.x * 256 + tid) * kTC;
     if (t0 >= Lv) return;
     const float2 s1 = st1[b], s2 = st2[b];
     float g[kTC][HA];
-    load_g<H, HA>(hbuf + (size_t)b * HA * Lp + t0, Lp, t0, Lv, s1.x, s1.y, gws, gbs, g);
-    const float *xb = x + (size_t)b * C * Lp + t0;
+    load_g<H, HA>(hbuf + (size_t)b * HA * Lp + t0, Lp, t0, Lv, s1.x, s1.y, sm.gws, sm.gbs, g);
+    const float *xb = x + (size_t)b * C * Lp;
     float *yb = y + (size_t)b * C * Lp + t0;
-    const float mu2 = s2.x, rs2 = s2.y;
-    auto ld3 = [&](const float *p, float (&r)[kTC]) {
-#pragma unroll
-        for (int j = 0; j < kTC; j += 2) {
-            float2 f = make_float2(0.f, 0.f);
-            if (t0 + j < Lp) f = *reinterpret_cast<const float2 *>(p + j);
-            r[j] = f.x; r[j + 1] = f.y;
-        }
-    };
     v2f gp[kTC / 2][HA];
 #pragma unroll
     for (int jp = 0; jp < kTC / 2; ++jp)
 #pragma unroll
         for (int m = 0; m < HA; ++m) gp[jp][m] = (v2f){g[2 * jp][m], g[2 * jp + 1][m]};
-    float rn[kTC];
-    ld3(xb, rn);
-#pragma unroll 2
-    for (int c = 0; c < C; ++c) {
-        float r[kTC];
-#pragma unroll
-        for (int j = 0; j < kTC; ++j) r[j] = rn[j];
-        if (c + 1 < C) ld3(xb + (size_t)(c + 1) * Lp, rn);
-        const float4 *wp = reinterpret_cast<const float4 *>(w3s + (size_t)c * HA * 4);
-        v2f zv[kTC / 2], zg[kTC / 2];
-#pragma unroll
-        for (int jp = 0; jp < kTC / 2; ++jp) { zv[jp] = splat2(b3s[c]); zg[jp] = splat2(b3s[c + C]); }
-#pragma unroll
-        for (int k = 0; k < HA; ++k) {
-            const float4 w = wp[k];
-#pragma unroll
-            for (int jp = 0; jp < kTC / 2; ++jp) {
-                zv[jp] = fma2((v2f){w.x, w.y}, gp[jp][k], zv[jp]);
-                zg[jp] = fma2((v2f){w.z, w.w}, gp[jp][k], zg[jp]);
-            }
-        }
-        const float aA = rs2 * g2ws[c], aB = g2bs[c] - mu2 * aA, gA = rs2 * g2ws[c + C], gB = g2bs[c + C] - mu2 * gA, sc = lss[c];
+    const ResOff ro{clamp_col(t0, Lp), clamp_col(t0 + 2, Lp), clamp_col(t0 + 4, Lp)};
+    Res r0 = ld_res(xb, ro), r1 = ld_res(xb + (size_t)Lp, ro), r2 = ld_res(xb + 2 * (size_t)Lp, ro);
+    auto step = [&](int c, Res &rs, bool refill) {
+        __builtin_amdgcn_sched_barrier(0);
+        const float r[kTC] = {rs.a.x, rs.a.y, rs.b.x, rs.b.y, rs.c.x, rs.c.y};
         float o[kTC];
-#pragma unroll
-        for (int j = 0; j < kTC; ++j) o[j] = r[j] + sc * (fmaf(zv[j >> 1][j & 1], aA, aB) * sigmoid_f(fmaf(zg[j >> 1][j & 1], gA, gB)));
+        out_channel<C, HA>(sm, c, gp, s2.x, s2.y, r, o);
+        if (refill) rs = ld_res(xb + (size_t)(c + 3) * Lp, ro);
 #pragma unroll
         for (int j = 0; j < kTC; j += 2)
             if (t0 + j < Lp) *reinterpret_cast<float2 *>(yb + (size_t)c * Lp + j) = make_float2(o[j], o[j + 1]);
-    }
+    };
+#pragma unroll 1
+    for (int c = 0; c < C - 3; c += 3) { step(c, r0, true); step(c + 1, r1, true); step(c + 2, r2, true); }
+    step(C - 3, r0, false); step(C - 2, r1, false); step(C - 1, r2, false);
+}
+
+template <int C, int H>
+__global__ __launch_bounds__(256) void dconv_t_out_conv3_kernel(const DConvRowLayer L1, const DConvRowLayer L2, const float *__restrict__ x,
+                                                                const float *__restrict__ h1, float *__restrict__ y1, float *__restrict__ h2,
+                                                                int Lv, int Lp, const float2 *__restrict__ st1, const float2 *__restrict__ st2,
+                                                                double *__restrict__ stats) {
+    static_assert(C % 3 == 0, "the channel loop is unrolled by three");
+    constexpr int HA = (H + 3) / 4 * 4;
+    __shared__ OutLds<C, HA> sm;
+    __shared__ __attribute__((aligned(16))) float w0s[C * 3 * HA];
+    __shared__ float b0s[HA];
+    const int tid = threadIdx.x, b = blockIdx.y, lane = tid & 63;
+    out_stage<C, HA>(L1, sm);
+    for (int i = tid; i < C * 3 * HA; i += 256) w0s[i] = L2.w0[i];
+    if (tid < HA) b0s[tid] = L2.b0[tid];
+    __syncthreads();
+    const int wbase = (blockIdx.x * 4 + (tid >> 6)) * kFL * kTC;
+    const int t0 = wbase + (lane - 1) * kTC;
+    const bool act = t0 >= 0 && t0 < Lv;
+    const bool own = act && lane >= 1 && lane <= kFL;
+    v2f hid[kTC][HA / 2];
+#pragma unroll
+    for (int j = 0; j < kTC; ++j)
+#pragma unroll
+        for (int m = 0; m < HA / 2; ++m) hid[j][m] = (v2f){b0s[2 * m], b0s[2 * m + 1]};
+    if (wbase < Lv) {
+        const float2 s1 = st1[b], s2 = st2[b];
+        float g[kTC][HA];
+        if (act) load_g<H, HA>(h1 + (size_t)b * HA * Lp + t0, Lp, t0, Lv, s1.x, s1.y, sm.gws, sm.gbs, g);
+        else {
+#pragma unroll
+            for (int j = 0; j < kTC; ++j)
+#pragma unroll
+                for (int m = 0; m < HA; ++m) g[j][m] = 0.f;
+        }
+        v2f gp[kTC / 2][HA];
+#pragma unroll
+        for (int jp = 0; jp < kTC / 2; ++jp)
+#pragma unroll
+            for (int m = 0; m < HA; ++m) gp[jp][m] = (v2f){g[2 * jp][m], g[2 * jp + 1][m]};
+        const float *xb = x + (size_t)b * C * Lp;
+        float *yb = y1 + (size_t)b * C * Lp + t0;
+        const ResOff ro{clamp_col(t0, Lp), clamp_col(t0 + 2, Lp), clamp_col(t0 + 4, Lp)};
+        Res r0 = ld_res(xb, ro), r1 = ld_res(xb + (size_t)Lp, ro), r2 = ld_res(xb + 2 * (size_t)Lp, ro);
+        auto step = [&](int c, Res &rs, bool refill) {
+            __builtin_amdgcn_sched_barrier(0);
+            const float r[kTC] = {rs.a.x, rs.a.y, rs.b.x, rs.b.y, rs.c.x, rs.c.y};
+            float o[kTC];
+            out_channel<C, HA>(sm, c, gp, s2.x, s2.y, r, o);
+            if (refill) rs = ld_res(xb + (size_t)(c + 3) * Lp, ro);
+            if (own) {
+#pragma unroll
+                for (int j = 0; j < kTC; j += 2)
+                    if (t0 + j < Lp) *reinterpret_cast<float2 *>(yb + (size_t)c * Lp + j) = make_float2(o[j], o[j + 1]);
+            }
+            float z[kTC];
+#pragma unroll
+            for (int j = 0; j < kTC; ++j) z[j] = (act && t0 + j < Lv) ? o[j] : 0.f;
+            const float l0 = from_lower(z[4]), l1 = from_lower(z[5]), u0 = from_upper(z[0]), u1 = from_upper(z[1]);
+            const v2f v[10] = {splat2(l0), splat2(l1), splat2(z[0]), splat2(z[1]), splat2(z[2]), splat2(z[3]), splat2(z[4]), splat2(z[5]),
+                               splat2(u0), splat2(u1)};
+            __builtin_amdgcn_sched_barrier(0);
+            conv3_taps<HA, 2>(w0s + c * 3 * HA, v, hid);
+        };
+#pragma unroll 1
+        for (int c = 0; c < C - 3; c += 3) { step(c, r0, true); step(c + 1, r1, true); step(c + 2, r2, true); }
+        step(C - 3, r0, false); step(C - 2, r1, false); step(C - 1, r2, false);
+    }
+    double p1 = 0.0, p2 = 0.0;
+    if (own) hidden_out<H, HA>(hid, h2 + (size_t)b * HA * Lp + t0, t0, Lv, Lp, p1, p2);
+    block_stats(p1, p2, stats, b);
 }
 
 bool dconv_time_supported(int C, int Lp) { return (C == 48 || C == 96) && Lp % 2 == 0; }
+
+namespace {
+template <int C, int H>
+int time_pass_a(const DConvTimeLayer &l, int dil, int B, int Lv, int Lp, const float *x, float *hbuf, double *stats, float2 *st1, hipStream_t st) {
+    const dim3 grid(ceil_div(Lv, 256 * kTC), B), blk(256);
+    if (dil == 1) hipLaunchKernelGGL((dconv_t_conv3_kernel<C, H, 1>), grid, blk, 0, st, l.w, x, hbuf, Lv, Lp, stats);
+    else hipLaunchKernelGGL((dconv_t_conv3_kernel<C, H, 2>), grid, blk, 0, st, l.w, x, hbuf, Lv, Lp, stats);
+    MI_CHECK_LAUNCH();
+    return launch_finalize_stats(stats, B, (double)H * Lv, 1e-5f, 0, st1, nullptr, st);
+}
+template <int C, int H>
+int time_pass_b(const DConvTimeLayer &l, int B, int Lv, int Lp, const float *hbuf, double *gram, const float2 *st1, float2 *st2, hipStream_t st) {
+    hipLaunchKernelGGL((dconv_t_gram_kernel<H>), dim3(ceil_div(Lv, 256 * kTC), B), dim3(256), 0, st, l.w, hbuf, Lv, Lp, st1, gram);
+    MI_CHECK_LAUNCH();
+    hipLaunchKernelGGL(dconv_t_gram_finalize_kernel, dim3(B), dim3(64), 0, st, gram, H, l.gram_a, l.gram_v, l.gram_c, l.sum_b3, l.sum_b3sq,
+                       (double)Lv, 2.0 * C * Lv, 1e-5f, st2);
+    MI_CHECK_LAUNCH();
+    return MI_OK;
+}
+template <int C, int H>
+int time_pass_c(const DConvTimeLayer &l, int B, int Lv, int Lp, const float *x, const float *hbuf, float *y, const float2 *st1, const float2 *st2,
+                hipStream_t st) {
+    hipLaunchKernelGGL((dconv_t_out_kernel<C, H>), dim3(ceil_div(Lv, 256 * kTC), B), dim3(256), 0, st, l.w, x, hbuf, y, Lv, Lp, st1, st2);
+    MI_CHECK_LAUNCH();
+    return MI_OK;
+}
+template <int C, int H>
+int time_layer(const DConvTimeLayer &l, int dil, int B, int Lv, int Lp, const float *x, float *y, float *hbuf, double *stats, double *gram,
+               float2 *st1, float2 *st2, hipStream_t st) {
+    MI_TRY((time_pass_a<C, H>(l, dil, B, Lv, Lp, x, hbuf, stats, st1, st)));
+    MI_TRY((time_pass_b<C, H>(l, B, Lv, Lp, hbuf, gram, st1, st2, st)));
+    return time_pass_c<C, H>(l, B, Lv, Lp, x, hbuf, y, st1, st2, st);
+}
+template <int C, int H>
+int time_block(const DConvTimeLayer &l0, const DConvTimeLayer &l1, int B, int Lv, int Lp, const float *x, float *y1, float *y2, float *hbuf,
+               double *stats, double *gram, float2 *st1a, float2 *st2a, float2 *st1b, float2 *st2b, hipStream_t st) {
+    constexpr int HA = (H + 3) / 4 * 4;
+    float *h1 = hbuf, *h2 = hbuf + (size_t)B * HA * Lp;
+    MI_TRY((time_pass_a<C, H>(l0, 1, B, Lv, Lp, x, h1, stats, st1a, st)));
+    MI_TRY((time_pass_b<C, H>(l0, B, Lv, Lp, h1, gram, st1a, st2a, st)));
+    hipLaunchKernelGGL((dconv_t_out_conv3_kernel<C, H>), dim3(ceil_div(Lv, 4 * kFL * kTC), B), dim3(256), 0, st, l0.w, l1.w, x, h1, y1, h2, Lv, Lp,
+                       st1a, st2a, stats);
+    MI_CHECK_LAUNCH();
+    MI_TRY(launch_finalize_stats(stats, B, (double)H * Lv, 1e-5f, 0, st1b, nullptr, st));
+    MI_TRY((time_pass_b<C, H>(l1, B, Lv, Lp, h2, gram, st1b, st2b, st)));
+    return time_pass_c<C, H>(l1, B, Lv, Lp, y1, h2, y2, st1b, st2b, st);
+}
+}
 
 int launch_dconv_time_layer(const DConvTimeLayer &l, int C, int dil, int B, int Lv, int Lp, const float *x, float *y, float *hbuf,
                             double *stats, double *gram, float2 *st1, float2 *st2, hipStream_t st) {
     MI_REQUIRE(dconv_time_supported(C, Lp) && (dil == 1 || dil == 2), "dconv_time: unsupported C=%d Lp=%d dil=%d", C, Lp, dil);
     MI_REQUIRE(x != y && ((uintptr_t)x & 7) == 0 && ((uintptr_t)y & 7) == 0 && ((uintptr_t)hbuf & 7) == 0, "dconv_time: bad buffers");
-    const int H = C / 8;
-    const dim3 grid(ceil_div(Lv, 256 * kTC), B), blk(256);
-#define MI_DT(CC, HH)                                                                                                         \
-    do {                                                                                                                      \
-        if (dil == 1) hipLaunchKernelGGL((dconv_t_conv3_kernel<CC, HH, 1>), grid, blk, 0, st, l.w, x, hbuf, Lv, Lp, stats);      \
-        else hipLaunchKernelGGL((dconv_t_conv3_kernel<CC, HH, 2>), grid, blk, 0, st, l.w, x, hbuf, Lv, Lp, stats);               \
-        MI_CHECK_LAUNCH();                                                                                                    \
-        MI_TRY(launch_finalize_stats(stats, B, (double)HH * Lv, 1e-5f, 0, st1, nullptr, st));                                  \
-        hipLaunchKernelGGL((dconv_t_gram_kernel<HH>), grid, blk, 0, st, l.w, hbuf, Lv, Lp, st1, gram);                           \
-        MI_CHECK_LAUNCH();                                                                                                    \
-        hipLaunchKernelGGL(dconv_t_gram_finalize_kernel, dim3(B), dim3(64), 0, st, gram, HH, l.gram_a, l.gram_v,               \
-                           l.gram_c, l.sum_b3, l.sum_b3sq, (double)Lv, 2.0 * CC * Lv, 1e-5f, st2);                             \
-        MI_CHECK_LAUNCH();                                                                                                    \
-        hipLaunchKernelGGL((dconv_t_out_kernel<CC, HH>), grid, blk, 0, st, l.w, x, hbuf, y, Lv, Lp, st1, st2);                   \
-        MI_CHECK_LAUNCH();                                                                                                    \
-    } while (0)
-    if (C == 48) MI_DT(48, 6);
-    else MI_DT(96, 12);
-#undef MI_DT
-    (void)H;
-    return MI_OK;
-}
-
-}
+    if (C == 48) return time_layer<48, 6>(l, dil, B, Lv, Lp, x, y, hbuf, stats, gram, st1, st2, st);
+    return time_layer<96, 12>(l, dil, B, Lv, Lp, x, y, hbuf, stats, gram, st1, st2, st);
+}
+
+int launch_dconv_time_block(const DConvTimeLayer &l0, const DConvTimeLayer &l1, int C, int B, int Lv, int Lp, const float *x, float *y1,
+                            float *y2, float *hbuf, size_t hbuf_floats, double *stats, double *gram, float2 *st1a, float2 *st2a,
+                            float2 *st1b, float2 *st2b, hipStream_t st) {
+    MI_REQUIRE(dconv_time_supported(C, Lp), "dconv_time: unsupported C=%d Lp=%d", C, Lp);
+    MI_REQUIRE(x != y1 && y1 != y2 && (((uintptr_t)x | (uintptr_t)y1 | (uintptr_t)y2 | (uintptr_t)hbuf) & 7) == 0, "dconv_time: bad buffers");
+    const size_t need = 2 * (size_t)B * ((C / 8 + 3) / 4 * 4) * Lp;
+    MI_REQUIRE(hbuf_floats >= need, "dconv_time: two hidden tensors need %zu floats, the buffer holds %zu", need, hbuf_floats);
+    if (C == 48) return time_block<48, 6>(l0, l1, B, Lv, Lp, x, y1, y2, hbuf, stats, gram, st1a, st2a, st1b, st2b, st);
+    return time_block<96, 12>(l0, l1, B, Lv, Lp, x, y1, y2, hbuf, stats, gram, st1a, st2a, st1b, st2b, st);
+}
+
+}
diff --git a/demucs_amd/csrc/engine_core.h b/demucs_amd/csrc/engine_core.h
--- a/demucs_amd/csrc/engine_core.h
+++ b/demucs_amd/csrc/engine_core.h
@@ -181,6 +181,7 @@
     int make_ktab(const Gather &g, int Kpad, mi_ktab_entry **out);
     int load_dconv(const WeightTable &wt, const std::string &prefix, int C, int64_t chan_stride, int D2, bool freq, DConvW *dw, int comp = 8);
     double *dconv_gram = nullptr;
+    size_t dconv_hidden_floats = 0;
     double *dconv_gram2 = nullptr;
     size_t dconv_gram2_bytes = 0;
     bool dconv_tap_dma = false;
diff --git a/demucs_amd/csrc/engine_core.hip b/demucs_amd/csrc/engine_core.hip
--- a/demucs_amd/csrc/engine_core.hip
+++ b/demucs_amd/csrc/engine_core.hip
@@ -313,12 +313,8 @@
     if (w.has_time && g.row_mode == 0 && g.D1 == 1) {
         MI_REQUIRE(dconv_gram, "dconv: the engine set no Gram buffer for the time kernels");
         return prof.timed(102, "dconv_time_kernels", 2.0 * 2.0 * (3.0 * C * h + 2.0 * C * h) * (double)g.B * g.D2, 2.0 * 4.0 * C * (double)g.B * g.D2, st, [&] {
-            float *s = x, *dd = tmp;
-            for (int dlayer = 0; dlayer < 2; ++dlayer) {
-                MI_TRY(launch_dconv_time_layer(w.tl[dlayer], C, 1 << dlayer, g.B, g.D2, g.pitch(), s, dd, hidden, stats, dconv_gram, st1, st2, st));
-                std::swap(s, dd);
-            }
-            return (int)MI_OK;
+            return launch_dconv_time_block(w.tl[0], w.tl[1], C, g.B, g.D2, g.pitch(), x, tmp, x, hidden, dconv_hidden_floats, stats, dconv_gram,
+                                           st1, st2, st1, st2, st);
         });
     }
     const double cnt_row = g.row_mode ? (double)g.D2 : (double)g.D1 * g.D2;
diff --git a/demucs_amd/csrc/kernels.h b/demucs_amd/csrc/kernels.h
--- a/demucs_amd/csrc/kernels.h
+++ b/demucs_amd/csrc/kernels.h
@@ -94,6 +94,9 @@
 bool dconv_time_supported(int C, int Lp);
 int launch_dconv_time_layer(const DConvTimeLayer &l, int C, int dil, int B, int Lv, int Lp, const float *x, float *y, float *hbuf,
                             double *stats, double *gram, float2 *st1, float2 *st2, hipStream_t st);
+int launch_dconv_time_block(const DConvTimeLayer &l0, const DConvTimeLayer &l1, int C, int B, int Lv, int Lp, const float *x, float *y1,
+                            float *y2, float *hbuf, size_t hbuf_floats, double *stats, double *gram, float2 *st1a, float2 *st2a,
+                            float2 *st1b, float2 *st2b, hipStream_t st);
 
 int launch_conv(const mi_conv_desc &d, hipStream_t st);
 
diff --git a/demucs_amd/csrc/model.h b/demucs_amd/csrc/model.h
--- a/demucs_amd/csrc/model.h
+++ b/demucs_amd/csrc/model.h
@@ -36,6 +36,7 @@
     float *w_yspec = nullptr, *w_ytime = nullptr, *w_yt = nullptr, *w_fr = nullptr;
     double *w_stats = nullptr, *w_stats_t = nullptr, *w_gram = nullptr, *w_gram2 = nullptr, *w_gram2_t = nullptr;
     size_t gram2t_bytes = 0;
+    size_t hidden_floats = 0;
     size_t gram2_bytes = 0;
     float2 *w_st1 = nullptr, *w_st2 = nullptr, *w_st1_t = nullptr, *w_st2_t = nullptr;
     float2 *w_norm_f = nullptr, *w_denorm_f = nullptr, *w_norm_t = nullptr, *w_denorm_t = nullptr;
diff --git a/demucs_amd/csrc/model.hip b/demucs_amd/csrc/model.hip
--- a/demucs_amd/csrc/model.hip
+++ b/demucs_amd/csrc/model.hip
@@ -234,7 +234,7 @@
         ws = w;
     }
     static_cast<WorkspacePtrs &>(*this) = *ws;
-    dconv_gram = w_gram; dconv_gram2 = w_gram2; dconv_gram2_bytes = gram2_bytes;
+    dconv_gram = w_gram; dconv_hidden_floats = hidden_floats; dconv_gram2 = w_gram2; dconv_gram2_bytes = gram2_bytes;
     dconv_tap_dma = true;
     return MI_OK;
 }
@@ -262,6 +262,7 @@
             w.w_eimg[0][i] = pf; w.w_eimg[1][i] = pt;
         }
     MI_TRY(A(&w.w_h, big / 2)); MI_TRY(A(&w.w_th, big / 2));
+    w.hidden_floats = (big / 2) * B;
     for (float **p : {&w.w_a, &w.w_b, &w.w_ta, &w.w_tb, &w.w_c, &w.w_tc}) {
         MI_TRY(w.mem.alloc((void **)p, (big * B + 64) * sizeof(float)));
         *p += 32;
diff --git a/include/demucs_amd.h b/include/demucs_amd.h
--- a/include/demucs_amd.h
+++ b/include/demucs_amd.h
@@ -310,6 +310,10 @@
 int mi_dconv_time_layer(const float *x_dev, float *y_dev, int32_t B, int32_t C, int32_t Lv, int32_t Lp, int32_t dil,
                         const float *weights_host, float *hbuf_dev, double *stats_dev, double *gram_dev, float *st_dev, void *stream);
 
+int mi_dconv_time_block(const float *x_dev, float *y1_dev, float *y2_dev, int32_t B, int32_t C, int32_t Lv, int32_t Lp, int32_t dil0, int32_t dil1,
+                        const float *weights_host, float *hbuf_dev, int64_t hbuf_floats, double *stats_dev, double *gram_dev, float *st_dev,
+                        void *stream);
+
 void mi_debug_set_post_launch_hook(void (*hook)(void *stream));
 
 enum mi_conv_route {
```

Measured after the change: 2361, median of 2. No clear change (+0.1%).
